# electech6/ORB_SLAM3_detailed_comments

Measured on AMD Instinct MI355X. Metric: frames/sec ORB extract+match, 752x480 stereo @1200 feat (1 frame = 1 stereo pair; BASELINE.json configs[1]), higher is better.
Workload: dtype u8

## Files before the change

orb_slam3_detailed_comments_amd/csrc/k_describe.hip:

```cpp
#include "orbx_types.h"
#include "orbx_block.h"
#include "orbx_simd.h"
#include "orbx_kernels.h"
#include "undistort_model.h"
#include "glibc_sincosf_model.h"
#include "glibc_logf_model.h"
#include "glibc_tanf_model.h"
#include "glibc_atan2f_model.h"

namespace orbx {

__device__ const signed char d_brief_pattern[1024] = {
#include "brief_pattern.inc"
};
#define BRIEF_PATTERN d_brief_pattern

__device__ __forceinline__ float fast_atan2_deg(float y, float x) {
    const float s = (float)(180.0 / 3.1415926535897932384626433832795);
    const float p1 = 0.9997878412794807f * s, p3 = -0.3258083974640975f * s;
    const float p5 = 0.1555786518463281f * s, p7 = -0.04432655554792128f * s;
    const float eps = 2.2204460492503131e-16f;
    const float ax = fabsf(x), ay = fabsf(y);
    float a, c, c2;
    if (ax >= ay) {
        c = __fdiv_rn(ay, __fadd_rn(ax, eps)); c2 = __fmul_rn(c, c);
        a = __fmul_rn(__fadd_rn(__fmul_rn(__fadd_rn(__fmul_rn(__fadd_rn(__fmul_rn(p7, c2), p5), c2), p3), c2), p1), c);
    } else {
        c = __fdiv_rn(ax, __fadd_rn(ay, eps)); c2 = __fmul_rn(c, c);
        a = __fsub_rn(90.f, __fmul_rn(__fadd_rn(__fmul_rn(__fadd_rn(__fmul_rn(__fadd_rn(__fmul_rn(p7, c2), p5), c2), p3), c2), p1), c));
    }
    if (x < 0) a = __fsub_rn(180.f, a);
    if (y < 0) a = __fsub_rn(360.f, a);
    return a;
}

__device__ __forceinline__ void steer_from_moments(float m01, float m10, float* angle, float* a, float* b) {
    const float ang = fast_atan2_deg(m01, m10);
    const float factorPI = (float)(3.1415926535897932384626433832795 / 180.f);
    const float rad = __fmul_rn(ang, factorPI);
    *angle = ang; *a = glibc_cosf(rad); *b = glibc_sinf(rad);
}

constexpr int kLayoutPer = 8;
__global__ void __launch_bounds__(256) k_layout(const LevelInfo* __restrict__ lv, int nlevels,
                                                const uint32_t* __restrict__ lvl_keys, int kp_total_cap,
                                                const int* __restrict__ lvl_count, int lap0, int lap1,
                                                int* __restrict__ final_idx, int* __restrict__ n_out, int* __restrict__ mono_out,
                                                int nb, int* __restrict__ row_start, int* __restrict__ row_items) {
    ORBX_DYN_SMEM(smem);
    __shared__ unsigned long long s_scan[20];
    __shared__ int s_cnt[kMaxLevels], s_off[kMaxLevels + 1];
    __shared__ float s_scale[kMaxLevels];
    const int b = (int)blockIdx.x, tid = (int)threadIdx.x;
    if (tid < nlevels) { s_cnt[tid] = lvl_count[(size_t)b * nlevels + tid]; s_off[tid] = lv[tid].kp_off; s_scale[tid] = lv[tid].scale; }
    if (tid == 0) s_off[nlevels] = kp_total_cap;
    int* hist = (int*)smem; int* cursor = hist + (nb + 1);
    if (row_start != nullptr) for (int i = tid; i <= nb; i += 256) hist[i] = 0;
    __syncthreads();
    auto bucket_of = [&](uint32_t key, int l) {
        float yf = (float)(key_y(key) + kBorder);
        if (l != 0) yf = __fmul_rn(yf, s_scale[l]);
        const int first = (int)floorf(__fsub_rn(yf, __fmul_rn(2.0f, s_scale[l])));
        return imin(imax(first, 0) >> kStereoRowShift, nb - 1);
    };
    int total = 0;
    for (int l = 0; l < nlevels; l++) total += s_cnt[l];
    int mono_run = 0, lap_run = 0;
    int valid[kLayoutPer], lvl[kLayoutPer], fin[kLayoutPer];
    uint32_t key[kLayoutPer];
    for (int base = 0; base < kp_total_cap; base += 256 * kLayoutPer) {
        const int s0 = base + tid * kLayoutPer;
        int l = 0;
        while (l + 1 < nlevels && s_off[l + 1] <= s0) l++;
#pragma unroll
        for (int k = 0; k < kLayoutPer; k++) {
            const int s = s0 + k;
            while (l + 1 < nlevels && s_off[l + 1] <= s) l++;
            lvl[k] = l;
            valid[k] = s < kp_total_cap && s - s_off[l] < s_cnt[l];
            key[k] = valid[k] ? lvl_keys[(size_t)b * kp_total_cap + s] : 0u;
        }
        int lapf[kLayoutPer], nm = 0, nl = 0;
#pragma unroll
        for (int k = 0; k < kLayoutPer; k++) {
            float xf = (float)(key_x(key[k]) + kBorder);
            if (lvl[k] != 0) xf = __fmul_rn(xf, s_scale[lvl[k]]);
            lapf[k] = valid[k] && xf >= (float)lap0 && xf <= (float)lap1;
            nm += valid[k] && !lapf[k]; nl += lapf[k];
            if (row_start != nullptr && valid[k]) atomicAdd(&hist[bucket_of(key[k], lvl[k])], 1);
        }
        unsigned long long tot;
        const unsigned long long ex = block_excl_scan<unsigned long long>((unsigned long long)nm | ((unsigned long long)nl << 32), &tot, s_scan);
        int pm = mono_run + (int)(ex & 0xFFFFFFFFu), pl = lap_run + (int)(ex >> 32);
#pragma unroll
        for (int k = 0; k < kLayoutPer; k++) {
            fin[k] = lapf[k] ? total - 1 - pl : pm;
            if (valid[k]) { final_idx[(size_t)b * kp_total_cap + s0 + k] = fin[k]; if (lapf[k]) pl++; else pm++; }
            else if (s0 + k < kp_total_cap) final_idx[(size_t)b * kp_total_cap + s0 + k] = total + (s0 + k) - (pm + pl);
        }
        mono_run += (int)(tot & 0xFFFFFFFFu); lap_run += (int)(tot >> 32);
    }
    if (tid == 0) { n_out[b] = total; mono_out[b] = mono_run; }
    if (row_start == nullptr) return;
    __syncthreads();
    int run = 0;
    for (int c0 = 0; c0 < nb; c0 += 256) {
        const int c = c0 + tid;
        const int v = c < nb ? hist[c] : 0;
        unsigned long long tot;
        const int ex = run + (int)block_excl_scan<unsigned long long>((unsigned long long)v, &tot, s_scan);
        if (c < nb) { cursor[c] = ex; row_start[(size_t)b * (nb + 1) + c] = ex; }
        run += (int)tot;
    }
    if (tid == 0) row_start[(size_t)b * (nb + 1) + nb] = run;
    __syncthreads();
    if (kp_total_cap <= 256 * kLayoutPer) {
#pragma unroll
        for (int k = 0; k < kLayoutPer; k++)
            if (valid[k]) row_items[(size_t)b * kp_total_cap + atomicAdd(&cursor[bucket_of(key[k], lvl[k])], 1)] = fin[k];
        return;
    }
    int l = 0;
    for (int s = tid; s < kp_total_cap; s += 256) {
        while (l + 1 < nlevels && s_off[l + 1] <= s) l++;
        if (s - s_off[l] < s_cnt[l])
            row_items[(size_t)b * kp_total_cap + atomicAdd(&cursor[bucket_of(lvl_keys[(size_t)b * kp_total_cap + s], l)], 1)] = final_idx[(size_t)b * kp_total_cap + s];
    }
}

constexpr int kKpPerWave = 8;
constexpr int kWinR = 18, kWinRows = 2 * kWinR + 1, kWinDw = 10, kWinTrips = (kWinRows * kWinDw + 63) / 64;
static_assert(kKpPerWave == kKpPerWaveDecl, "orbx_kernels.h out of date");
constexpr int kKpPerWaveSmall = kKpPerWaveSmallDecl;
template <int KPW>
__device__ __forceinline__ void orient_brief_impl(const LevelInfo* __restrict__ lv, int nlevels,
                                                      const uint8_t* __restrict__ pyr, const uint8_t* __restrict__ blur, size_t pyr_stride,
                                                      const uint32_t* __restrict__ lvl_keys, int kp_total_cap,
                                                      const int* __restrict__ lvl_count, const int* __restrict__ final_idx,
                                                      UmaxTab umax, KeyPointRec* __restrict__ out_kps,
                                                      unsigned long long* __restrict__ out_desc, int4* __restrict__ out_aux, int B, int groups_per_image) {
    __shared__ __attribute__((aligned(16))) uint8_t s_win[4][kWinRows * kWinDw * 4];
    const int id = (int)blockIdx.x, nx = groups_per_image;
    const int b = 8 * (id / (8 * nx)) + (id & 7), gx = (id >> 3) % nx;
    if (b >= B) return;
    const int lane = lane_id();
    const int slot0 = (gx * 4 + (int)(threadIdx.x >> 6)) * KPW;
    if (slot0 >= kp_total_cap) return;
    const int myslot = slot0 + (lane < KPW ? lane : 0);
    int my_valid = 0, my_level = 0, my_pitch = 0, my_fi = 0;
    uint32_t my_key = 0;
    int my_off = 0;
    if (myslot < kp_total_cap) {
        for (int l = 1; l < nlevels; l++) if (myslot >= lv[l].kp_off) my_level = l;
        const int i = myslot - lv[my_level].kp_off;
        my_valid = i < lvl_count[(size_t)b * nlevels + my_level];
        if (!my_valid && lane < KPW) {
            const int zrow = final_idx[(size_t)b * kp_total_cap + myslot];
            unsigned long long* z = out_desc + ((size_t)b * kp_total_cap + zrow) * 4;
            z[0] = 0ull; z[1] = 0ull; z[2] = 0ull; z[3] = 0ull;
        }
        if (my_valid) {
            my_key = lvl_keys[(size_t)b * kp_total_cap + myslot];
            my_pitch = lv[my_level].pitch;
            my_off = (int)lv[my_level].off + (key_y(my_key) + kBorder) * my_pitch + (key_x(my_key) + kBorder);
            my_fi = final_idx[(size_t)b * kp_total_cap + myslot];
        }
    }
    const unsigned long long vmask = __ballot(my_valid && lane < KPW);
    if (vmask == 0ull) return;
    const BufRsrc raw0 = buf_make(pyr + (size_t)b * pyr_stride);
    const BufRsrc blur0 = buf_make(blur + (size_t)b * pyr_stride);
    const int r8 = lane >> 3, cg = lane & 7;
    uint32_t wu4[4], wv4[4], on4[4];
#pragma unroll
    for (int trip = 0; trip < 4; trip++) {
        const int v = -kHalfPatch + 8 * trip + r8;
        const int av = v < 0 ? -v : v;
        uint32_t pu = 0, pv = 0, po = 0;
#pragma unroll
        for (int j = 0; j < 4; j++) {
            const int u = -kHalfPatch + 4 * cg + j;
            const int au = u < 0 ? -u : u;
            const bool on = av <= kHalfPatch && au <= kHalfPatch && au <= umax.u[av <= kHalfPatch ? av : 0];
            if (on) { pu |= (uint32_t)(u + 16) << (8 * j); pv |= (uint32_t)(v + 16) << (8 * j); po |= 1u << (8 * j); }
        }
        wu4[trip] = pu; wv4[trip] = pv; on4[trip] = po;
    }
    int my_m10 = 0, my_m01 = 0;
    for (int k = 0; k < KPW; k++) {
        if (!((vmask >> k) & 1ull)) continue;
        const int pitch = ORBX_READLANE(my_pitch, k);
        const uint32_t so = (uint32_t)(ORBX_READLANE(my_off, k) - kHalfPatch * pitch - kHalfPatch);
        uint32_t I4[4];
#pragma unroll
        for (int trip = 0; trip < 4; trip++)
            I4[trip] = buf_load_u32(raw0, (uint32_t)(__mul24(8 * trip + r8, pitch) + 4 * cg), so);
        uint32_t du = 0, dv = 0, ds = 0;
#pragma unroll
        for (int trip = 0; trip < 4; trip++) { du = dot4_u8(I4[trip], wu4[trip], du); dv = dot4_u8(I4[trip], wv4[trip], dv); ds = dot4_u8(I4[trip], on4[trip], ds); }
        int m10 = (int)du - 16 * (int)ds, m01 = (int)dv - 16 * (int)ds;
        m10 = wave_sum(m10); m01 = wave_sum(m01);
        if (lane == k) { my_m10 = m10; my_m01 = m01; }
    }
    float my_angle, my_a, my_b;
    steer_from_moments((float)my_m01, (float)my_m10, &my_angle, &my_a, &my_b);
    float px0[4], py0[4], px1[4], py1[4];
#pragma unroll
    for (int r = 0; r < 4; r++) {
        const signed char* p = &BRIEF_PATTERN[4 * (64 * r + lane)];
        px0[r] = (float)p[0]; py0[r] = (float)p[1]; px1[r] = (float)p[2]; py1[r] = (float)p[3];
    }
    uint8_t* win = s_win[threadIdx.x >> 6];
    for (int k = 0; k < KPW; k++) {
        if (!((vmask >> k) & 1ull)) continue;
        const int pitch = ORBX_READLANE(my_pitch, k);
        const uint32_t so = (uint32_t)(ORBX_READLANE(my_off, k) - kWinR * pitch - kWinR);
        const float a = __int_as_float(ORBX_READLANE(__float_as_int(my_a), k)), bb = __int_as_float(ORBX_READLANE(__float_as_int(my_b), k));
        const int fi = ORBX_READLANE(my_fi, k);
        uint32_t wv[kWinTrips];
#pragma unroll
        for (int t = 0; t < kWinTrips; t++) {
            const int i = lane + 64 * t;
            if (i < kWinRows * kWinDw) wv[t] = buf_load_u32(blur0, (uint32_t)(__mul24(i / kWinDw, pitch) + 4 * (i % kWinDw)), so);
        }
        ORBX_WAVE_SYNC();
#pragma unroll
        for (int t = 0; t < kWinTrips; t++) { const int i = lane + 64 * t; if (i < kWinRows * kWinDw) ((uint32_t*)win)[i] = wv[t]; }
        ORBX_WAVE_SYNC();
        constexpr float kRoundMagic = 12582912.0f;
        constexpr uint32_t kRoundFold = 0x400000u * (4u * kWinDw) + 0x4B400000u - (uint32_t)(kWinR * 4 * kWinDw + kWinR);
        int t0v[4], t1v[4];
#pragma unroll
        for (int r = 0; r < 4; r++) {
            const uint32_t r0 = __float_as_uint(__fadd_rn(__fadd_rn(__fmul_rn(px0[r], bb), __fmul_rn(py0[r], a)), kRoundMagic));
            const uint32_t c0 = __float_as_uint(__fadd_rn(__fsub_rn(__fmul_rn(px0[r], a), __fmul_rn(py0[r], bb)), kRoundMagic));
            const uint32_t r1 = __float_as_uint(__fadd_rn(__fadd_rn(__fmul_rn(px1[r], bb), __fmul_rn(py1[r], a)), kRoundMagic));
            const uint32_t c1 = __float_as_uint(__fadd_rn(__fsub_rn(__fmul_rn(px1[r], a), __fmul_rn(py1[r], bb)), kRoundMagic));
            t0v[r] = win[(uint32_t)__umul24(r0, 4 * kWinDw) + c0 - kRoundFold];
            t1v[r] = win[(uint32_t)__umul24(r1, 4 * kWinDw) + c1 - kRoundFold];
        }
        unsigned long long mine = 0;
#pragma unroll
        for (int r = 0; r < 4; r++) {
            const unsigned long long w = ORBX_BALLOT(t0v[r] < t1v[r]);
            if (lane == r) mine = w;
        }
        if (lane < 4) out_desc[((size_t)b * kp_total_cap + fi) * 4 + lane] = mine;
    }
    if (lane < KPW && my_valid) {
        const LevelInfo L = lv[my_level];
        KeyPointRec k;
        float xf = (float)(key_x(my_key) + kBorder), yf = (float)(key_y(my_key) + kBorder);
        if (my_level != 0) { xf = __fmul_rn(xf, L.scale); yf = __fmul_rn(yf, L.scale); }
        k.x = xf; k.y = yf; k.size = (float)L.patch; k.angle = my_angle; k.response = (float)key_s(my_key);
        k.octave = my_level; k.class_id = -1;
        out_kps[(size_t)b * kp_total_cap + my_fi] = k;
        const float r = __fmul_rn(2.0f, L.scale);
        int4 aux; aux.x = (int)floorf(__fsub_rn(yf, r)); aux.y = (int)ceilf(__fadd_rn(yf, r)); aux.z = __float_as_int(xf); aux.w = my_level;
        out_aux[(size_t)b * kp_total_cap + my_fi] = aux;
    }
}

__global__ void __launch_bounds__(256) k_orient_brief(const LevelInfo* __restrict__ lv, int nlevels,
                                                      const uint8_t* __restrict__ pyr, const uint8_t* __restrict__ blur, size_t pyr_stride,
                                                      const uint32_t* __restrict__ lvl_keys, int kp_total_cap,
                                                      const int* __restrict__ lvl_count, const int* __restrict__ final_idx,
                                                      UmaxTab umax, KeyPointRec* __restrict__ out_kps,
                                                      unsigned long long* __restrict__ out_desc, int4* __restrict__ out_aux, int B, int groups_per_image) {
    orient_brief_impl<kKpPerWave>(lv, nlevels, pyr, blur, pyr_stride, lvl_keys, kp_total_cap, lvl_count, final_idx, umax, out_kps, out_desc, out_aux, B, groups_per_image);
}
__global__ void __launch_bounds__(256) k_orient_brief_small(const LevelInfo* __restrict__ lv, int nlevels,
                                                      const uint8_t* __restrict__ pyr, const uint8_t* __restrict__ blur, size_t pyr_stride,
                                                      const uint32_t* __restrict__ lvl_keys, int kp_total_cap,
                                                      const int* __restrict__ lvl_count, const int* __restrict__ final_idx,
                                                      UmaxTab umax, KeyPointRec* __restrict__ out_kps,
                                                      unsigned long long* __restrict__ out_desc, int4* __restrict__ out_aux, int B, int groups_per_image) {
    orient_brief_impl<kKpPerWaveSmall>(lv, nlevels, pyr, blur, pyr_stride, lvl_keys, kp_total_cap, lvl_count, final_idx, umax, out_kps, out_desc, out_aux, B, groups_per_image);
}

__global__ void __launch_bounds__(256) k_undistort(const KeyPointRec* __restrict__ kps, const int* __restrict__ n_per_frame, int cap, UndistortParams U,
                                                   KeyPointRec* __restrict__ kps_un) {
    const size_t b = blockIdx.y;
    const int i = (int)(blockIdx.x * 256 + threadIdx.x);
    if (i >= cap || i >= n_per_frame[b]) return;
    KeyPointRec k = kps[b * (size_t)cap + i];
    float x, y;
    undistort_point(U, k.x, k.y, &x, &y);
    k.x = x; k.y = y;
    kps_un[b * (size_t)cap + i] = k;
}

__global__ void __launch_bounds__(256) k_model_selftest(int op, uint32_t start_bits, const float* __restrict__ a, const float* __restrict__ b, int n,
                                                        float* __restrict__ out) {
    const int i = (int)(blockIdx.x * 256 + threadIdx.x);
    if (i >= n) return;
    const float x = a != nullptr ? a[i] : at_float(start_bits + (uint32_t)i);
    const float y = b != nullptr ? b[i] : 0.0f;
    float r = 0.0f;
    switch (op) {
        case 0: r = glibc_cosf(x); break;
        case 1: r = glibc_sinf(x); break;
        case 2: r = glibc_logf_model<false>(x); break;
        case 3: r = glibc_tanf_model(x); break;
        case 4: r = glibc_atanf_model(x); break;
        case 5: r = glibc_atan2f_model(x, y); break;
        case 6: r = fast_atan2_deg(x, y); break;
        default: {
            float ca, sa;
            steer_from_moments(x, y, &r, &ca, &sa);
            out[(size_t)n + i] = ca; out[2 * (size_t)n + i] = sa;
        }
    }
    out[i] = r;
}

}
```

orb_slam3_detailed_comments_amd/csrc/k_match.hip:

```cpp
#include "orbx_types.h"
#include "orbx_block.h"
#include "orbx_kernels.h"
#include "orbx_simd.h"
#include "kb8_model.h"

namespace orbx {

__device__ __forceinline__ int hamming256(const unsigned long long* __restrict__ a, const unsigned long long* __restrict__ b) {
    return __popcll(a[0] ^ b[0]) + __popcll(a[1] ^ b[1]) + __popcll(a[2] ^ b[2]) + __popcll(a[3] ^ b[3]);
}

__global__ void __launch_bounds__(256) k_hamming_matrix(const unsigned long long* __restrict__ A, int na,
                                                        const unsigned long long* __restrict__ Bm, int nb,
                                                        int* __restrict__ out) {
    const int i = (int)blockIdx.y, j = (int)(blockIdx.x * 256 + threadIdx.x);
    if (i >= na || j >= nb) return;
    out[(size_t)i * nb + j] = hamming256(A + 4 * (size_t)i, Bm + 4 * (size_t)j);
}

__global__ void __launch_bounds__(256) k_stereo_match(const LevelInfo* __restrict__ lv,
                                                      const KeyPointRec* __restrict__ kpsL, const unsigned long long* __restrict__ descL, const int* __restrict__ nL,
                                                      const KeyPointRec* __restrict__ kpsR, const unsigned long long* __restrict__ descR,
                                                      const int4* __restrict__ auxR, const int* __restrict__ nR,
                                                      const int* __restrict__ bucket_start, const int* __restrict__ bucket_items, int nb, int lookback,
                                                      int cap, const uint8_t* __restrict__ pyrL, const uint8_t* __restrict__ pyrR, size_t pyr_stride,
                                                      StereoParams P, float* __restrict__ uRight, float* __restrict__ depth, int* __restrict__ sad) {
    const int b = (int)blockIdx.y, lane = lane_id();
    const int iL = (int)blockIdx.x * 4 + (int)(threadIdx.x >> 6);
    if (iL >= cap) return;
    const size_t o = (size_t)b * cap + iL;
    if (iL >= nL[b]) { if (lane == 0) { uRight[o] = -1.0f; depth[o] = -1.0f; sad[o] = -1; } return; }
    const KeyPointRec kL = kpsL[o];
    const int levelL = kL.octave;
    const float uL = kL.x, vL = kL.y;
    const float maxD = __fdiv_rn(P.mbf, P.mb);
    const float minU = __fsub_rn(uL, maxD), maxU = uL;
    float out_u = -1.0f, out_d = -1.0f; int out_sad = -1;
    const int rowL = __float2int_rz(vL);
    const int nr = nR[b];
    unsigned best = (unsigned)P.th_high << 16;
    if (!(maxU < 0)) {
        const unsigned long long* dl = descL + 4 * o;
        const unsigned long long d0 = dl[0], d1 = dl[1], d2 = dl[2], d3 = dl[3];
        const int4* ar = auxR + (size_t)b * cap;
        const int* bs = bucket_start + (size_t)b * (nb + 1);
        const int* items = bucket_items + (size_t)b * cap;
        const int jbeg = bs[imin(imax(rowL - lookback, 0) >> kStereoRowShift, nb - 1)], jend = bs[imin(imax(rowL, 0) >> kStereoRowShift, nb - 1) + 1];
        auto visit = [&](int iR, const int4& a) {
            if (rowL < a.x || rowL > a.y) return;
            if (a.w < levelL - 1 || a.w > levelL + 1) return;
            const float xr = __int_as_float(a.z);
            if (xr >= minU && xr <= maxU) {
                const unsigned long long* dr = descR + 4 * ((size_t)b * cap + iR);
                const int dist = __popcll(d0 ^ dr[0]) + __popcll(d1 ^ dr[1]) + __popcll(d2 ^ dr[2]) + __popcll(d3 ^ dr[3]);
                const unsigned cand = ((unsigned)dist << 16) | (unsigned)iR;
                if ((P.debug_flags & 2) ? dist < (int)(best >> 16) : cand < best) best = cand;
            }
        };
        if (P.debug_flags & 4) {
            for (int j = jend - 1; j >= jbeg; j--) { const int iR = items[j]; visit(iR, ar[iR]); }
        } else
        for (int base = jbeg; base < jend; base += 128) {
            int4 a[2]; int idx[2];
#pragma unroll
            for (int u = 0; u < 2; u++) {
                int j = base + 64 * u + lane;
                const bool in = j < jend;
                if (P.debug_flags & 1) j = jend - 1 - (j - jbeg);
                idx[u] = in ? items[j] : -1;
            }
#pragma unroll
            for (int u = 0; u < 2; u++) {
                if (idx[u] >= 0) a[u] = ar[idx[u]]; else { a[u].x = 1; a[u].y = 0; a[u].z = 0; a[u].w = 0; }
            }
#pragma unroll
            for (int u = 0; u < 2; u++) visit(idx[u], a[u]);
        }
    }
    best = wave_min_u32(best);
    const int bestDist = (int)(best >> 16);
    if (bestDist < P.th_orb && nr > 0) {
        const int bestIdxR = (int)(best & 0xFFFFu);
        const float uR0 = kpsR[(size_t)b * cap + bestIdxR].x;
        const LevelInfo Lv = lv[levelL];
        const float sf = Lv.inv_scale;
        const float scaleduL = roundf(__fmul_rn(kL.x, sf)), scaledvL = roundf(__fmul_rn(kL.y, sf));
        const float scaleduR0 = roundf(__fmul_rn(uR0, sf));
        const int w = 5, Lh = 5;
        const float iniu = scaleduR0 + (float)(Lh - w), endu = scaleduR0 + (float)(Lh + w + 1);
        const int cu = (int)scaleduL, cv = (int)scaledvL, cr = (int)scaleduR0;
        const bool inb = cv - w >= 0 && cv + w < Lv.h && cu - w >= 0 && cu + w < Lv.w && cr - Lh - w >= 0 && cr + Lh + w < Lv.w;
        if (!(iniu < 0 || endu >= (float)Lv.w) && inb) {
            const uint8_t* IL = pyrL + (size_t)b * pyr_stride + Lv.off;
            const uint8_t* IR = pyrR + (size_t)b * pyr_stride + Lv.off;
            const int g = lane >> 4, k = lane & 15;
            uint32_t acc = 0;
            if (k < 11) {
#pragma unroll
                for (int t = 0; t < 3; t++) {
                    const int row = g + 4 * t;
                    if (row < 11) {
                        const int rofs = __mul24(cv - w + row, Lv.pitch);
                        const uint8_t* lp = IL + (uint32_t)(rofs + (cu - w));
                        const uint8_t* rp = IR + (uint32_t)(rofs + (cr - w - Lh + k));
                        const uint32_t l0 = load_u32_any(lp), l1 = load_u32_any(lp + 4), l2 = load_u32_any(lp + 7) & 0xFFFFFF00u;
                        const uint32_t r0 = load_u32_any(rp), r1 = load_u32_any(rp + 4), r2 = load_u32_any(rp + 7) & 0xFFFFFF00u;
                        acc = sad4_u8(l0, r0, sad4_u8(l1, r1, sad4_u8(l2, r2, acc)));
                    }
                }
            }
            acc += __shfl_xor(acc, 16);
            acc += __shfl_xor(acc, 32);
            const unsigned skey = wave_min_u32(k < 11 ? (acc << 4) | (unsigned)k : 0xFFFFFFFFu);
            const int bestS = (int)(skey >> 4), bi = (int)(skey & 15u), bestinc = bi - Lh;
            if (!(bestinc == -Lh || bestinc == Lh)) {
                const float dist1 = (float)ORBX_READLANE(acc, bi - 1), dist2 = (float)bestS, dist3 = (float)ORBX_READLANE(acc, bi + 1);
                const float deltaR = __fdiv_rn(__fsub_rn(dist1, dist3),
                                               __fmul_rn(2.0f, __fsub_rn(__fadd_rn(dist1, dist3), __fmul_rn(2.0f, dist2))));
                if (!(deltaR < -1 || deltaR > 1)) {
                    float bestuR = __fmul_rn(Lv.scale, __fadd_rn(__fadd_rn(scaleduR0, (float)bestinc), deltaR));
                    float disparity = __fsub_rn(uL, bestuR);
                    if (disparity >= 0 && disparity < maxD) {
                        if (disparity <= 0) { disparity = 0.01f; bestuR = (float)((double)uL - 0.01); }
                        out_d = __fdiv_rn(P.mbf, disparity);
                        out_u = bestuR;
                        out_sad = bestS;
                    }
                }
            }
        }
    }
    if (lane == 0) { uRight[o] = out_u; depth[o] = out_d; sad[o] = out_sad; }
}

__global__ void __launch_bounds__(256) k_stereo_median(const int* __restrict__ nL, int cap,
                                                       float* __restrict__ uRight, float* __restrict__ depth,
                                                       const int* __restrict__ sad, int* __restrict__ n_matches) {
    __shared__ unsigned long long s_scan[20];
    __shared__ int s_hist[256];
    __shared__ int s_med[3];
    const int b = (int)blockIdx.x, tid = (int)threadIdx.x;
    const int n = nL[b];
    const int* sd = sad + (size_t)b * cap;
    int med = -1;
    for (int pass = 0; pass < 2; pass++) {
        s_hist[tid] = 0;
        __syncthreads();
        const int bin = pass ? s_med[1] : 0;
        for (int i = tid; i < n; i += 256) {
            const int s = sd[i];
            if (s >= 0 && (pass == 0 || (s >> 7) == bin)) atomicAdd(&s_hist[pass ? s & 127 : imin(s >> 7, 255)], 1);
        }
        __syncthreads();
        unsigned long long tot;
        const int c = s_hist[tid];
        const int ex = (int)block_excl_scan<unsigned long long>((unsigned long long)c, &tot, s_scan);
        const int cnt = pass ? 0 : (int)tot;
        if (pass == 0 && cnt == 0) { if (tid == 0) n_matches[b] = 0; return; }
        const int k = pass ? s_med[2] : cnt / 2;
        if (ex <= k && k < ex + c) {
            if (pass == 0) { s_med[1] = tid; s_med[2] = k - ex; }
            else s_med[0] = (bin << 7) | tid;
        }
        __syncthreads();
    }
    med = s_med[0];
    const float median = (float)med;
    const float thDist = __fmul_rn(1.5f * 1.4f, median);
    int kept = 0;
    for (int i = tid; i < n; i += 256) {
        const int s = sad[(size_t)b * cap + i];
        if (s >= 0) {
            if (!((float)s < thDist)) { uRight[(size_t)b * cap + i] = -1.0f; depth[(size_t)b * cap + i] = -1.0f; }
            else kept++;
        }
    }
    kept = wave_sum(kept);
    if ((tid & 63) == 0) s_scan[tid >> 6] = (unsigned long long)kept;
    __syncthreads();
    if (tid == 0) n_matches[b] = (int)(s_scan[0] + s_scan[1] + s_scan[2] + s_scan[3]);
}

__global__ void __launch_bounds__(256) k_knn2(const unsigned long long* __restrict__ descQ, const int* __restrict__ qoff, const int* __restrict__ nq,
                                              const unsigned long long* __restrict__ descT, const int* __restrict__ toff, const int* __restrict__ nt,
                                              int cap, int* __restrict__ idx0, int* __restrict__ dist0, int* __restrict__ idx1, int* __restrict__ dist1,
                                              uint8_t* __restrict__ ratio_ok) {
    const int b = (int)blockIdx.y, lane = lane_id();
    const int q = (int)blockIdx.x * 4 + (int)(threadIdx.x >> 6);
    const int q0 = qoff ? qoff[b] : 0, t0 = toff ? toff[b] : 0;
    const int nQ = nq[b] - q0, nT = nt[b] - t0;
    if (q >= cap) return;
    const size_t o = (size_t)b * cap + q;
    if (q >= nQ) { if (lane == 0) { idx0[o] = -1; idx1[o] = -1; dist0[o] = -1; dist1[o] = -1; ratio_ok[o] = 0; } return; }
    const unsigned long long* dq = descQ + 4 * ((size_t)b * cap + q0 + q);
    const unsigned long long a0 = dq[0], a1 = dq[1], a2 = dq[2], a3 = dq[3];
    unsigned k0 = 0xFFFFFFFFu, k1 = 0xFFFFFFFFu;
    for (int j = lane; j < nT; j += 64) {
        const unsigned long long* dt = descT + 4 * ((size_t)b * cap + t0 + j);
        const int d = __popcll(a0 ^ dt[0]) + __popcll(a1 ^ dt[1]) + __popcll(a2 ^ dt[2]) + __popcll(a3 ^ dt[3]);
        const unsigned key = ((unsigned)d << 16) | (unsigned)j;
        if (key < k0) { k1 = k0; k0 = key; } else if (key < k1) k1 = key;
    }
    const unsigned b0 = wave_min_u32(k0);
    if (k0 == b0) k0 = k1;
    const unsigned b1 = wave_min_u32(k0);
    if (lane == 0) {
        const int i0 = b0 == 0xFFFFFFFFu ? -1 : (int)(b0 & 0xFFFF), i1 = b1 == 0xFFFFFFFFu ? -1 : (int)(b1 & 0xFFFF);
        const int dd0 = i0 < 0 ? -1 : (int)(b0 >> 16), dd1 = i1 < 0 ? -1 : (int)(b1 >> 16);
        idx0[o] = i0; idx1[o] = i1; dist0[o] = dd0; dist1[o] = dd1;
        ratio_ok[o] = (i1 >= 0 && (double)(float)dd0 < (double)(float)dd1 * 0.7) ? 1 : 0;
    }
}

__global__ void __launch_bounds__(256) k_knn2_mfma(const unsigned long long* __restrict__ descQ, const int* __restrict__ qoff, const int* __restrict__ nq,
                                                   const unsigned long long* __restrict__ descT, const int* __restrict__ toff, const int* __restrict__ nt,
                                                   int cap, int* __restrict__ idx0, int* __restrict__ dist0, int* __restrict__ idx1,
                                                   int* __restrict__ dist1, uint8_t* __restrict__ ratio_ok) {
    __shared__ unsigned s_top[4][32][2];
    __shared__ uint32_t s_lut[16];
    const int b = (int)blockIdx.y, lane = lane_id(), w = wave_id();
    const int qbase = (int)blockIdx.x * 32;
    const int q0 = qoff ? qoff[b] : 0, t0 = toff ? toff[b] : 0;
    const int nQ = nq[b] - q0, nT = nt[b] - t0;
    unsigned k0 = 0xFFFFFFFFu, k1 = 0xFFFFFFFFu;
    if (qbase < nQ) {
        if (threadIdx.x < 16) {
            const uint32_t bits = (uint32_t)__umul24((uint32_t)threadIdx.x, 0x204081u) & 0x01010101u;
            s_lut[threadIdx.x] = 0x01010101u | ((bits << 8) - bits);
        }
        __syncthreads();
        const int r = lane & 31, hoff = 16 * (lane >> 5);
        auto expand = [&](const uint32_t raw[4], int s) {
            const uint32_t h = (raw[s >> 1] >> (16 * (s & 1))) & 0xFFFFu;
            v4i_t v; int e[4];
#pragma unroll
            for (int j = 0; j < 4; j++) e[j] = (int)s_lut[(h >> (4 * j)) & 15u];
            __builtin_memcpy(&v, e, 16);
            return v;
        };
        auto load_bits = [&](const unsigned long long* desc, int row, uint32_t raw[4]) {
            __builtin_memcpy(raw, (const uint8_t*)(desc + 4 * ((size_t)b * cap + imin(row, cap - 1))) + hoff, 16);
        };
        v4i_t qb[8];
        {
            uint32_t raw[4];
            load_bits(descQ, q0 + qbase + r, raw);
#pragma unroll
            for (int s = 0; s < 8; s++) qb[s] = expand(raw, s);
        }
        const int ntiles = (nT + 31) >> 5;
        const int mlane = (256 << 15) + 4 * (lane >> 5);
        auto process = [&](const uint32_t raw[4], int tt) {
            v16i_t acc = v16i_zero();
#pragma unroll
            for (int s = 0; s < 8; s++) acc = mfma_i8_32x32x32(expand(raw, s), qb[s], acc);
            const int base = mlane + tt * 32;
            if ((tt + 1) * 32 <= nT) {
#pragma unroll
                for (int i = 0; i < 16; i++) {
                    const unsigned key = (unsigned)(__mul24(acc[i], -32768) + base + ((i & 3) + 8 * (i >> 2)));
                    k1 = umin32(k1, umax32(k0, key)); k0 = umin32(k0, key);
                }
            } else {
#pragma unroll
                for (int i = 0; i < 16; i++) {
                    unsigned key = (unsigned)(__mul24(acc[i], -32768) + base + ((i & 3) + 8 * (i >> 2)));
                    if ((int)(key & 0xFFFFu) >= nT) key = 0xFFFFFFFFu;
                    k1 = umin32(k1, umax32(k0, key)); k0 = umin32(k0, key);
                }
            }
        };
        uint32_t ta[4], tb[4];
        int tt = w;
        if (tt < ntiles) load_bits(descT, t0 + tt * 32 + r, ta);
        for (; tt + 4 < ntiles; tt += 8) {
            load_bits(descT, t0 + (tt + 4) * 32 + r, tb);
            process(ta, tt);
            if (tt + 8 < ntiles) load_bits(descT, t0 + (tt + 8) * 32 + r, ta);
            process(tb, tt + 4);
        }
        if (tt < ntiles) process(ta, tt);
        const unsigned p0 = __shfl_xor(k0, 32), p1 = __shfl_xor(k1, 32);
        const unsigned b0 = umin32(k0, p0), b1 = umin32(umax32(k0, p0), umin32(k1, p1));
        k0 = b0; k1 = b1;
        if (lane < 32) { s_top[w][lane][0] = k0; s_top[w][lane][1] = k1; }
        __syncthreads();
        if (w == 0 && lane < 32) {
#pragma unroll
            for (int o = 1; o < 4; o++) {
                const unsigned c0 = s_top[o][lane][0], c1 = s_top[o][lane][1];
                const unsigned n1 = umin32(umax32(k0, c0), umin32(k1, c1));
                k0 = umin32(k0, c0); k1 = n1;
            }
        }
    }
    const int q = qbase + lane;
    if (w == 0 && lane < 32 && q < cap) {
        const size_t o = (size_t)b * cap + q;
        if (q >= nQ) { idx0[o] = -1; idx1[o] = -1; dist0[o] = -1; dist1[o] = -1; ratio_ok[o] = 0; }
        else {
            const int i0 = k0 == 0xFFFFFFFFu ? -1 : (int)(k0 & 0xFFFF), i1 = k1 == 0xFFFFFFFFu ? -1 : (int)(k1 & 0xFFFF);
            const int dd0 = i0 < 0 ? -1 : (int)(k0 >> 16), dd1 = i1 < 0 ? -1 : (int)(k1 >> 16);
            idx0[o] = i0; idx1[o] = i1; dist0[o] = dd0; dist1[o] = dd1;
            ratio_ok[o] = (i1 >= 0 && (double)(float)dd0 < (double)(float)dd1 * 0.7) ? 1 : 0;
        }
    }
}

__global__ void __launch_bounds__(256) k_kb8_stereo(const KeyPointRec* __restrict__ kpsL, const int* __restrict__ monoL, const int* __restrict__ nL,
                                                    const KeyPointRec* __restrict__ kpsR, const int* __restrict__ monoR, int cap,
                                                    const int* __restrict__ idx0, const uint8_t* __restrict__ ratio_ok, KB8StereoParams P,
                                                    int* __restrict__ l2r, int* __restrict__ r2l, float* __restrict__ depth, float* __restrict__ p3d,
                                                    int* __restrict__ nmatches) {
    __shared__ int s_list[256];
    __shared__ int s_n;
    const int b = (int)blockIdx.y, i = (int)(blockIdx.x * 256 + threadIdx.x);
    if (threadIdx.x == 0) s_n = 0;
    __syncthreads();
    if (i < cap) {
        const size_t o = (size_t)b * cap + i;
        l2r[o] = -1; depth[o] = -1.0f;
        p3d[3 * o] = 0.f; p3d[3 * o + 1] = 0.f; p3d[3 * o + 2] = 0.f;
        const int q = i - monoL[b];
        if (i < nL[b] && q >= 0 && ratio_ok[(size_t)b * cap + q]) s_list[atomicAdd(&s_n, 1)] = i;
    }
    __syncthreads();
    if ((int)threadIdx.x < s_n) {
        const int i2 = s_list[threadIdx.x];
        const size_t o = (size_t)b * cap + i2;
        const int j = idx0[(size_t)b * cap + (i2 - monoL[b])] + monoR[b];
        const KeyPointRec kl = kpsL[o], kr = kpsR[(size_t)b * cap + j];
        KB8Cam c1, c2;
#pragma unroll
        for (int k = 0; k < 8; k++) { c1.p[k] = P.cam1[k]; c2.p[k] = P.cam2[k]; }
        float r1[3], r2[3], p[3];
        kb8_unproject(c1, kl.x, kl.y, r1);
        kb8_unproject(c2, kr.x, kr.y, r2);
        const float z = kb8_triangulate_matches(c1, c2, r1, r2, kl.x, kl.y, kr.x, kr.y, P.R12, P.t12, pick(P.sigma2, kl.octave), pick(P.sigma2, kr.octave), p);
        if (z > 0.0001f) {
            l2r[o] = j; depth[o] = z;
            p3d[3 * o] = p[0]; p3d[3 * o + 1] = p[1]; p3d[3 * o + 2] = p[2];
            atomicMax(&r2l[(size_t)b * cap + j], i2);
            atomicAdd(&nmatches[b], 1);
        }
    }
}

__global__ void __launch_bounds__(256) k_distinctive(const unsigned long long* __restrict__ desc, const int* __restrict__ start, int P,
                                                     int* __restrict__ best) {
    __shared__ int s_hist[4][320];
    const int lane = lane_id(), w = wave_id();
    const int p = (int)blockIdx.x * 4 + w;
    if (p >= P) return;
    const int s0 = start[p], N = start[p + 1] - s0;
    int* hist = s_hist[w];
#pragma unroll
    for (int t = 0; t < 5; t++) hist[lane * 5 + t] = 0;
    ORBX_WAVE_SYNC();
    if (N <= 0) { if (lane == 0) best[p] = -1; return; }
    const int rank = (N - 1) >> 1;
    int bestMedian = 0x7fffffff, bestIdx = 0;
    for (int i = 0; i < N; i++) {
        const unsigned long long* di = desc + 4 * (size_t)(s0 + i);
        const unsigned long long a0 = di[0], a1 = di[1], a2 = di[2], a3 = di[3];
        for (int j = lane; j < N; j += 64) {
            const unsigned long long* dj = desc + 4 * (size_t)(s0 + j);
            const int d = __popcll(a0 ^ dj[0]) + __popcll(a1 ^ dj[1]) + __popcll(a2 ^ dj[2]) + __popcll(a3 ^ dj[3]);
            atomicAdd(&hist[d], 1);
        }
        ORBX_WAVE_SYNC();
        int c[5], mine = 0;
#pragma unroll
        for (int t = 0; t < 5; t++) { c[t] = hist[lane * 5 + t]; mine += c[t]; }
        const int incl = wave_incl_scan(mine);
        int before = incl - mine, median = -1;
        if (before <= rank && rank < incl) {
#pragma unroll
            for (int t = 0; t < 5; t++) { if (median < 0 && rank < before + c[t]) median = lane * 5 + t; before += c[t]; }
        }
        const unsigned long long who = __ballot(median >= 0);
        median = __shfl(median, __ffsll(who) - 1);
        if (median < bestMedian) { bestMedian = median; bestIdx = i; }
#pragma unroll
        for (int t = 0; t < 5; t++) hist[lane * 5 + t] = 0;
        ORBX_WAVE_SYNC();
    }
    if (lane == 0) best[p] = bestIdx;
}

template <bool kLds>
__device__ __forceinline__ void distinctive_point(const DistinctiveRec R, int r, const unsigned long long* const* __restrict__ kf_desc,
                                                  const int* __restrict__ obs_kf, const int* __restrict__ obs_feat, int* __restrict__ best,
                                                  unsigned long long* __restrict__ best_desc, unsigned long long* cols) {
    constexpr int kChunks = kLds ? kDistinctiveMax / 64 : 1, kNever = 0x7fff;
    const int lane = lane_id(), N = R.n, rank = (N - 1) >> 1;
    unsigned long long c0 = 0, c1 = 0, c2 = 0, c3 = 0;
    if (kLds) {
        for (int j = lane; j < N; j += 64) {
            const unsigned long long* dj = kf_desc[obs_kf[R.start + j]] + 4 * (size_t)obs_feat[R.start + j];
            cols[j] = dj[0]; cols[N + j] = dj[1]; cols[2 * N + j] = dj[2]; cols[3 * N + j] = dj[3];
        }
        __syncthreads();
    } else if (lane < N) {
        const unsigned long long* dj = kf_desc[obs_kf[R.start + lane]] + 4 * (size_t)obs_feat[R.start + lane];
        c0 = dj[0]; c1 = dj[1]; c2 = dj[2]; c3 = dj[3];
    }
    int bestMedian = 257, bestIdx = 0;
    for (int i = 0; i < N; i++) {
        unsigned long long a0, a1, a2, a3;
        int d[kChunks];
        if (kLds) {
            a0 = cols[i]; a1 = cols[N + i]; a2 = cols[2 * N + i]; a3 = cols[3 * N + i];
#pragma unroll
            for (int c = 0; c < kChunks; c++) {
                if (c * 64 < N) {
                    const int j = c * 64 + lane, jj = imin(j, N - 1);
                    const int dist = __popcll(a0 ^ cols[jj]) + __popcll(a1 ^ cols[N + jj]) + __popcll(a2 ^ cols[2 * N + jj]) + __popcll(a3 ^ cols[3 * N + jj]);
                    d[c] = dist + (j < N ? 0 : kNever);
                }
            }
        } else {
            a0 = (unsigned long long)readlane_i64((long long)c0, i); a1 = (unsigned long long)readlane_i64((long long)c1, i);
            a2 = (unsigned long long)readlane_i64((long long)c2, i); a3 = (unsigned long long)readlane_i64((long long)c3, i);
            d[0] = __popcll(a0 ^ c0) + __popcll(a1 ^ c1) + __popcll(a2 ^ c2) + __popcll(a3 ^ c3) + (lane < N ? 0 : kNever);
        }
        auto count_le = [&](int v) {
            int n = 0;
#pragma unroll
            for (int c = 0; c < kChunks; c++)
                if (c * 64 < N) n += __popcll(ORBX_BALLOT(d[c] <= v));
            return n;
        };
        if (count_le(bestMedian - 1) > rank) {
            int lo = 0, hi = bestMedian - 1;
            while (lo < hi) {
                const int mid = (lo + hi) >> 1;
                if (count_le(mid) > rank) hi = mid; else lo = mid + 1;
            }
            bestMedian = lo; bestIdx = i;
        }
    }
    if (kLds) {
        if (lane < 4) {
            const unsigned long long v = cols[lane * N + bestIdx];
            best_desc[4 * (size_t)r + lane] = v;
            if (R.store) R.store[lane] = v;
        }
    } else if (lane == bestIdx) {
        unsigned long long* o = best_desc + 4 * (size_t)r;
        o[0] = c0; o[1] = c1; o[2] = c2; o[3] = c3;
        if (R.store) { R.store[0] = c0; R.store[1] = c1; R.store[2] = c2; R.store[3] = c3; }
    }
    if (lane == 0) best[r] = bestIdx;
}

template <bool kLds>
__global__ void __launch_bounds__(256) k_distinctive_resident(const DistinctiveRec* __restrict__ recs, int first, int count,
                                                              const unsigned long long* const* __restrict__ kf_desc, const int* __restrict__ obs_kf,
                                                              const int* __restrict__ obs_feat, int* __restrict__ best, unsigned long long* __restrict__ best_desc) {
    ORBX_DYN_SMEM(smem);
    const int k = (int)blockIdx.x * (int)(blockDim.x >> 6) + ORBX_UNIFORM(wave_id());
    if (k >= count) return;
    const int r = first + k;
    distinctive_point<kLds>(recs[r], r, kf_desc, obs_kf, obs_feat, best, best_desc, kLds ? (unsigned long long*)smem : nullptr);
}
template __global__ void k_distinctive_resident<false>(const DistinctiveRec* __restrict__, int, int, const unsigned long long* const* __restrict__, const int* __restrict__,
                                                       const int* __restrict__, int* __restrict__, unsigned long long* __restrict__);
template __global__ void k_distinctive_resident<true>(const DistinctiveRec* __restrict__, int, int, const unsigned long long* const* __restrict__, const int* __restrict__,
                                                      const int* __restrict__, int* __restrict__, unsigned long long* __restrict__);

}
```

orb_slam3_detailed_comments_amd/csrc/orbx_api.cpp:

```cpp
#include <mutex>
#include "orbx_internal.h"

#ifndef ORBX_PYR_FUSED_BATCH
#define ORBX_PYR_FUSED_BATCH 8
#endif
#ifndef ORBX_RESIZE_MIN_BLOCKS
#define ORBX_RESIZE_MIN_BLOCKS 2048
#endif
#ifndef ORBX_RESIZE_STRIP
#define ORBX_RESIZE_STRIP 16
#endif
#ifndef ORBX_FAST_LIST_BYTES
#define ORBX_FAST_LIST_BYTES 2048
#endif
#ifndef ORBX_QT_BIG_PIXELS
#define ORBX_QT_BIG_PIXELS 40000
#endif
#ifndef ORBX_QT_WIDE_BATCH
#define ORBX_QT_WIDE_BATCH 32
#endif
#ifndef ORBX_PRESORT_MAX
#define ORBX_PRESORT_MAX 5
#endif

using namespace orbx;

namespace orbx {
static thread_local std::string g_err;
int fail(int code, const char* fmt, ...) {
    char buf[512]; va_list ap; va_start(ap, fmt); vsnprintf(buf, sizeof buf, fmt, ap); va_end(ap);
    g_err = buf; return code;
}
const char* last_error_string() { return g_err.c_str(); }
}

namespace {
const char* kStageNames[ORBX_NSTAGES] = {"import", "pyramid", "fast_cells", "quadtree", "blur", "layout", "orient_brief", "match"};
}

namespace {

void init_tables(orbx_extractor* h) {
    h->scale[0] = 1.0f; h->sigma2[0] = 1.0f;
    for (int i = 1; i < h->nlevels; i++) {
        h->scale[i] = (float)(h->scale[i - 1] * h->scaleFactor);
        h->sigma2[i] = h->scale[i] * h->scale[i];
    }
    for (int i = 0; i < h->nlevels; i++) {
        h->inv_scale[i] = 1.0f / h->scale[i];
        h->inv_sigma2[i] = 1.0f / h->sigma2[i];
    }
    const float factor = (float)(1.0f / h->scaleFactor);
    float want = h->nfeatures * (1 - factor) / (1 - (float)pow((double)factor, (double)h->nlevels));
    int sum = 0;
    for (int l = 0; l < h->nlevels - 1; l++) {
        h->quota[l] = round_half_even_f(want);
        sum += h->quota[l];
        want *= factor;
    }
    h->quota[h->nlevels - 1] = std::max(h->nfeatures - sum, 0);
    int* um = h->umax.u;
    const int vmax = (int)floor(kHalfPatch * sqrt(2.f) / 2 + 1), vmin = (int)ceil(kHalfPatch * sqrt(2.f) / 2);
    const double hp2 = kHalfPatch * kHalfPatch;
    for (int v = 0; v <= vmax; ++v) um[v] = round_half_even_d(sqrt(hp2 - v * v));
    for (int v = kHalfPatch, v0 = 0; v >= vmin; --v) {
        while (um[v0] == um[v0 + 1]) ++v0;
        um[v] = v0;
        ++v0;
    }
}

void resize_axis(int ssize, int dsize, bool clamp_edges, std::vector<ResizeTap>& out) {
    const double inv = (double)dsize / ssize, sc = 1.0 / inv;
    for (int d = 0; d < dsize; d++) {
        float f = (float)((d + 0.5) * sc - 0.5);
        int s = (int)floorf(f);
        f -= s;
        if (clamp_edges) {
            if (s < 0) { f = 0; s = 0; }
            if (s >= ssize - 1) { f = 0; s = ssize - 1; }
        }
        int a0 = round_half_even_f((1.f - f) * 2048.f), a1 = round_half_even_f(f * 2048.f);
        a0 = std::min(std::max(a0, -32768), 32767); a1 = std::min(std::max(a1, -32768), 32767);
        ResizeTap t; t.ofs = s; t.w = (a0 & 0xFFFF) | (a1 << 16);
        out.push_back(t);
    }
}

void pyramid_spans(const orbx_extractor* h, bool columns, std::vector<PyrSpan>& out, int& ntiles, int* max_extent) {
    const int nl = h->nlevels, top = nl - 1;
    auto size_of = [&](int l) { return columns ? h->lv[l].w : h->lv[l].h; };
    auto taps_of = [&](int l) { return (columns ? h->xtab.data() + h->lv[l].xtab_off : h->ytab.data() + h->lv[l].ytab_off); };
    auto lo = [&](int l, int d) { return std::min(std::max(taps_of(l)[d].ofs, 0), size_of(l - 1) - 1); };
    auto hi = [&](int l, int d) { return std::min(std::max(taps_of(l)[d].ofs + 1, 0), size_of(l - 1) - 1); };
    const int T = (size_of(top) + kPyrTile - 1) / kPyrTile;
    ntiles = T;
    for (int l = 0; l < nl; l++) max_extent[l] = 0;
    out.assign((size_t)T * nl, PyrSpan{0, 0, 0, 0});
    std::vector<int> own0((size_t)(T + 1) * nl);
    for (int t = 0; t <= T; t++) own0[(size_t)t * nl + top] = std::min(t * kPyrTile, size_of(top));
    for (int l = top - 1; l >= 0; l--)
        for (int t = 0; t <= T; t++)
            own0[(size_t)t * nl + l] = t == 0 ? 0 : t == T ? size_of(l) : lo(l + 1, own0[(size_t)t * nl + l + 1]);
    for (int t = 0; t < T; t++) {
        int a = 0, b = 0;
        for (int l = top; l >= 0; l--) {
            const int o0 = own0[(size_t)t * nl + l], o1 = own0[(size_t)(t + 1) * nl + l];
            if (l == top) { a = o0; b = o1; }
            else {
                const int na = lo(l + 1, a), nb = hi(l + 1, std::min(b, size_of(l + 1)) - 1) + 1;
                a = l == 0 ? na : std::min(o0, na); b = l == 0 ? nb : std::max(o1, nb);
            }
            if (columns) { a &= ~3; b = (b + 3) & ~3; }
            PyrSpan sp; sp.a = (int16_t)a; sp.b = (int16_t)b; sp.o0 = (int16_t)o0; sp.o1 = (int16_t)o1;
            out[(size_t)t * nl + l] = sp;
            max_extent[l] = std::max(max_extent[l], b - a);
        }
    }
}

struct QuadtreePlan { int first_lds, node_cap_lds, lut_x, lut_y; size_t smem_lds, smem_spill, pool_stride; };
QuadtreePlan quadtree_plan(const orbx_extractor* h, int counter_bytes) {
    QuadtreePlan p;
    p.lut_x = (int)align_up((size_t)h->lv[0].bw + 1, 8); p.lut_y = (int)align_up((size_t)h->lv[0].bh + 1, 8);
    const size_t tables = (size_t)(h->nb_cap + 2) * 4 + (size_t)(counter_bytes + (counter_bytes == 32 ? 4 : 0)) * h->nb_cap + 2 * (size_t)(p.lut_x + p.lut_y) + 64;
    const size_t limit = rt::lds_limit(h->device);
    p.first_lds = h->nlevels; p.node_cap_lds = 0; p.smem_lds = 0;
    int cap = 0;
    for (int l = h->nlevels - 1; l >= 0; l--) {
        cap = std::max(cap, h->lv[l].kp_cap + 8);
        const size_t smem = align_up((size_t)cap * 81, 16) + tables;
        if (cap > h->qt_lds_nodes || smem + 2048 > limit) break;
        p.first_lds = l; p.node_cap_lds = cap; p.smem_lds = smem;
    }
    p.smem_spill = tables;
    p.pool_stride = align_up((size_t)h->node_cap * 81, 256);
    return p;
}

void export_layout(orbx_extractor* h) {
    FrameLayout& fl = h->exp_fl;
    memset(&fl, 0, sizeof fl);
    fl.edge = h->exp_edge;
    size_t off = 0; int bands = 0;
    for (int l = 0; l < h->nlevels; l++) {
        const int fw = h->lv[l].w + 2 * fl.edge, fh = h->lv[l].h + 2 * fl.edge;
        fl.step[l] = (int)align_up((size_t)fw, 16);
        fl.off[l] = (int)off; off = align_up(off + (size_t)fl.step[l] * fh, 64);
        fl.band[l] = bands; bands += (fh + kFrameRows - 1) / kFrameRows;
    }
    for (int l = h->nlevels; l <= kMaxLevels; l++) fl.band[l] = bands;
    h->exp_stride = align_up(off, 256);
}
int export_drain(orbx_extractor* h) { return h->have_exp_stream ? rt::stream_sync(h->s_exp) : 0; }
int export_prepare(orbx_extractor* h) {
    if (h->exp_edge <= 0 || h->W <= 0 || h->maxB <= 0) return ORBX_OK;
    if (export_drain(h)) return fail(ORBX_E_DEVICE, "export stream sync failed: %s", rt::last_error());
    export_layout(h);
    const size_t bytes = (size_t)h->maxB * h->exp_stride;
    if (bytes != h->exp_cap) h->exp_slot = -1;
    int e = h->d_exp.ensure(bytes);
    for (int k = 0; k < h->exp_depth; k++) e |= h->h_exp[k].ensure(bytes);
    if (e) return fail(ORBX_E_DEVICE, "allocation of the pyramid export (%d slots of %zu bytes) failed", h->exp_depth, bytes);
    h->exp_cap = bytes;
    return ORBX_OK;
}
void export_release(orbx_extractor* h) {
    export_drain(h);
    h->d_exp.release();
    for (auto& x : h->h_exp) x.release();
    for (auto& ev : h->ev_exp_slot) { rt::event_destroy(ev); ev = 0; }
    rt::event_destroy(h->ev_exp_fork); rt::event_destroy(h->ev_exp_read); h->ev_exp_fork = h->ev_exp_read = 0;
    if (h->have_exp_stream) rt::stream_destroy(h->s_exp);
    h->s_exp = 0; h->have_exp_stream = false;
    h->exp_edge = h->exp_depth = 0; h->exp_slot = -1; h->exp_B = 0; h->exp_cap = 0; h->exp_count = 0; h->exp_pending = h->exp_guard = false;
}
int export_enqueue(orbx_extractor* h, int B) {
    if (h->d_exp.n < (size_t)B * h->exp_stride) return fail(ORBX_E_INTERNAL, "pyramid export staging not allocated");
    const int slot = (int)(h->exp_count % (uint64_t)h->exp_depth);
    int e = rt::event_record(h->ev_exp_fork, h->s0) | rt::stream_wait_event(h->s_exp, h->ev_exp_fork);
    ORBX_LAUNCH(k_frame_pyramid, dim3(h->exp_fl.band[h->nlevels], B, 1), dim3(256, 1, 1), 0, h->s_exp, (const LevelInfo*)h->d_lv.p, h->nlevels,
                (const uint8_t*)h->d_pyr.p, h->pyr_stride, h->d_exp.p, h->exp_stride, h->exp_fl);
    e |= rt::event_record(h->ev_exp_read, h->s_exp);
    e |= rt::copy_d2h(h->h_exp[slot].p, h->d_exp.p, (size_t)B * h->exp_stride, h->s_exp);
    e |= rt::event_record(h->ev_exp_slot[slot], h->s_exp);
    if (e || rt::check_launch()) return fail(ORBX_E_DEVICE, "pyramid export failed: %s", rt::last_error());
    h->exp_slot = slot; h->exp_B = B; h->exp_count++; h->exp_pending = h->exp_guard = true;
    return ORBX_OK;
}

int configure(orbx_extractor* h, int W, int H, int B) {
    if (W <= 0 || H <= 0 || B <= 0) return fail(ORBX_E_ARG, "bad size %dx%d batch %d", W, H, B);
    const bool same_geom = (W == h->W && H == h->H);
    if (same_geom && B <= h->maxB && h->cfg_qt_lds_nodes == h->qt_lds_nodes) return ORBX_OK;
    if (rt::set_device(h->device)) return fail(ORBX_E_DEVICE, "hipSetDevice(%d) failed", h->device);
    if (export_drain(h)) return fail(ORBX_E_DEVICE, "export stream sync failed: %s", rt::last_error());
    if (!same_geom) {
        h->exp_slot = -1;
        if (W - 2 * kBorder > 4095 || H - 2 * kBorder > 4095) return fail(ORBX_E_ARG, "image larger than 4127 px is not supported");
        h->W = h->H = 0; h->maxB = 0; h->lastB = 0; h->ncells = 0; h->kp_total_cap = 0;
        h->cells.clear(); h->xtab.clear(); h->ytab.clear();
        size_t off = 0; int cand_off = 0, kp_off = 0, node_cap = 0, tile_b = 0, inner_b = 0, nb_cap = 1;
        for (int l = 0; l < h->nlevels; l++) {
            LevelInfo& L = h->lv[l];
            memset(&L, 0, sizeof L);
            L.w = round_half_even_f((float)W * h->inv_scale[l]);
            L.h = round_half_even_f((float)H * h->inv_scale[l]);
            L.pitch = (int)align_up((size_t)L.w, 64);
            L.off = (int)off; off += align_up((size_t)L.pitch * L.h, 256);
            L.scale = h->scale[l]; L.inv_scale = h->inv_scale[l]; L.quota = h->quota[l];
            L.patch = (int)(31 * h->scale[l]);
            const float Wc = 35;
            const int minBX = kBorder, minBY = kBorder, maxBX = L.w - kBorder, maxBY = L.h - kBorder;
            const float width = (float)(maxBX - minBX), height = (float)(maxBY - minBY);
            if (width < Wc || height < Wc) return fail(ORBX_E_ARG, "level %d (%dx%d) is too small for the 35-px FAST cell grid", l, L.w, L.h);
            L.ncols = (int)(width / Wc); L.nrows = (int)(height / Wc);
            L.wcell = (int)ceil(width / L.ncols); L.hcell = (int)ceil(height / L.nrows);
            L.bw = maxBX - minBX; L.bh = maxBY - minBY;
            L.nini = (int)roundf((float)L.bw / (float)L.bh);
            if (L.nini < 1) return fail(ORBX_E_ARG, "aspect ratio < 0.5 is not supported (the reference divides by zero)");
            L.hX = (float)L.bw / (float)L.nini;
            L.cell_begin = (int)h->cells.size();
            L.cand_off = cand_off;
            int slot = cand_off;
            for (int i = 0; i < L.nrows; i++) {
                const float iniY = (float)(minBY + i * L.hcell);
                float maxY = iniY + L.hcell + 6;
                if (iniY >= maxBY - 3) continue;
                if (maxY > maxBY) maxY = (float)maxBY;
                for (int j = 0; j < L.ncols; j++) {
                    const float iniX = (float)(minBX + j * L.wcell);
                    float maxX = iniX + L.wcell + 6;
                    if (iniX >= maxBX - 6) continue;
                    if (maxX > maxBX) maxX = (float)maxBX;
                    CellInfo c; memset(&c, 0, sizeof c);
                    c.level = (int16_t)l;
                    c.x0 = (int16_t)((int)iniX + 3); c.x1 = (int16_t)((int)maxX - 3);
                    c.y0 = (int16_t)((int)iniY + 3); c.y1 = (int16_t)((int)maxY - 3);
                    c.slot_off = slot;
                    const int iw = std::max(c.x1 - c.x0, 0), ih = std::max(c.y1 - c.y0, 0);
                    slot += ((iw + 1) / 2) * ((ih + 1) / 2);
                    if (iw > 0 && ih > 0) {
                        const int gx0 = (c.x0 - 3) & ~3, gx1 = (c.x1 + 3 + 3) & ~3;
                        const int wp = gx1 - gx0 <= kFastPitch ? kFastPitch : gx1 - gx0;
                        if (iw > 240 || iw * ih >= 8192 || wp * (ih + 6) > 16384) return fail(ORBX_E_ARG, "FAST cell too large");
                        tile_b = std::max(tile_b, wp * (ih + 6));
                        inner_b = std::max(inner_b, wp * (ih + 2));
                    }
                    h->cells.push_back(c);
                }
            }
            L.cell_count = (int)h->cells.size() - L.cell_begin;
            L.cand_cap = slot - cand_off;
            cand_off = slot;
            L.kp_cap = std::max(L.quota + 3, 4 * L.nini);
            L.kp_off = kp_off; kp_off += L.kp_cap;
            L.presort_depth = 0;
            while (L.presort_depth < ORBX_PRESORT_MAX && L.nini * (1 << (2 * (L.presort_depth + 1))) <= 1024) L.presort_depth++;
            nb_cap = std::max(nb_cap, L.nini * (1 << (2 * L.presort_depth)));
            L.qt_threads = (long long)L.bw * L.bh >= ORBX_QT_BIG_PIXELS ? kQuadtreeThreads : 256;
            node_cap = std::max(node_cap, L.kp_cap + 8);
            if (l > 0) {
                L.xtab_off = (int)h->xtab.size(); resize_axis(h->lv[l - 1].w, L.w, true, h->xtab);
                L.ytab_off = (int)h->ytab.size(); resize_axis(h->lv[l - 1].h, L.h, false, h->ytab);
                bool ok = true;
                const ResizeTap* xt = h->xtab.data() + L.xtab_off;
                for (int x = 0; x < L.w && ok; x += 4)
                    for (int k = 0; k < 4; k++) { const int xx = std::min(x + k, L.w - 1); if (std::min(xt[xx].ofs + 1, h->lv[l - 1].w - 1) - xt[x].ofs > 7 || xt[xx].ofs < xt[x].ofs) ok = false; }
                h->resize_rows_ok[l] = ok;
            }
        }
        h->pyr_stride = off; h->cand_stride = (size_t)cand_off; h->ncells = (int)h->cells.size();
        h->pyr_fused_ok = false; h->xspan.clear(); h->yspan.clear();
        if (h->nlevels > 1) {
            int mw[kMaxLevels], mh[kMaxLevels];
            pyramid_spans(h, true, h->xspan, h->pyr_ntx, mw);
            pyramid_spans(h, false, h->yspan, h->pyr_nty, mh);
            int nt = 0;
            for (int l = 1; l < h->nlevels; l++) { h->pyr_toff.x[l] = nt; nt += mw[l]; h->pyr_toff.y[l] = nt; nt += mh[l]; }
            h->pyr_toff.total = nt;
            size_t bufa = 0, bufb = 0, items = 0;
            for (int tx = 0; tx < h->pyr_ntx; tx++)
                for (int ty = 0; ty < h->pyr_nty; ty++)
                    for (int l = 0; l < h->nlevels; l++) {
                        const PyrSpan& sx = h->xspan[(size_t)tx * h->nlevels + l]; const PyrSpan& sy = h->yspan[(size_t)ty * h->nlevels + l];
                        const size_t bytes = (size_t)(sx.b - sx.a) * (sy.b - sy.a);
                        (l & 1 ? bufb : bufa) = std::max(l & 1 ? bufb : bufa, bytes);
                        items = std::max(items, bytes / 4);
                    }
            h->pyr_buf_a = (int)align_up(bufa, 16); h->pyr_buf_b = (int)align_up(bufb, 16);
            h->pyr_fused_ok = items < 8192 && (size_t)h->pyr_buf_a + h->pyr_buf_b + 8 * (size_t)nt + 48 * (size_t)h->nlevels <= 60000;
        }
        h->kp_total_cap = kp_off; h->node_cap = node_cap; h->nb_cap = nb_cap;
        h->fast_tile_bytes = (int)align_up((size_t)tile_b, 16); h->fast_inner_bytes = (int)align_up((size_t)inner_b, 16);
        if (h->kp_total_cap >= 65535) { h->kp_total_cap = 0; return fail(ORBX_E_ARG, "nfeatures too large"); }
        int e = 0;
        e |= h->d_lv.ensure(kMaxLevels); e |= h->d_cells.ensure(h->cells.size());
        e |= h->d_xtab.ensure(std::max<size_t>(h->xtab.size(), 1)); e |= h->d_ytab.ensure(std::max<size_t>(h->ytab.size(), 1));
        e |= h->d_xspan.ensure(std::max<size_t>(h->xspan.size(), 1)); e |= h->d_yspan.ensure(std::max<size_t>(h->yspan.size(), 1));
        if (e) return fail(ORBX_E_DEVICE, "device allocation failed (tables)");
        rt::copy_h2d(h->d_lv.p, h->lv, sizeof(LevelInfo) * kMaxLevels, h->s0);
        rt::copy_h2d(h->d_cells.p, h->cells.data(), sizeof(CellInfo) * h->cells.size(), h->s0);
        if (!h->xtab.empty()) rt::copy_h2d(h->d_xtab.p, h->xtab.data(), sizeof(ResizeTap) * h->xtab.size(), h->s0);
        if (!h->ytab.empty()) rt::copy_h2d(h->d_ytab.p, h->ytab.data(), sizeof(ResizeTap) * h->ytab.size(), h->s0);
        if (!h->xspan.empty()) rt::copy_h2d(h->d_xspan.p, h->xspan.data(), sizeof(PyrSpan) * h->xspan.size(), h->s0);
        if (!h->yspan.empty()) rt::copy_h2d(h->d_yspan.p, h->yspan.data(), sizeof(PyrSpan) * h->yspan.size(), h->s0);
        if (rt::stream_sync(h->s0)) return fail(ORBX_E_DEVICE, "table upload failed: %s", rt::last_error());
        h->W = W; h->H = H;
    }
    if (B > h->maxB || h->cfg_qt_lds_nodes != h->qt_lds_nodes) {
        const QuadtreePlan qp = quadtree_plan(h, 32);
        if (qp.first_lds > 0 && h->d_qtpool.ensure((size_t)std::max(B, h->maxB) * qp.first_lds * qp.pool_stride))
            return fail(ORBX_E_DEVICE, "device allocation failed (quadtree node pool, batch %d of %dx%d)", B, W, H);
        h->cfg_qt_lds_nodes = h->qt_lds_nodes;
    }
    if (B > h->maxB) {
        const size_t b = (size_t)B, cap = (size_t)h->kp_total_cap;
        int e = 0;
        e |= h->d_pyr.ensure(b * h->pyr_stride + 256); e |= h->d_blur.ensure(b * h->pyr_stride + 256);
        e |= h->d_slots.ensure(b * h->cand_stride + 4); e |= h->d_candA.ensure(b * h->cand_stride + 4); e |= h->d_candB.ensure(b * h->cand_stride + 4);
        e |= h->d_cell_count.ensure(b * h->ncells); e |= h->d_lvl_count.ensure(b * h->nlevels); e |= h->d_qtsorted.ensure(b * h->nlevels);
        e |= h->d_lvl_keys.ensure(b * cap); e |= h->d_final_idx.ensure(b * cap);
        e |= h->d_nm.ensure(2 * b + 4);
        h->d_status.p = h->d_nm.p ? h->d_nm.p + 2 * b : nullptr; h->d_status.n = h->d_nm.p ? 4 : 0;
        e |= h->d_kps.ensure(b * cap); e |= h->d_desc.ensure(b * cap * 4); e |= h->d_aux.ensure(b * cap * 4);
        e |= h->d_uRight.ensure(b * cap); e |= h->d_depth.ensure(b * cap); e |= h->d_sad.ensure(b * cap); e |= h->d_nmatch.ensure(b);
        e |= h->d_rowstart.ensure(b * (size_t)((h->H >> kStereoRowShift) + 3)); e |= h->d_rowitems.ensure(b * cap);
        e |= h->d_knn.ensure(4 * b * cap); e |= h->d_ratio.ensure(b * cap);
        e |= h->h_nm.ensure(3 * b + 4); e |= h->h_cnt.ensure(2 * b + 4); e |= h->d_qtprof.ensure(32);
        if (e) return fail(ORBX_E_DEVICE, "device allocation failed (batch %d of %dx%d)", B, W, H);
        h->cnt_gen = 0;
        rt::memset_async(h->d_status.p, 0, 4 * sizeof(int), h->s0);
        rt::memset_async(h->d_pyr.p, 0, b * h->pyr_stride + 256, h->s0);
        h->maxB = B;
    }
    return export_prepare(h);
}

void stage_begin(orbx_extractor* h, int st, rt::stream_t s) { if (h->profile) rt::event_record(h->ev_stage[st][0], s); }
void stage_end(orbx_extractor* h, int st, rt::stream_t s) { if (h->profile) rt::event_record(h->ev_stage[st][1], s); }

void enqueue_input(orbx_extractor* h, int B, const uint8_t* d_images, int sw, int sh, int stride, size_t image_stride) {
    const LevelInfo& L0 = h->lv[0];
    const dim3 blk2(64, 4, 1);
    const int C = h->in_channels;
    uint8_t* lvl0 = h->d_pyr.p + L0.off;
    const uint8_t* cur = d_images; int cur_stride = stride; size_t cur_img = image_stride;
    if (h->in_geometry != 0) {
        const bool direct = C == 1;
        uint8_t* dst = direct ? lvl0 : h->d_frame.p;
        const int dpitch = direct ? L0.pitch : L0.w * C; const size_t dstride = direct ? h->pyr_stride : (size_t)L0.w * L0.h * C;
        dim3 grid(((dpitch + C - 1) / C + 63) / 64, (L0.h + 3) / 4, B);
        if (h->in_geometry == 1)
            ORBX_LAUNCH(k_input_remap, grid, blk2, 0, h->s0, cur, sw, sh, cur_stride, cur_img, C, (const float*)h->d_mapx.p, (const float*)h->d_mapy.p,
                        L0.w, L0.h, dst, dpitch, dstride);
        else
            ORBX_LAUNCH(k_input_resize, grid, blk2, 0, h->s0, cur, sw, sh, cur_stride, cur_img, C, (const ResizeTap*)h->d_in_xt.p,
                        (const ResizeTap*)h->d_in_yt.p, L0.w, L0.h, dst, dpitch, dstride);
        cur = dst; cur_stride = dpitch; cur_img = dstride;
        if (direct) return;
    }
    const int ry = h->in_gray_variant ? 4899 : 9798, gy = h->in_gray_variant ? 9617 : 19235, by = h->in_gray_variant ? 1868 : 3735;
    dim3 grid((L0.pitch + 255) / 256, (L0.h + 3) / 4, B);
    ORBX_LAUNCH(k_input_gray, grid, blk2, 0, h->s0, cur, cur_stride, cur_img, C, h->in_rgb ? 0 : 2, ry, gy, by, h->in_gray_variant ? 14 : 15, L0.w, L0.h,
                lvl0, L0.pitch, h->pyr_stride);
}

int enqueue_extract(orbx_extractor* h, int B, const uint8_t* d_images, int src_w, int src_h, int stride, size_t image_stride, int lap0, int lap1, bool capturing) {
    const int nl = h->nlevels;
    const dim3 blk2(64, 4, 1), blk1(256, 1, 1);
    stage_begin(h, ST_IMPORT, h->s0);
    if (h->in_active && (h->in_channels != 1 || h->in_geometry != 0)) enqueue_input(h, B, d_images, src_w, src_h, stride, image_stride);
    else if (d_images == h->d_pyr.p + h->lv[0].off && stride == h->lv[0].pitch && image_stride == h->pyr_stride) {
    } else {
        const LevelInfo& L0 = h->lv[0];
        dim3 grid((L0.pitch + 255) / 256, (L0.h + 3) / 4, B);
        ORBX_LAUNCH(k_import, grid, blk2, 0, h->s0, (const LevelInfo*)h->d_lv.p, d_images, stride, image_stride, h->d_pyr.p, h->pyr_stride);
    }
    stage_end(h, ST_IMPORT, h->s0);
    if (B > ORBX_QT_WIDE_BATCH) { rt::event_record(h->ev_import, h->s0); h->import_lazy = false; }
    else h->import_lazy = true;
    stage_begin(h, ST_PYRAMID, h->s0);
    const bool fused = nl > 1 && h->pyr_fused_ok && (h->pyramid_mode == 2 || (h->pyramid_mode == 0 && B <= ORBX_PYR_FUSED_BATCH));
    if (fused) {
        dim3 grid(h->pyr_ntx * h->pyr_nty, B, 1);
        const size_t smem = (size_t)h->pyr_buf_a + h->pyr_buf_b + 8 * (size_t)h->pyr_toff.total + 48 * (size_t)nl;
        ORBX_LAUNCH(k_pyramid_fused, grid, dim3(kPyrThreads, 1, 1), smem, h->s0, (const LevelInfo*)h->d_lv.p, nl, (const ResizeTap*)h->d_xtab.p, (const ResizeTap*)h->d_ytab.p,
                    (const PyrSpan*)h->d_xspan.p, (const PyrSpan*)h->d_yspan.p, h->pyr_ntx, h->d_pyr.p, h->pyr_stride, h->pyr_buf_a, h->pyr_buf_b, h->pyr_toff);
    }
    for (int l = 1; l < nl && !fused; l++) {
        const LevelInfo& L = h->lv[l]; const LevelInfo& S = h->lv[l - 1];
        if (h->resize_rows_ok[l]) {
            int strip = ORBX_RESIZE_STRIP;
            while (strip > 4 && (long)((L.pitch + 255) / 256) * ((L.h + 4 * strip - 1) / (4 * strip)) * B < ORBX_RESIZE_MIN_BLOCKS) strip >>= 1;
            dim3 gridr((L.pitch + 255) / 256, (L.h + 4 * strip - 1) / (4 * strip), B);
            ORBX_LAUNCH(k_resize_rows, gridr, blk2, 0, h->s0, (const LevelInfo*)h->d_lv.p, l, (const ResizeTap*)h->d_xtab.p, (const ResizeTap*)h->d_ytab.p,
                        h->d_pyr.p, h->pyr_stride, strip);
            continue;
        }
        dim3 grid((L.pitch + 255) / 256, (L.h + kResizeRows - 1) / kResizeRows, B);
        const int lds_pitch = (int)align_up((size_t)ceil(256.0 * S.w / L.w) + 12, 4);
        const int lds_rows = (int)ceil((double)kResizeRows * S.h / L.h) + 3;
        ORBX_LAUNCH(k_resize, grid, blk2, (size_t)lds_pitch * lds_rows, h->s0, (const LevelInfo*)h->d_lv.p, l, (const ResizeTap*)h->d_xtab.p,
                    (const ResizeTap*)h->d_ytab.p, h->d_pyr.p, h->pyr_stride, lds_pitch, lds_rows);
    }
    stage_end(h, ST_PYRAMID, h->s0);
    if (!capturing && h->exp_edge > 0) { const int rc = export_enqueue(h, B); if (rc) return rc; }
    BlurTaps taps;
    {
        static const int A[7] = {18, 34, 48, 56, 48, 34, 18}, Bt[7] = {18, 34, 49, 55, 49, 34, 18};
        for (int i = 0; i < 7; i++) taps.k[i] = h->gauss_variant == 1 ? Bt[i] : A[i];
    }
    const bool blur_large = B > ORBX_QT_WIDE_BATCH;
    const int blur_rows = blur_large ? kBlurRowsLarge : kBlurRows;
    BlurTiles tiles; int nt = 0;
    for (int l = 0; l < nl; l++) { tiles.begin[l] = nt; nt += ((h->lv[l].w + 255) / 256) * ((h->lv[l].h + 4 * blur_rows - 1) / (4 * blur_rows)); }
    for (int l = nl; l <= kMaxLevels; l++) tiles.begin[l] = nt;
    const int fast_blocks = (h->ncells + 8 * kFastXcdRun - 1) / (8 * kFastXcdRun) * (8 * kFastXcdRun);
    const int list_bytes = ORBX_FAST_LIST_BYTES;
    const size_t fast_smem = 16 + (size_t)h->fast_tile_bytes + (size_t)h->fast_inner_bytes + (size_t)list_bytes + 64;
    const dim3 blkf(kFastThreadsDecl, 1, 1);
    const bool small_forms = B <= ORBX_QT_WIDE_BATCH && !h->profile && !h->serial;
    const bool one_launch = small_forms && h->small_forms;
    if (one_launch) {
        dim3 grid(4 * nt + fast_blocks, B, 1);
        ORBX_LAUNCH(k_fast_cells_blur, grid, blkf, fast_smem, h->s0, (const LevelInfo*)h->d_lv.p, (const CellInfo*)h->d_cells.p, h->ncells,
                    (const uint8_t*)h->d_pyr.p, h->pyr_stride, h->iniTh, h->minTh, h->d_slots.p, h->cand_stride, h->d_cell_count.p,
                    h->fast_tile_bytes, list_bytes, h->d_status.p, nl, h->d_blur.p, taps, tiles, 4 * nt);
    } else {
        rt::stream_t sb = h->serial ? h->s0 : h->s1;
        rt::event_record(h->ev_fork, h->s0);
        rt::stream_wait_event(sb, h->ev_fork);
        stage_begin(h, ST_BLUR, sb);
        {
            dim3 grid(nt, B, 1);
            if (blur_large) ORBX_LAUNCH(k_blur_large, grid, blk2, 0, sb, (const LevelInfo*)h->d_lv.p, nl, (const uint8_t*)h->d_pyr.p, h->d_blur.p, h->pyr_stride, taps, tiles);
            else ORBX_LAUNCH(k_blur, grid, blk2, 0, sb, (const LevelInfo*)h->d_lv.p, nl, (const uint8_t*)h->d_pyr.p, h->d_blur.p, h->pyr_stride, taps, tiles);
        }
        stage_end(h, ST_BLUR, sb);
        rt::event_record(h->ev_join, sb);
        stage_begin(h, ST_FAST, h->s0);
        {
            dim3 grid(fast_blocks, B, 1);
            ORBX_LAUNCH(k_fast_cells, grid, blkf, fast_smem, h->s0, (const LevelInfo*)h->d_lv.p, (const CellInfo*)h->d_cells.p, h->ncells,
                        (const uint8_t*)h->d_pyr.p, h->pyr_stride, h->iniTh, h->minTh, h->d_slots.p, h->cand_stride, h->d_cell_count.p,
                        h->fast_tile_bytes, list_bytes, h->d_status.p);
        }
    }
    stage_end(h, ST_FAST, h->s0);
    const int nb_rows = (h->H >> kStereoRowShift) + 2;
    stage_begin(h, ST_QUADTREE, h->s0);
    {
        int qt_block = 256;
        if (B <= ORBX_QT_WIDE_BATCH) for (int l = 0; l < nl; l++) qt_block = std::max(qt_block, h->lv[l].qt_threads);
        const int wide = qt_block > 256, counter_bytes = wide ? 32 : 16;
        const QuadtreePlan qp = quadtree_plan(h, counter_bytes);
        h->qt_pool_levels = qp.first_lds;
        const dim3 blkq(qt_block, 1, 1);
        long long* prof = h->serial ? (long long*)h->d_qtprof.p : (long long*)nullptr;
        if (qp.smem_spill + 2048 > rt::lds_limit(h->device))
            return fail(ORBX_E_CAPACITY, "the quadtree's bucket tables at %dx%d need %zu bytes of LDS, the device allows %zu", h->W, h->H, qp.smem_spill + 2048, rt::lds_limit(h->device));
        if (qp.first_lds > 0) {
            if (h->d_qtpool.n < (size_t)B * qp.first_lds * qp.pool_stride) return fail(ORBX_E_INTERNAL, "quadtree node pool not allocated");
            ORBX_LAUNCH(k_quadtree_spill, dim3(B, qp.first_lds, 1), blkq, qp.smem_spill, h->s0, (const LevelInfo*)h->d_lv.p, (const CellInfo*)h->d_cells.p, h->ncells,
                        (const int*)h->d_cell_count.p, (const uint32_t*)h->d_slots.p, h->cand_stride, h->d_candA.p, h->d_candB.p, h->cand_stride,
                        h->d_lvl_keys.p, h->kp_total_cap, h->d_lvl_count.p, nl, h->node_cap, h->nb_cap, qp.lut_x, qp.lut_y, h->d_status.p,
                        prof, wide, counter_bytes, h->d_qtpool.p, qp.pool_stride, h->d_qtsorted.p, h->qt_eager);
        }
        if (qp.first_lds < nl)
            ORBX_LAUNCH(k_quadtree, dim3(B, nl - qp.first_lds, 1), blkq, qp.smem_lds, h->s0, (const LevelInfo*)h->d_lv.p, (const CellInfo*)h->d_cells.p, h->ncells,
                        (const int*)h->d_cell_count.p, (const uint32_t*)h->d_slots.p, h->cand_stride, h->d_candA.p, h->d_candB.p, h->cand_stride,
                        h->d_lvl_keys.p, h->kp_total_cap, h->d_lvl_count.p, nl, qp.node_cap_lds, h->nb_cap, qp.lut_x, qp.lut_y, h->d_status.p,
                        prof, wide, counter_bytes, qp.first_lds, h->d_qtsorted.p, h->qt_eager);
    }
    stage_end(h, ST_QUADTREE, h->s0);
    stage_begin(h, ST_LAYOUT, h->s0);
    {
        dim3 grid(B, 1, 1);
        ORBX_LAUNCH(k_layout, grid, blk1, 2 * (size_t)(nb_rows + 1) * sizeof(int), h->s0, (const LevelInfo*)h->d_lv.p, nl, (const uint32_t*)h->d_lvl_keys.p, h->kp_total_cap,
                    (const int*)h->d_lvl_count.p, lap0, lap1, h->d_final_idx.p, h->d_nm.p, h->d_nm.p + h->maxB, nb_rows, h->d_rowstart.p, h->d_rowitems.p);
    }
    stage_end(h, ST_LAYOUT, h->s0);
    if (!one_launch) rt::stream_wait_event(h->s0, h->ev_join);
    stage_begin(h, ST_DESCRIBE, h->s0);
    {
        const bool small = B <= ORBX_QT_WIDE_BATCH;
        const int kpw = small ? kKpPerWaveSmallDecl : kKpPerWaveDecl;
        const int gpi = (h->kp_total_cap + 4 * kpw - 1) / (4 * kpw);
        dim3 grid(gpi * 8 * ((B + 7) / 8), 1, 1);
        if (small) ORBX_LAUNCH(k_orient_brief_small, grid, blk1, 0, h->s0, (const LevelInfo*)h->d_lv.p, nl, (const uint8_t*)h->d_pyr.p, (const uint8_t*)h->d_blur.p,
                    h->pyr_stride, (const uint32_t*)h->d_lvl_keys.p, h->kp_total_cap, (const int*)h->d_lvl_count.p, (const int*)h->d_final_idx.p,
                    h->umax, h->d_kps.p, h->d_desc.p, (int4*)h->d_aux.p, B, gpi);
        else ORBX_LAUNCH(k_orient_brief, grid, blk1, 0, h->s0, (const LevelInfo*)h->d_lv.p, nl, (const uint8_t*)h->d_pyr.p, (const uint8_t*)h->d_blur.p,
                    h->pyr_stride, (const uint32_t*)h->d_lvl_keys.p, h->kp_total_cap, (const int*)h->d_lvl_count.p, (const int*)h->d_final_idx.p,
                    h->umax, h->d_kps.p, h->d_desc.p, (int4*)h->d_aux.p, B, gpi);
    }
    if (h->undist.active) {
        dim3 grid((h->kp_total_cap + 255) / 256, B, 1);
        ORBX_LAUNCH(k_undistort, grid, blk1, 0, h->s0, (const KeyPointRec*)h->d_kps.p, (const int*)h->d_nm.p, h->kp_total_cap, h->undist, h->d_kps_un.p);
    }
    stage_end(h, ST_DESCRIBE, h->s0);
    if (B > ORBX_QT_WIDE_BATCH && !capturing) {
        const int e = rt::copy_d2h(h->h_cnt.p, h->d_nm.p, sizeof(int) * (2 * h->maxB + 1), h->s0) | rt::event_record(h->ev_done, h->s0);
        h->done_lazy = false; h->cnt_gen = e ? 0 : h->extract_gen + 1;
    } else h->done_lazy = true;
    h->lastB = B; h->extract_gen++; h->ex_undist_gen = h->undist_gen; h->ex_undist_active = h->undist.active != 0;
    if (rt::check_launch()) return fail(ORBX_E_DEVICE, "kernel launch failed: %s", rt::last_error());
    return ORBX_OK;
}

}

extern "C" {

const char* orbx_last_error(void) { return orbx::last_error_string(); }
const char* orbx_stage_name(int i) { return (i >= 0 && i < ORBX_NSTAGES) ? kStageNames[i] : ""; }
int orbx_device_count(void) { return rt::device_count(); }

int orbx_create(orbx_extractor** out, int nfeatures, float scale_factor, int nlevels, int ini_th, int min_th, int device_id) {
    if (!out) return fail(ORBX_E_ARG, "null out");
    *out = nullptr;
    if (nfeatures <= 0 || nlevels < 1 || nlevels > kMaxLevels || !(scale_factor > 1.0f) || ini_th < 0 || min_th < 0 || ini_th > 255 || min_th > 255)
        return fail(ORBX_E_ARG, "bad extractor parameters");
    if (rt::device_count() <= device_id || device_id < 0) return fail(ORBX_E_DEVICE, "no usable GPU %d (HIP reports %d devices)", device_id, rt::device_count());
    if (rt::set_device(device_id)) return fail(ORBX_E_DEVICE, "hipSetDevice(%d) failed", device_id);
    orbx_extractor* h = new orbx_extractor();
    h->nfeatures = nfeatures; h->scaleFactor = scale_factor; h->nlevels = nlevels; h->iniTh = ini_th; h->minTh = min_th; h->device = device_id;
    init_tables(h);
    int e = rt::stream_create(&h->s0) | rt::stream_create(&h->s1) | rt::stream_create(&h->s_copy) | rt::event_create(&h->ev_fork) | rt::event_create(&h->ev_join) |
            rt::event_create(&h->ev_done) | rt::event_create(&h->ev_copy) | rt::event_create(&h->ev_import) | rt::event_create(&h->ev_lp);
    for (int i = 0; i < ORBX_NSTAGES; i++) { e |= rt::event_create(&h->ev_stage[i][0]); e |= rt::event_create(&h->ev_stage[i][1]); h->stage_ms[i] = 0; }
    h->have_streams = true;
    if (e) { orbx_destroy(h); return fail(ORBX_E_DEVICE, "stream/event creation failed"); }
    *out = h;
    return ORBX_OK;
}

void orbx_destroy(orbx_extractor* h) {
    if (!h) return;
    rt::set_device(h->device);
    export_release(h);
    if (h->have_streams) {
        rt::stream_sync(h->s0); rt::stream_sync(h->s1);
#ifndef ORBX_EMU
        if (h->graph_exec) (void)hipGraphExecDestroy(h->graph_exec);
        if (h->graph) (void)hipGraphDestroy(h->graph);
#endif
        for (int i = 0; i < ORBX_NSTAGES; i++) { rt::event_destroy(h->ev_stage[i][0]); rt::event_destroy(h->ev_stage[i][1]); }
        rt::stream_sync(h->s_copy);
        rt::event_destroy(h->ev_fork); rt::event_destroy(h->ev_join); rt::event_destroy(h->ev_done); rt::event_destroy(h->ev_copy); rt::event_destroy(h->ev_import); rt::event_destroy(h->ev_lp);
        rt::stream_destroy(h->s0); rt::stream_destroy(h->s1); rt::stream_destroy(h->s_copy);
    }
    orbv_forget_handle(h);
    h->d_lv.release(); h->d_cells.release(); h->d_xtab.release(); h->d_ytab.release(); h->d_xspan.release(); h->d_yspan.release(); h->d_pyr.release(); h->d_blur.release(); h->d_stage.release();
    h->d_slots.release(); h->d_candA.release(); h->d_candB.release(); h->d_lvl_keys.release(); h->d_cell_count.release(); h->d_lvl_count.release(); h->d_qtsorted.release();
    h->d_final_idx.release(); h->d_status.p = nullptr; h->d_status.n = 0; h->d_nm.release(); h->d_kps.release(); h->d_desc.release();
    h->d_uRight.release(); h->d_depth.release(); h->d_sad.release(); h->d_nmatch.release(); h->d_knn.release(); h->d_ratio.release();
    h->d_l2r.release(); h->d_r2l.release(); h->d_p3d.release(); h->d_hamA.release(); h->d_hamB.release(); h->d_hamOut.release(); h->h_stage.release(); h->h_nm.release(); h->h_cnt.release();
    for (auto& x : h->d_sr) x.release();
    h->h_packA.release(); h->h_packB.release(); h->h_out.release(); h->h_res.release();
    for (auto& x : h->d_si) x.release();
    h->d_kps_un.release();
    h->d_lp.release(); h->d_depth_in.release(); h->h_lp_in.release(); h->h_lp_out.release();
    h->d_aux.release(); h->d_qtprof.release(); h->d_qtpool.release(); h->d_rowstart.release(); h->d_rowitems.release();
    h->d_mapx.release(); h->d_mapy.release(); h->d_in_xt.release(); h->d_in_yt.release(); h->d_frame.release();
    h->d_exp.release(); for (auto& x : h->h_exp) x.release();
    delete h;
}

int orbx_set_gaussian_taps(orbx_extractor* h, int variant) {
    if (!h || (variant != 0 && variant != 1)) return fail(ORBX_E_ARG, "bad gaussian variant");
    h->gauss_variant = variant; return ORBX_OK;
}
int orbx_reserve(orbx_extractor* h, int width, int height, int max_batch) { if (!h) return fail(ORBX_E_ARG, "null handle"); return configure(h, width, height, max_batch); }
int orbx_get_levels(const orbx_extractor* h) { return h ? h->nlevels : 0; }
float orbx_get_scale_factor(const orbx_extractor* h) { return h ? (float)h->scaleFactor : 0.f; }
int orbx_get_level_tables(const orbx_extractor* h, float* scale, float* inv_scale, float* sigma2, float* inv_sigma2, int* fpl, int* umax16) {
    if (!h) return fail(ORBX_E_ARG, "null handle");
    for (int i = 0; i < h->nlevels; i++) {
        if (scale) scale[i] = h->scale[i];
        if (inv_scale) inv_scale[i] = h->inv_scale[i];
        if (sigma2) sigma2[i] = h->sigma2[i];
        if (inv_sigma2) inv_sigma2[i] = h->inv_sigma2[i];
        if (fpl) fpl[i] = h->quota[i];
    }
    if (umax16) for (int i = 0; i < 16; i++) umax16[i] = h->umax.u[i];
    return ORBX_OK;
}
int orbx_max_keypoints(const orbx_extractor* h) {
    if (!h) return 0;
    if (h->kp_total_cap) return h->kp_total_cap;
    int s = 0; for (int l = 0; l < h->nlevels; l++) s += std::max(h->quota[l] + 3, 16); return s;
}

int orbx_extract_batch(orbx_extractor* h, int B, const uint8_t* images, int width, int height, int stride, size_t image_stride,
                       int on_device, int lap0, int lap1) {
    if (!h) return fail(ORBX_E_ARG, "null handle");
    if (!images || width <= 0 || height <= 0 || B <= 0) return fail(ORBX_E_EMPTY, "empty image");
    const int C = h->in_active ? h->in_channels : 1;
    const size_t row_bytes = (size_t)width * C;
    if ((size_t)stride < row_bytes) return fail(ORBX_E_ARG, "stride < width * channels");
    if (B > 1 && image_stride < (size_t)stride * (height - 1) + row_bytes) return fail(ORBX_E_ARG, "image_stride too small");
    const bool geom = h->in_active && h->in_geometry != 0;
    int rc = configure(h, geom ? h->in_out_w : width, geom ? h->in_out_h : height, B);
    if (rc) return rc;
    rt::set_device(h->device);
    if (h->undist.active && h->d_kps_un.ensure((size_t)h->maxB * h->kp_total_cap)) return fail(ORBX_E_DEVICE, "allocation failed (undistorted keypoints)");
    if (h->in_active) {
        if (h->in_geometry == 2 && (h->in_tap_w != width || h->in_tap_h != height)) {
            std::vector<ResizeTap> xt, yt;
            resize_axis(width, h->in_out_w, true, xt); resize_axis(height, h->in_out_h, false, yt);
            if (h->d_in_xt.ensure(xt.size()) || h->d_in_yt.ensure(yt.size())) return fail(ORBX_E_DEVICE, "allocation failed");
            rt::copy_h2d(h->d_in_xt.p, xt.data(), sizeof(ResizeTap) * xt.size(), h->s0); rt::copy_h2d(h->d_in_yt.p, yt.data(), sizeof(ResizeTap) * yt.size(), h->s0);
            rt::stream_sync(h->s0);
            h->in_tap_w = width; h->in_tap_h = height;
        }
        if (geom && C > 1 && h->d_frame.ensure((size_t)B * h->W * h->H * C + 16)) return fail(ORBX_E_DEVICE, "allocation failed");
    }
    if (h->fetch_pending) return fail(ORBX_E_INTERNAL, "a download of the previous results is still in flight");
    if (h->exp_guard) {
        if (rt::stream_wait_event(h->s0, h->ev_exp_read)) return fail(ORBX_E_DEVICE, "extraction could not be ordered behind the pyramid export: %s", rt::last_error());
        h->exp_guard = false;
    }
    const uint8_t* d_images = images;
    if (!on_device) {
        const size_t bytes = (size_t)(B - 1) * image_stride + (size_t)stride * (height - 1) + row_bytes;
        if (h->d_stage.ensure(bytes + 16)) return fail(ORBX_E_DEVICE, "staging allocation failed");
        if (rt::copy_h2d(h->d_stage.p, images, bytes, h->s0)) return fail(ORBX_E_DEVICE, "H2D copy failed: %s", rt::last_error());
        d_images = h->d_stage.p;
    }
    if (h->copy_pending) {
        if (rt::stream_wait_event(h->s0, h->ev_copy)) return fail(ORBX_E_DEVICE, "extraction could not be ordered behind the input upload: %s", rt::last_error());
        h->copy_pending = false;
    }
#ifndef ORBX_EMU
    if (h->use_graph && !h->profile && !h->in_active) {
        const bool same = h->graph_exec && h->g_B == B && h->g_images == d_images && h->g_stride == stride && h->g_image_stride == image_stride &&
                          h->g_lap0 == lap0 && h->g_lap1 == lap1 && h->g_W == h->W && h->g_H == h->H && h->g_pyr == h->d_pyr.p && h->g_gauss == h->gauss_variant && h->g_undist_gen == h->undist_gen && h->g_pyramid_mode == h->pyramid_mode && h->g_small_forms == h->small_forms && h->g_exp_edge == h->exp_edge;
        if (!same) {
            if (h->graph_exec) { (void)hipGraphExecDestroy(h->graph_exec); h->graph_exec = nullptr; }
            if (h->graph) { (void)hipGraphDestroy(h->graph); h->graph = nullptr; }
            if (hipStreamBeginCapture(h->s0, hipStreamCaptureModeThreadLocal) != hipSuccess) return fail(ORBX_E_DEVICE, "graph capture failed to start");
            rc = enqueue_extract(h, B, d_images, width, height, stride, image_stride, lap0, lap1, true);
            const hipError_t e = hipStreamEndCapture(h->s0, &h->graph);
            if (rc || e != hipSuccess || hipGraphInstantiate(&h->graph_exec, h->graph, nullptr, nullptr, 0) != hipSuccess) {
                h->graph_exec = nullptr;
                return fail(ORBX_E_DEVICE, "graph capture/instantiate failed: %s", rt::last_error());
            }
            h->g_B = B; h->g_images = d_images; h->g_stride = stride; h->g_image_stride = image_stride; h->g_lap0 = lap0; h->g_lap1 = lap1;
            h->g_W = h->W; h->g_H = h->H; h->g_pyr = h->d_pyr.p; h->g_gauss = h->gauss_variant; h->g_undist_gen = h->undist_gen; h->g_pyramid_mode = h->pyramid_mode; h->g_small_forms = h->small_forms; h->g_exp_edge = h->exp_edge;
        }
        if (hipGraphLaunch(h->graph_exec, h->s0) != hipSuccess) return fail(ORBX_E_DEVICE, "graph launch failed: %s", rt::last_error());
        if (h->exp_edge > 0 && (rc = export_enqueue(h, B))) return rc;
        h->import_lazy = true; h->done_lazy = true;
        h->lastB = B; h->extract_gen++; h->ex_undist_gen = h->undist_gen; h->ex_undist_active = h->undist.active != 0;
        return ORBX_OK;
    }
#endif
    return enqueue_extract(h, B, d_images, width, height, stride, image_stride, lap0, lap1, false);
}

int orbx_set_input(orbx_extractor* h, const OrbxInputSpec* spec) {
    if (!h) return fail(ORBX_E_ARG, "null handle");
    if (!spec) { h->in_active = false; return ORBX_OK; }
    if (spec->channels != 1 && spec->channels != 3 && spec->channels != 4) return fail(ORBX_E_ARG, "channels must be 1, 3 or 4");
    if (spec->geometry < 0 || spec->geometry > 2) return fail(ORBX_E_ARG, "unknown geometry");
    if (spec->geometry != 0 && (spec->out_w <= 0 || spec->out_h <= 0)) return fail(ORBX_E_ARG, "output size missing");
    if (spec->geometry == 1 && (!spec->map_x || !spec->map_y)) return fail(ORBX_E_ARG, "rectification maps missing");
    rt::set_device(h->device);
    if (spec->geometry == 1) {
        const size_t n = (size_t)spec->out_w * spec->out_h;
        if (h->d_mapx.ensure(n) || h->d_mapy.ensure(n)) return fail(ORBX_E_DEVICE, "allocation failed");
        if (rt::copy_h2d(h->d_mapx.p, spec->map_x, n * sizeof(float), h->s0) | rt::copy_h2d(h->d_mapy.p, spec->map_y, n * sizeof(float), h->s0) | rt::stream_sync(h->s0))
            return fail(ORBX_E_DEVICE, "map upload failed");
    }
    h->in_channels = spec->channels; h->in_rgb = spec->rgb ? 1 : 0; h->in_gray_variant = spec->gray_variant ? 1 : 0; h->in_geometry = spec->geometry;
    h->in_out_w = spec->out_w; h->in_out_h = spec->out_h; h->in_tap_w = h->in_tap_h = 0;
    h->in_active = true;
    return ORBX_OK;
}

int orbx_sync(orbx_extractor* h) {
    if (!h) return fail(ORBX_E_ARG, "null handle");
    rt::set_device(h->device);
    if (rt::stream_sync(h->s0) || rt::stream_sync(h->s1)) return fail(ORBX_E_DEVICE, "stream sync failed: %s", rt::last_error());
    if (h->copy_pending && rt::stream_sync(h->s_copy)) return fail(ORBX_E_DEVICE, "copy stream sync failed: %s", rt::last_error());
    if (export_drain(h)) return fail(ORBX_E_DEVICE, "export stream sync failed: %s", rt::last_error());
    if (h->profile) for (int i = 0; i < ORBX_NSTAGES; i++) if (i != ST_MATCH) h->stage_ms[i] = rt::event_elapsed_ms(h->ev_stage[i][0], h->ev_stage[i][1]);
    return ORBX_OK;
}

int orbx_fetch(orbx_extractor* h, OrbxKeyPoint* kps, uint8_t* desc, int cap, int* n_out, int* mono_out) {
    if (!h || h->lastB <= 0) return fail(ORBX_E_ARG, "nothing to fetch");
    rt::set_device(h->device);
    const int B = h->lastB; const size_t tc = (size_t)h->kp_total_cap;
    const size_t kb = (size_t)B * tc * sizeof(KeyPointRec), db = (size_t)B * tc * 32;
    const bool direct = (cap == h->kp_total_cap);
    if (!direct && h->h_stage.ensure(kb + db + 64)) return fail(ORBX_E_DEVICE, "pinned allocation failed");
    const int* nm = h->h_nm.p;
    int e = 0;
    if (h->cnt_gen == h->extract_gen) {
        if (rt::event_sync(h->ev_done)) return fail(ORBX_E_DEVICE, "extraction failed: %s", rt::last_error());
        nm = h->h_cnt.p;
        h->fetch_pending = true;
        if (kps) e |= rt::copy_d2h(direct ? (void*)kps : (void*)h->h_stage.p, h->d_kps.p, kb, h->s1);
        if (desc) e |= rt::copy_d2h(direct ? (void*)desc : (void*)(h->h_stage.p + kb), h->d_desc.p, db, h->s1);
        const int se = rt::stream_sync(h->s1);
        h->fetch_pending = se != 0;
        e |= se;
    } else {
        e = rt::copy_d2h(h->h_nm.p, h->d_nm.p, sizeof(int) * (2 * h->maxB + 1), h->s0);
        if (kps) e |= rt::copy_d2h(direct ? (void*)kps : (void*)h->h_stage.p, h->d_kps.p, kb, h->s0);
        if (desc) e |= rt::copy_d2h(direct ? (void*)desc : (void*)(h->h_stage.p + kb), h->d_desc.p, db, h->s0);
        e |= rt::stream_sync(h->s0);
    }
    if (e) return fail(ORBX_E_DEVICE, "D2H failed: %s", rt::last_error());
    if (h->profile) orbx_sync(h);
    if (nm[2 * h->maxB] != 0) return fail(ORBX_E_INTERNAL, "device quadtree capacity check tripped");
    int rc = ORBX_OK;
    for (int b = 0; b < B; b++) {
        const int n = nm[b];
        if (n_out) n_out[b] = n;
        if (mono_out) mono_out[b] = nm[h->maxB + b];
        if (direct) continue;
        if (n > cap) { rc = ORBX_E_CAPACITY; continue; }
        if (kps) memcpy(kps + (size_t)b * cap, h->h_stage.p + (size_t)b * tc * sizeof(KeyPointRec), (size_t)n * sizeof(KeyPointRec));
        if (desc) memcpy(desc + (size_t)b * cap * 32, h->h_stage.p + kb + (size_t)b * tc * 32, (size_t)n * 32);
    }
    if (rc) return fail(rc, "output capacity %d too small", cap);
    return ORBX_OK;
}

int orbx_extract(orbx_extractor* h, const uint8_t* image, int width, int height, int stride, int lap0, int lap1,
                 OrbxKeyPoint* kps, uint8_t* desc, int cap, int* n_out, int* mono_out) {
    if (n_out) *n_out = 0;
    if (mono_out) *mono_out = -1;
    int rc = orbx_extract_batch(h, 1, image, width, height, stride, (size_t)stride * height, 0, lap0, lap1);
    if (rc) return rc;
    return orbx_fetch(h, kps, desc, cap, n_out, mono_out);
}

int orbx_pyramid_level(orbx_extractor* h, int b, int level, int blurred, uint8_t* dst, int dst_stride, int* width, int* height) {
    if (!h || level < 0 || level >= h->nlevels || b < 0 || b >= h->lastB) return fail(ORBX_E_ARG, "bad pyramid query");
    const LevelInfo& L = h->lv[level];
    if (width) *width = L.w;
    if (height) *height = L.h;
    if (!dst) return ORBX_OK;
    if (dst_stride < L.w) return fail(ORBX_E_ARG, "dst_stride < width");
    rt::set_device(h->device);
    const size_t plane = (size_t)L.pitch * L.h;
    if (h->h_stage.ensure(plane + 64)) return fail(ORBX_E_DEVICE, "pinned allocation failed");
    rt::stream_sync(h->s1);
    const uint8_t* src = (blurred ? h->d_blur.p : h->d_pyr.p) + (size_t)b * h->pyr_stride + L.off;
    if (rt::copy_d2h(h->h_stage.p, src, plane, h->s0) || rt::stream_sync(h->s0)) return fail(ORBX_E_DEVICE, "D2H failed");
    for (int y = 0; y < L.h; y++) memcpy(dst + (size_t)y * dst_stride, h->h_stage.p + (size_t)y * L.pitch, L.w);
    return ORBX_OK;
}

int orbx_pyramid_fetch(orbx_extractor* h, int b, int blurred, uint8_t* const* dst, const int* dst_stride) {
    if (!h || !dst || !dst_stride || b < 0 || b >= h->lastB) return fail(ORBX_E_ARG, "bad pyramid query");
    for (int l = 0; l < h->nlevels; l++) if (!dst[l] || dst_stride[l] < h->lv[l].w) return fail(ORBX_E_ARG, "level %d: destination missing or too narrow", l);
    rt::set_device(h->device);
    if (h->h_stage.ensure(h->pyr_stride + 64)) return fail(ORBX_E_DEVICE, "pinned allocation failed");
    rt::stream_sync(h->s1);
    const uint8_t* src = (blurred ? h->d_blur.p : h->d_pyr.p) + (size_t)b * h->pyr_stride;
    if (rt::copy_d2h(h->h_stage.p, src, h->pyr_stride, h->s0) || rt::stream_sync(h->s0)) return fail(ORBX_E_DEVICE, "D2H failed");
    for (int l = 0; l < h->nlevels; l++) {
        const LevelInfo& L = h->lv[l];
        for (int y = 0; y < L.h; y++) memcpy(dst[l] + (size_t)y * dst_stride[l], h->h_stage.p + L.off + (size_t)y * L.pitch, L.w);
    }
    return ORBX_OK;
}

int orbx_set_pyramid_export(orbx_extractor* h, int edge, int depth) {
    if (!h) return fail(ORBX_E_ARG, "null handle");
    if (edge < 0 || edge > kExportMaxEdge || (edge > 0 && (depth < 1 || depth > kExportMaxDepth)))
        return fail(ORBX_E_ARG, "pyramid export: edge 0 (off) .. %d, depth 1 .. %d", kExportMaxEdge, kExportMaxDepth);
    if (edge == h->exp_edge && (edge == 0 || depth == h->exp_depth)) return ORBX_OK;
    rt::set_device(h->device);
    export_release(h);
    if (edge == 0) return ORBX_OK;
    int e = rt::stream_create(&h->s_exp);
    h->have_exp_stream = e == 0;
    e |= rt::event_create(&h->ev_exp_fork) | rt::event_create(&h->ev_exp_read);
    for (int k = 0; k < depth; k++) e |= rt::event_create(&h->ev_exp_slot[k]);
    if (e) { export_release(h); return fail(ORBX_E_DEVICE, "pyramid export: stream/event creation failed"); }
    h->exp_edge = edge; h->exp_depth = depth;
    const int rc = export_prepare(h);
    if (rc) export_release(h);
    return rc;
}

int orbx_pyramid_exported(orbx_extractor* h, int b, const uint8_t** base, size_t* offset, int* step, int* width, int* height) {
    if (!h || h->exp_slot < 0 || b < 0 || b >= h->exp_B || b >= h->lastB)
        return fail(ORBX_E_ARG, "no exported pyramid for image %d of the last extraction (export off, switched on since, or the geometry changed)", b);
    rt::set_device(h->device);
    if (rt::event_sync(h->ev_exp_slot[h->exp_slot])) return fail(ORBX_E_DEVICE, "pyramid export failed: %s", rt::last_error());
    if (base) *base = h->h_exp[h->exp_slot].p + (size_t)b * h->exp_stride;
    for (int l = 0; l < h->nlevels; l++) {
        if (offset) offset[l] = (size_t)h->exp_fl.off[l];
        if (step) step[l] = h->exp_fl.step[l];
        if (width) width[l] = h->lv[l].w;
        if (height) height[l] = h->lv[l].h;
    }
    return ORBX_OK;
}

int orbx_device_alloc(orbx_extractor* h, size_t bytes, void** dptr) {
    if (!h || !dptr) return fail(ORBX_E_ARG, "null");
    rt::set_device(h->device);
    *dptr = rt::dmalloc(bytes);
    return *dptr ? ORBX_OK : fail(ORBX_E_DEVICE, "hipMalloc(%zu) failed", bytes);
}
int orbx_device_free(orbx_extractor* h, void* dptr) { if (!h) return ORBX_E_ARG; rt::set_device(h->device); rt::dfree(dptr); return ORBX_OK; }
int orbx_device_upload(orbx_extractor* h, void* dptr, const void* host, size_t bytes) {
    if (!h || !dptr || !host) return fail(ORBX_E_ARG, "null");
    rt::set_device(h->device);
    if (rt::copy_h2d(dptr, host, bytes, h->s0) || rt::stream_sync(h->s0)) return fail(ORBX_E_DEVICE, "upload failed");
    return ORBX_OK;
}

int orbx_device_upload_async(orbx_extractor* h, void* dptr, const void* host, size_t bytes) {
    if (!h || !dptr || !host) return fail(ORBX_E_ARG, "null");
    rt::set_device(h->device);
    record_import_if_pending(h);
    if (h->lastB > 0 && rt::stream_wait_event(h->s_copy, h->ev_import)) return fail(ORBX_E_DEVICE, "upload could not be ordered behind the previous extraction: %s", rt::last_error());
    if (h->exp_pending && rt::stream_wait_event(h->s_copy, h->ev_exp_read)) return fail(ORBX_E_DEVICE, "upload could not be ordered behind the pyramid export: %s", rt::last_error());
    if (rt::copy_h2d(dptr, host, bytes, h->s_copy) || rt::event_record(h->ev_copy, h->s_copy)) return fail(ORBX_E_DEVICE, "upload failed: %s", rt::last_error());
    h->copy_pending = true;
    return ORBX_OK;
}

int orbx_debug_quadtree_profile(orbx_extractor* h, long long out[16]) {
    if (!h || !out || !h->d_qtprof.p) return ORBX_E_ARG;
    rt::set_device(h->device);
    if (rt::copy_d2h(out, h->d_qtprof.p, sizeof(long long) * 16, h->s0) || rt::stream_sync(h->s0)) return ORBX_E_DEVICE;
    return ORBX_OK;
}

int orbx_debug_simd_selftest(orbx_extractor* h, const uint32_t* a, const uint32_t* b, const uint32_t* c, int n, uint32_t* out) {
    if (!h || !a || !b || !c || !out || n <= 0 || (n & 255)) return fail(ORBX_E_ARG, "bad arguments (n must be a positive multiple of 256)");
    rt::set_device(h->device);
    orbx::DevBuf<uint32_t> d;
    const size_t N = (size_t)n;
    if (d.ensure((3 + kSimdSelftestOps) * N)) return fail(ORBX_E_DEVICE, "allocation failed");
    int e = rt::copy_h2d(d.p, a, 4 * N, h->s0) | rt::copy_h2d(d.p + N, b, 4 * N, h->s0) | rt::copy_h2d(d.p + 2 * N, c, 4 * N, h->s0);
    dim3 grid((n + 255) / 256, 1, 1), blk(256, 1, 1);
    ORBX_LAUNCH(k_simd_selftest, grid, blk, 0, h->s0, (const uint32_t*)d.p, (const uint32_t*)(d.p + N), (const uint32_t*)(d.p + 2 * N), n, d.p + 3 * N);
    e |= rt::copy_d2h(out, d.p + 3 * N, 4 * N * kSimdSelftestOps, h->s0);
    if (e || rt::stream_sync(h->s0) || rt::check_launch()) { d.release(); return fail(ORBX_E_DEVICE, "self-test failed: %s", rt::last_error()); }
    d.release();
    return ORBX_OK;
}

int orbx_debug_model_eval(orbx_extractor* h, int op, uint32_t start_bits, const float* a, const float* b, int n, float* out) {
    if (!h || !out || n <= 0 || n > kModelSelftestMax || op < 0 || op >= kModelSelftestOps) return fail(ORBX_E_ARG, "bad arguments (op 0 .. %d, 1 .. %d elements)", kModelSelftestOps - 1, kModelSelftestMax);
    if (op >= 5 && (!a || !b)) return fail(ORBX_E_ARG, "op %d takes two operand arrays", op);
    rt::set_device(h->device);
    orbx::DevBuf<float> d;
    const size_t N = (size_t)n, nout = op == 7 ? 3 * N : N, off_a = nout, off_b = nout + (a ? N : 0);
    if (d.ensure(off_b + (b ? N : 0))) return fail(ORBX_E_DEVICE, "allocation failed");
    int e = 0;
    if (a) e |= rt::copy_h2d(d.p + off_a, a, 4 * N, h->s0);
    if (b) e |= rt::copy_h2d(d.p + off_b, b, 4 * N, h->s0);
    dim3 grid((n + 255) / 256, 1, 1), blk(256, 1, 1);
    ORBX_LAUNCH(k_model_selftest, grid, blk, 0, h->s0, op, start_bits, a ? (const float*)(d.p + off_a) : (const float*)nullptr,
                b ? (const float*)(d.p + off_b) : (const float*)nullptr, n, d.p);
    e |= rt::copy_d2h(out, d.p, 4 * nout, h->s0);
    if (e || rt::stream_sync(h->s0) || rt::check_launch()) { d.release(); return fail(ORBX_E_DEVICE, "model self-test failed: %s", rt::last_error()); }
    d.release();
    return ORBX_OK;
}

int orbx_debug_quadtree_selftest(orbx_extractor* h, int op, int spill, int threads, const void* in, int n, int start, int total, int mx, int my, void* out) {
    if (!h || !in || !out || (threads != 256 && threads != 1024) || (spill != 0 && spill != 1)) return fail(ORBX_E_ARG, "bad arguments (256 or 1024 threads, spill 0 or 1)");
    size_t in_bytes = 0, out_bytes = 0, pool_bytes = 0, smem = 0;
    if (op == ORBX_QT_SELFTEST_SORT) {
        const int nmax = spill ? 65535 : 4095;
        if (n < 0 || n > nmax) return fail(ORBX_E_ARG, "the %s form sorts at most %d keys", spill ? "pool" : "LDS", nmax);
        in_bytes = out_bytes = (size_t)n * 8;
        (spill ? pool_bytes : smem) = quadtree_selftest_sort_bytes(n, spill != 0);
    } else if (op == ORBX_QT_SELFTEST_PARTITION4) {
        if (n < 1 || start < 1 || total > (1 << 24) || (long long)start + n > (long long)total) return fail(ORBX_E_ARG, "the span [start, start + n) must lie inside [1, total)");
        in_bytes = (size_t)total * 4; out_bytes = in_bytes + 16;
    } else if (op == ORBX_QT_SELFTEST_SCAN) {
        if (n != threads) return fail(ORBX_E_ARG, "the scan takes one value per thread");
        in_bytes = (size_t)n * 8; out_bytes = in_bytes + 8;
    } else return fail(ORBX_E_ARG, "no such self-test %d", op);
    rt::set_device(h->device);
    if (smem + 2048 > rt::lds_limit(h->device)) return fail(ORBX_E_CAPACITY, "%d keys need %zu bytes of LDS, the device allows %zu", n, smem + 2048, rt::lds_limit(h->device));
    orbx::DevBuf<uint8_t> d;
    const size_t off_out = align_up(in_bytes + 8, 256), off_pool = off_out + align_up(out_bytes + 8, 256);
    if (d.ensure(off_pool + pool_bytes + 256)) return fail(ORBX_E_DEVICE, "allocation failed");
    int e = in_bytes ? rt::copy_h2d(d.p, in, in_bytes, h->s0) : 0;
    if (op == ORBX_QT_SELFTEST_PARTITION4) e |= rt::copy_h2d(d.p + off_out, out, in_bytes, h->s0);
    ORBX_LAUNCH(k_quadtree_selftest, dim3(1, 1, 1), dim3(threads, 1, 1), smem, h->s0, op, spill, (const void*)d.p, (void*)(d.p + off_out), d.p + off_pool, n, start, total, mx, my);
    if (out_bytes) e |= rt::copy_d2h(out, d.p + off_out, out_bytes, h->s0);
    if (e || rt::stream_sync(h->s0) || rt::check_launch()) { d.release(); return fail(ORBX_E_DEVICE, "self-test failed: %s", rt::last_error()); }
    d.release();
    return ORBX_OK;
}

int orbx_debug_live_resources(long long out[4]) {
    if (!out) return fail(ORBX_E_ARG, "null out");
    const rt::Live& l = rt::live();
    out[0] = l.dev.load(); out[1] = l.pinned.load(); out[2] = l.streams.load(); out[3] = l.events.load();
    return ORBX_OK;
}

int orbx_host_alloc(orbx_extractor* h, size_t bytes, void** hptr) {
    if (!h || !hptr) return fail(ORBX_E_ARG, "null");
    rt::set_device(h->device);
    *hptr = rt::hmalloc(bytes);
    return *hptr ? ORBX_OK : fail(ORBX_E_DEVICE, "pinned host allocation of %zu bytes failed", bytes);
}
int orbx_host_free(orbx_extractor* h, void* hptr) { if (!h) return ORBX_E_ARG; rt::set_device(h->device); rt::hfree(hptr); return ORBX_OK; }

int orbx_debug_stereo_flags(orbx_extractor* h, int flags) { if (!h) return ORBX_E_ARG; h->debug_stereo_flags = flags; return ORBX_OK; }

int orbx_device_outputs(orbx_extractor* h, void** kps, void** desc, void** n, void** mono, int* cap, int* B) {
    if (!h || h->lastB <= 0) return fail(ORBX_E_ARG, "nothing extracted yet");
    if (kps) *kps = h->d_kps.p;
    if (desc) *desc = h->d_desc.p;
    if (n) *n = h->d_nm.p;
    if (mono) *mono = h->d_nm.p + h->maxB;
    if (cap) *cap = h->kp_total_cap;
    if (B) *B = h->lastB;
    return ORBX_OK;
}

int orbx_set_undistort(orbx_extractor* h, const float K[4], const float* dist, int ndist, int opencv_variant) {
    if (!h) return fail(ORBX_E_ARG, "null handle");
    h->undist_gen++;
    memset(&h->undist, 0, sizeof h->undist);
    if (!K || !dist || ndist <= 0 || dist[0] == 0.0f) return ORBX_OK;
    if (ndist != 4 && ndist != 5) return fail(ORBX_E_ARG, "distortion coefficients: k1, k2, p1, p2[, k3]");
    if (opencv_variant != 0 && opencv_variant != 1) return fail(ORBX_E_ARG, "bad OpenCV variant");
    UndistortParams& U = h->undist;
    U.fx = K[0]; U.fy = K[1]; U.cx = K[2]; U.cy = K[3]; U.ifx = 1. / U.fx; U.ify = 1. / U.fy;
    for (int i = 0; i < ndist; i++) U.k[i] = dist[i];
    U.variant = opencv_variant; U.active = 1;
    return ORBX_OK;
}
int orbx_fetch_undistorted(orbx_extractor* h, OrbxKeyPoint* kps_un, int cap) {
    if (!h || !kps_un || h->lastB <= 0) return fail(ORBX_E_ARG, "nothing to fetch");
    if (cap < h->kp_total_cap) return fail(ORBX_E_CAPACITY, "rows need %d entries", h->kp_total_cap);
    rt::set_device(h->device);
    const size_t tc = (size_t)h->kp_total_cap;
    if (undistort_stale(h)) return fail(ORBX_E_ARG, "orbx_set_undistort was called after the last extraction: mvKeysUn of that batch belongs to the previous model - extract again");
    const KeyPointRec* src = h->ex_undist_active ? h->d_kps_un.p : h->d_kps.p;
    int e = 0;
    if ((size_t)cap == tc) e = rt::copy_d2h(kps_un, src, (size_t)h->lastB * tc * sizeof(KeyPointRec), h->s0);
    else for (int b = 0; b < h->lastB; b++) e |= rt::copy_d2h(kps_un + (size_t)b * cap, src + (size_t)b * tc, tc * sizeof(KeyPointRec), h->s0);
    if (e || rt::stream_sync(h->s0)) return fail(ORBX_E_DEVICE, "D2H failed: %s", rt::last_error());
    return ORBX_OK;
}
int orbx_undistorted_bounds(const orbx_extractor* h, int width, int height, float out[4]) {
    if (!h || !out) return fail(ORBX_E_ARG, "null");
    if (!h->undist.active) { out[0] = 0.0f; out[1] = (float)width; out[2] = 0.0f; out[3] = (float)height; return ORBX_OK; }
    float x[4], y[4];
    const float cu[4] = {0.0f, (float)width, 0.0f, (float)width}, cv[4] = {0.0f, 0.0f, (float)height, (float)height};
    for (int i = 0; i < 4; i++) undistort_point(h->undist, cu[i], cv[i], &x[i], &y[i]);
    out[0] = std::min(x[0], x[2]); out[1] = std::max(x[1], x[3]); out[2] = std::min(y[0], y[1]); out[3] = std::max(y[2], y[3]);
    return ORBX_OK;
}

int orbx_input_buffer(orbx_extractor* h, int width, int height, int B, void** dptr, int* stride, size_t* image_stride) {
    if (!h || !dptr) return fail(ORBX_E_ARG, "null");
    if (h->in_active && (h->in_channels != 1 || h->in_geometry != 0)) return fail(ORBX_E_ARG, "zero-copy input needs plain 8-bit grey frames (an input pre-step is set)");
    const int rc = configure(h, width, height, B); if (rc) return rc;
    if (h->exp_pending && rt::event_sync(h->ev_exp_read)) return fail(ORBX_E_DEVICE, "pyramid export failed: %s", rt::last_error());
    *dptr = h->d_pyr.p + h->lv[0].off;
    if (stride) *stride = h->lv[0].pitch;
    if (image_stride) *image_stride = h->pyr_stride;
    return ORBX_OK;
}
int orbx_input_upload(orbx_extractor* h, int B, const uint8_t* images, int width, int height, int stride, size_t image_stride) {
    void* d = nullptr; int pitch = 0; size_t istr = 0;
    if (!images || stride < width) return fail(ORBX_E_ARG, "bad input images");
    int rc = orbx_input_buffer(h, width, height, B, &d, &pitch, &istr); if (rc) return rc;
    rt::set_device(h->device);
    int e = 0;
    for (int b = 0; b < B; b++) e |= rt::copy2d((uint8_t*)d + (size_t)b * istr, (size_t)pitch, images + (size_t)b * image_stride, (size_t)stride, (size_t)width, (size_t)height, 0, h->s0);
    if (e || rt::stream_sync(h->s0)) return fail(ORBX_E_DEVICE, "input upload failed: %s", rt::last_error());
    return ORBX_OK;
}

int orbx_device_snapshot(orbx_extractor* h, void* desc_dst, void* n_dst) {
    if (!h || h->lastB <= 0) return fail(ORBX_E_ARG, "nothing extracted yet");
    rt::set_device(h->device);
    int e = 0;
    if (desc_dst) e |= rt::copy_d2d(desc_dst, h->d_desc.p, (size_t)h->lastB * h->kp_total_cap * 32, h->s0);
    if (n_dst) e |= rt::copy_d2d(n_dst, h->d_nm.p, sizeof(int) * (size_t)h->lastB, h->s0);
    if (e || rt::stream_sync(h->s0)) return fail(ORBX_E_DEVICE, "snapshot failed: %s", rt::last_error());
    return ORBX_OK;
}
int orbx_device_id(const orbx_extractor* h) { return h ? (rt::memory_is_host() ? ORBX_DEVICE_HOST : h->device) : ORBX_E_ARG; }

int orbx_set_pyramid_mode(orbx_extractor* h, int mode) {
    if (!h || mode < 0 || mode > 2) return fail(ORBX_E_ARG, "pyramid mode 0 (by batch size), 1 (one launch per level) or 2 (one launch)");
    h->pyramid_mode = mode;
    return ORBX_OK;
}

int orbx_set_small_batch_forms(orbx_extractor* h, int on) { if (!h) return ORBX_E_ARG; h->small_forms = on != 0; return ORBX_OK; }
int orbx_set_host_wait(int device_id, int mode) {
    if (mode < 0 || mode > 3) return fail(ORBX_E_ARG, "host wait mode %d (0 default, 1 blocking, 2 spin, 3 yield)", mode);
    if (device_id < 0 || device_id >= rt::device_count()) return fail(ORBX_E_DEVICE, "no usable GPU %d", device_id);
    if (rt::set_host_wait(device_id, mode)) return fail(ORBX_E_DEVICE, "hipSetDeviceFlags failed: %s", rt::last_error());
    return ORBX_OK;
}
int orbx_debug_quadtree_pool_levels(orbx_extractor* h) { return h ? h->qt_pool_levels : ORBX_E_ARG; }
int orbx_debug_quadtree_lds_nodes(orbx_extractor* h, int max_nodes) {
    if (!h || max_nodes < 0) return ORBX_E_ARG;
    h->qt_lds_nodes = std::min(max_nodes, kQuadtreeLdsNodes);
    h->g_B = 0;
    return ORBX_OK;
}

int orbx_debug_quadtree_eager(orbx_extractor* h, int on) {
    if (!h) return ORBX_E_ARG;
    h->qt_eager = on != 0;
    h->g_B = 0;
    return ORBX_OK;
}
int orbx_debug_quadtree_sorted(orbx_extractor* h, int b, int* per_level) {
    if (!h || !per_level || b < 0 || b >= h->lastB || !h->d_qtsorted.p) return fail(ORBX_E_ARG, "bad probe");
    rt::set_device(h->device);
    if (rt::stream_sync(h->s0) || rt::copy_d2h(per_level, h->d_qtsorted.p + (size_t)b * h->nlevels, sizeof(int) * h->nlevels, h->s0) || rt::stream_sync(h->s0))
        return fail(ORBX_E_DEVICE, "probe failed: %s", rt::last_error());
    return ORBX_OK;
}

int orbx_set_graph_replay(orbx_extractor* h, int on) { if (!h) return ORBX_E_ARG; h->use_graph = on != 0; return ORBX_OK; }

int orbx_profile_enable(orbx_extractor* h, int on) { if (!h) return ORBX_E_ARG; h->profile = on != 0; h->serial = on == 2; return ORBX_OK; }
int orbx_profile_get(orbx_extractor* h, float ms[ORBX_NSTAGES]) {
    if (!h || !ms) return ORBX_E_ARG;
    for (int i = 0; i < ORBX_NSTAGES; i++) ms[i] = h->stage_ms[i];
    return ORBX_OK;
}

int orbx_debug_candidates(orbx_extractor* h, int b, int level, int* xys, int cap) {
    if (!h || (!xys && cap > 0) || level < 0 || level >= h->nlevels || b < 0 || b >= h->lastB) return fail(ORBX_E_ARG, "bad probe");
    rt::set_device(h->device);
    rt::stream_sync(h->s0);
    const LevelInfo& L = h->lv[level];
    std::vector<int> counts(L.cell_count);
    rt::copy_d2h(counts.data(), h->d_cell_count.p + (size_t)b * h->ncells + L.cell_begin, sizeof(int) * L.cell_count, h->s0);
    std::vector<uint32_t> slots(L.cand_cap + 1);
    rt::copy_d2h(slots.data(), h->d_slots.p + (size_t)b * h->cand_stride + L.cand_off, sizeof(uint32_t) * L.cand_cap, h->s0);
    rt::stream_sync(h->s0);
    int n = 0;
    for (int c = 0; c < L.cell_count; c++) {
        const int so = h->cells[L.cell_begin + c].slot_off - L.cand_off;
        for (int k = 0; k < counts[c]; k++) {
            if (n < cap) { const uint32_t key = slots[so + k]; xys[3 * n] = key_x(key); xys[3 * n + 1] = key_y(key); xys[3 * n + 2] = key_s(key); }
            n++;
        }
    }
    return n;
}
int orbx_debug_level_keys(orbx_extractor* h, int b, int level, int* xys, int cap) {
    if (!h || (!xys && cap > 0) || level < 0 || level >= h->nlevels || b < 0 || b >= h->lastB) return fail(ORBX_E_ARG, "bad probe");
    rt::set_device(h->device);
    rt::stream_sync(h->s0);
    const LevelInfo& L = h->lv[level];
    int cnt = 0;
    rt::copy_d2h(&cnt, h->d_lvl_count.p + (size_t)b * h->nlevels + level, sizeof(int), h->s0);
    std::vector<uint32_t> keys(L.kp_cap);
    rt::copy_d2h(keys.data(), h->d_lvl_keys.p + (size_t)b * h->kp_total_cap + L.kp_off, sizeof(uint32_t) * L.kp_cap, h->s0);
    rt::stream_sync(h->s0);
    for (int i = 0; i < cnt && i < cap; i++) { xys[3 * i] = key_x(keys[i]); xys[3 * i + 1] = key_y(keys[i]); xys[3 * i + 2] = key_s(keys[i]); }
    return cnt;
}

int orbm_hamming_matrix(orbx_extractor* h, const uint8_t* a, int na, const uint8_t* b, int nb, int* out) {
    if (!h || !a || !b || !out || na <= 0 || nb <= 0) return fail(ORBX_E_ARG, "bad hamming arguments");
    rt::set_device(h->device);
    if (h->d_hamA.ensure((size_t)na * 4) || h->d_hamB.ensure((size_t)nb * 4) || h->d_hamOut.ensure((size_t)na * nb)) return fail(ORBX_E_DEVICE, "allocation failed");
    const size_t ba = (size_t)na * 32, bb = (size_t)nb * 32;
    if (h->h_packA.ensure(ba + bb + 16)) return fail(ORBX_E_DEVICE, "allocation failed");
    memcpy(h->h_packA.p, a, ba); memcpy(h->h_packA.p + ba, b, bb);
    rt::copy_h2d(h->d_hamA.p, h->h_packA.p, ba, h->s0);
    rt::copy_h2d(h->d_hamB.p, h->h_packA.p + ba, bb, h->s0);
    dim3 grid((nb + 255) / 256, na, 1), blk(256, 1, 1);
    ORBX_LAUNCH(k_hamming_matrix, grid, blk, 0, h->s0, (const unsigned long long*)h->d_hamA.p, na, (const unsigned long long*)h->d_hamB.p, nb, h->d_hamOut.p);
    if (fetch_sync(h, out, h->d_hamOut.p, sizeof(int) * (size_t)na * nb)) return fail(ORBX_E_DEVICE, "hamming failed: %s", rt::last_error());
    return ORBX_OK;
}

static int check_pair(orbx_extractor* L, int lf, orbx_extractor* R, int rf, int B) {
    if (!L || !R || B <= 0 || lf < 0 || rf < 0) return fail(ORBX_E_ARG, "bad matcher arguments");
    if (lf + B > L->lastB || rf + B > R->lastB) return fail(ORBX_E_ARG, "matcher range exceeds the last extracted batch");
    if (L->W != R->W || L->H != R->H || L->nlevels != R->nlevels || L->kp_total_cap != R->kp_total_cap || L->device != R->device)
        return fail(ORBX_E_ARG, "left/right extractors differ in geometry, parameters or device");
    return ORBX_OK;
}

int orbm_stereo_match(orbx_extractor* L, int lf, orbx_extractor* R, int rf, int B, float bf, float bl) {
    int rc = check_pair(L, lf, R, rf, B); if (rc) return rc;
    rt::set_device(L->device);
    if (L != R) { record_done_if_pending(R); rt::stream_wait_event(L->s0, R->ev_done); }
    const int cap = L->kp_total_cap;
    StereoParams P; P.mbf = bf; P.mb = bl; P.th_high = 100; P.th_orb = (100 + 50) / 2;
    P.debug_flags = L->debug_stereo_flags;
    if (L->profile) rt::event_record(L->ev_stage[ST_MATCH][0], L->s0);
    dim3 grid((cap + 3) / 4, B, 1), blk(256, 1, 1);
    const int nb = (R->H >> kStereoRowShift) + 2;
    const int lookback = (int)std::ceil(4.0f * R->scale[R->nlevels - 1]) + 2;
    ORBX_LAUNCH(k_stereo_match, grid, blk, 0, L->s0, (const LevelInfo*)L->d_lv.p,
                (const KeyPointRec*)(L->d_kps.p + (size_t)lf * cap), (const unsigned long long*)(L->d_desc.p + (size_t)lf * cap * 4), (const int*)(L->d_nm.p + lf),
                (const KeyPointRec*)(R->d_kps.p + (size_t)rf * cap), (const unsigned long long*)(R->d_desc.p + (size_t)rf * cap * 4),
                (const int4*)(R->d_aux.p + (size_t)rf * cap * 4), (const int*)(R->d_nm.p + rf),
                (const int*)(R->d_rowstart.p + (size_t)rf * (nb + 1)), (const int*)(R->d_rowitems.p + (size_t)rf * cap), nb, lookback, cap, (const uint8_t*)(L->d_pyr.p + (size_t)lf * L->pyr_stride), (const uint8_t*)(R->d_pyr.p + (size_t)rf * R->pyr_stride), L->pyr_stride,
                P, L->d_uRight.p, L->d_depth.p, L->d_sad.p);
    dim3 grid2(B, 1, 1);
    ORBX_LAUNCH(k_stereo_median, grid2, blk, 0, L->s0, (const int*)(L->d_nm.p + lf), cap, L->d_uRight.p, L->d_depth.p,
                (const int*)L->d_sad.p, L->d_nmatch.p);
    if (L->profile) rt::event_record(L->ev_stage[ST_MATCH][1], L->s0);
    L->ur_B = 0;
    if (rt::check_launch()) return fail(ORBX_E_DEVICE, "kernel launch failed: %s", rt::last_error());
    L->ur_first = lf; L->ur_B = B; L->ur_gen = L->extract_gen;
    return ORBX_OK;
}

int orbm_stereo_fetch(orbx_extractor* L, int B, float* uRight, float* depth, int cap, int* n_matches) {
    if (!L || B <= 0 || B > L->maxB) return fail(ORBX_E_ARG, "bad fetch");
    rt::set_device(L->device);
    const size_t tc = (size_t)L->kp_total_cap;
    const bool direct = ((size_t)cap == tc);
    if (!direct && L->h_stage.ensure(2 * B * tc * sizeof(float) + 64)) return fail(ORBX_E_DEVICE, "pinned allocation failed");
    float* hu = direct ? uRight : (float*)L->h_stage.p; float* hd = direct ? depth : hu + B * tc;
    int e = 0;
    if (hu) e |= rt::copy_d2h(hu, L->d_uRight.p, B * tc * sizeof(float), L->s0);
    if (hd) e |= rt::copy_d2h(hd, L->d_depth.p, B * tc * sizeof(float), L->s0);
    e |= rt::copy_d2h(L->h_nm.p, L->d_nmatch.p, sizeof(int) * B, L->s0);
    if (e || rt::stream_sync(L->s0)) return fail(ORBX_E_DEVICE, "D2H failed: %s", rt::last_error());
    if (L->profile) L->stage_ms[ST_MATCH] = rt::event_elapsed_ms(L->ev_stage[ST_MATCH][0], L->ev_stage[ST_MATCH][1]);
    const size_t ncopy = std::min<size_t>(tc, (size_t)cap);
    for (int b = 0; b < B; b++) {
        if (!direct && uRight) memcpy(uRight + (size_t)b * cap, hu + b * tc, ncopy * sizeof(float));
        if (!direct && depth) memcpy(depth + (size_t)b * cap, hd + b * tc, ncopy * sizeof(float));
        if (n_matches) n_matches[b] = L->h_nm.p[b];
    }
    return ORBX_OK;
}

int orbm_knn2(orbx_extractor* L, int lf, orbx_extractor* R, int rf, int B) {
    int rc = check_pair(L, lf, R, rf, B); if (rc) return rc;
    rt::set_device(L->device);
    if (L != R) { record_done_if_pending(R); rt::stream_wait_event(L->s0, R->ev_done); }
    const int cap = L->kp_total_cap; const size_t bc = (size_t)L->maxB * cap;
    if (L->profile) rt::event_record(L->ev_stage[ST_MATCH][0], L->s0);
    const dim3 blk(256, 1, 1);
    const int* qoff = L->d_nm.p + L->maxB + lf; const int* nq = L->d_nm.p + lf;
    const int* toff = R->d_nm.p + R->maxB + rf; const int* nt = R->d_nm.p + rf;
    if (L->debug_stereo_flags & 8) {
        dim3 grid((cap + 3) / 4, B, 1);
        ORBX_LAUNCH(k_knn2, grid, blk, 0, L->s0,
                    (const unsigned long long*)(L->d_desc.p + (size_t)lf * cap * 4), qoff, nq,
                    (const unsigned long long*)(R->d_desc.p + (size_t)rf * cap * 4), toff, nt,
                    cap, L->d_knn.p, L->d_knn.p + bc, L->d_knn.p + 2 * bc, L->d_knn.p + 3 * bc, L->d_ratio.p);
    } else {
        dim3 grid((cap + 31) / 32, B, 1);
        ORBX_LAUNCH(k_knn2_mfma, grid, blk, 0, L->s0,
                    (const unsigned long long*)(L->d_desc.p + (size_t)lf * cap * 4), qoff, nq,
                    (const unsigned long long*)(R->d_desc.p + (size_t)rf * cap * 4), toff, nt,
                    cap, L->d_knn.p, L->d_knn.p + bc, L->d_knn.p + 2 * bc, L->d_knn.p + 3 * bc, L->d_ratio.p);
    }
    if (L->profile) rt::event_record(L->ev_stage[ST_MATCH][1], L->s0);
    if (rt::check_launch()) return fail(ORBX_E_DEVICE, "kernel launch failed: %s", rt::last_error());
    return ORBX_OK;
}

int orbm_stereo_fisheye(orbx_extractor* L, int lf, orbx_extractor* R, int rf, int B, const OrbmKB8Stereo* S) {
    if (L) L->fe_B = 0;
    if (!S) return fail(ORBX_E_ARG, "null camera parameters");
    int rc = orbm_knn2(L, lf, R, rf, B); if (rc) return rc;
    const int cap = L->kp_total_cap; const size_t bc = (size_t)L->maxB * cap;
    if (L->d_l2r.ensure(bc) || L->d_r2l.ensure(bc) || L->d_p3d.ensure(3 * bc)) return fail(ORBX_E_DEVICE, "allocation failed");
    KB8StereoParams P; memset(&P, 0, sizeof P);
    for (int i = 0; i < 8; i++) { P.cam1[i] = S->cam1[i]; P.cam2[i] = S->cam2[i]; }
    for (int i = 0; i < 9; i++) P.R12[i] = S->R12[i];
    for (int i = 0; i < 3; i++) P.t12[i] = S->t12[i];
    for (int l = 0; l < L->nlevels; l++) P.sigma2[l] = L->sigma2[l];
    rt::memset_async(L->d_r2l.p, 0xFF, sizeof(int) * (size_t)B * cap, L->s0);
    rt::memset_async(L->d_nmatch.p, 0, sizeof(int) * (size_t)B, L->s0);
    dim3 grid((cap + 255) / 256, B, 1), blk(256, 1, 1);
    ORBX_LAUNCH(k_kb8_stereo, grid, blk, 0, L->s0, (const KeyPointRec*)(L->d_kps.p + (size_t)lf * cap), (const int*)(L->d_nm.p + L->maxB + lf), (const int*)(L->d_nm.p + lf),
                (const KeyPointRec*)(R->d_kps.p + (size_t)rf * cap), (const int*)(R->d_nm.p + R->maxB + rf), cap, (const int*)L->d_knn.p, (const uint8_t*)L->d_ratio.p, P,
                L->d_l2r.p, L->d_r2l.p, L->d_depth.p, L->d_p3d.p, L->d_nmatch.p);
    if (L->profile) rt::event_record(L->ev_stage[ST_MATCH][1], L->s0);
    if (rt::check_launch()) return fail(ORBX_E_DEVICE, "kernel launch failed: %s", rt::last_error());
    L->fe_R = R; L->fe_lf = lf; L->fe_rf = rf; L->fe_B = B; L->fe_gen_L = L->extract_gen; L->fe_gen_R = R->extract_gen;
    return ORBX_OK;
}

int orbm_stereo_fisheye_fetch(orbx_extractor* L, int B, int* l2r, int* r2l, float* depth, float* p3d, int* n_matches, int cap) {
    if (!L || B <= 0 || B > L->maxB || !L->d_l2r.p) return fail(ORBX_E_ARG, "bad fetch");
    rt::set_device(L->device);
    const size_t tc = (size_t)L->kp_total_cap, n = (size_t)B * tc;
    if (L->h_stage.ensure(n * (2 * sizeof(int) + 4 * sizeof(float)) + 64)) return fail(ORBX_E_DEVICE, "pinned allocation failed");
    int* hl = (int*)L->h_stage.p; int* hr = hl + n; float* hd = (float*)(hr + n); float* hp = hd + n;
    int e = rt::copy_d2h(hl, L->d_l2r.p, n * sizeof(int), L->s0) | rt::copy_d2h(hr, L->d_r2l.p, n * sizeof(int), L->s0) |
            rt::copy_d2h(hd, L->d_depth.p, n * sizeof(float), L->s0) | rt::copy_d2h(hp, L->d_p3d.p, 3 * n * sizeof(float), L->s0) |
            rt::copy_d2h(L->h_nm.p, L->d_nmatch.p, sizeof(int) * B, L->s0);
    if (e || rt::stream_sync(L->s0)) return fail(ORBX_E_DEVICE, "D2H failed: %s", rt::last_error());
    if (L->profile) L->stage_ms[ST_MATCH] = rt::event_elapsed_ms(L->ev_stage[ST_MATCH][0], L->ev_stage[ST_MATCH][1]);
    const size_t ncopy = std::min<size_t>(tc, (size_t)cap);
    for (int b = 0; b < B; b++) {
        if (l2r) memcpy(l2r + (size_t)b * cap, hl + b * tc, ncopy * sizeof(int));
        if (r2l) memcpy(r2l + (size_t)b * cap, hr + b * tc, ncopy * sizeof(int));
        if (depth) memcpy(depth + (size_t)b * cap, hd + b * tc, ncopy * sizeof(float));
        if (p3d) memcpy(p3d + 3 * (size_t)b * cap, hp + 3 * b * tc, 3 * ncopy * sizeof(float));
        if (n_matches) n_matches[b] = L->h_nm.p[b];
    }
    return ORBX_OK;
}

int orbm_knn2_fetch(orbx_extractor* L, int B, int* idx0, int* dist0, int* idx1, int* dist1, uint8_t* ratio_ok, int cap) {
    if (!L || B <= 0 || B > L->maxB) return fail(ORBX_E_ARG, "bad fetch");
    rt::set_device(L->device);
    const size_t tc = (size_t)L->kp_total_cap, bc = (size_t)L->maxB * tc;
    if (L->h_stage.ensure(4 * B * tc * sizeof(int) + B * tc + 64)) return fail(ORBX_E_DEVICE, "pinned allocation failed");
    int* hk = (int*)L->h_stage.p; uint8_t* hr = L->h_stage.p + 4 * B * tc * sizeof(int);
    int e = 0;
    for (int k = 0; k < 4; k++) e |= rt::copy_d2h(hk + k * B * tc, L->d_knn.p + k * bc, B * tc * sizeof(int), L->s0);
    e |= rt::copy_d2h(hr, L->d_ratio.p, B * tc, L->s0);
    if (e || rt::stream_sync(L->s0)) return fail(ORBX_E_DEVICE, "D2H failed: %s", rt::last_error());
    if (L->profile) L->stage_ms[ST_MATCH] = rt::event_elapsed_ms(L->ev_stage[ST_MATCH][0], L->ev_stage[ST_MATCH][1]);
    const size_t ncopy = std::min<size_t>(tc, (size_t)cap);
    int* outs[4] = {idx0, dist0, idx1, dist1};
    for (int b = 0; b < B; b++) {
        for (int k = 0; k < 4; k++) if (outs[k]) memcpy(outs[k] + (size_t)b * cap, hk + k * B * tc + b * tc, ncopy * sizeof(int));
        if (ratio_ok) memcpy(ratio_ok + (size_t)b * cap, hr + b * tc, ncopy);
    }
    return ORBX_OK;
}

}
```

orb_slam3_detailed_comments_amd/csrc/orbx_internal.h:

```cpp
#pragma once
#include <algorithm>
#include <cmath>
#include <cstdarg>
#include <cstdint>
#include <cstring>
#include <mutex>
#include <string>
#include <vector>
#include "../../include/orbx.h"
#include "orbx_kernels.h"
#include "orbx_rt.h"

namespace orbx {

int fail(int code, const char* fmt, ...);

inline int round_half_even_f(float v) { return (int)lrintf(v); }
inline int round_half_even_d(double v) { return (int)lrint(v); }
inline size_t align_up(size_t v, size_t a) { return (v + a - 1) / a * a; }

constexpr int kExportMaxDepth = 8, kExportMaxEdge = 256;

enum Stage { ST_IMPORT = 0, ST_PYRAMID, ST_FAST, ST_QUADTREE, ST_BLUR, ST_LAYOUT, ST_DESCRIBE, ST_MATCH };

template <typename T> struct DevBuf {
    T* p = nullptr; size_t n = 0;
    int ensure(size_t count) {
        if (count <= n && p) return 0;
        rt::dfree(p); p = (T*)rt::dmalloc(count * sizeof(T)); n = p ? count : 0;
        return p ? 0 : -1;
    }
    void release() { rt::dfree(p); p = nullptr; n = 0; }
};
template <typename T> struct HostBuf {
    T* p = nullptr; size_t n = 0;
    int ensure(size_t count) {
        if (count <= n && p) return 0;
        rt::hfree(p); p = (T*)rt::hmalloc(count * sizeof(T)); n = p ? count : 0;
        return p ? 0 : -1;
    }
    void release() { rt::hfree(p); p = nullptr; n = 0; }
};

struct VocFrameArrays {
    const uint32_t* fv_node; const int* fv_start; const int* fv_feat; const int* nout; int cap, lastB, device, first; const void* handle; uint64_t extract_gen;
    int rig, first_r; const void* handle_r; uint64_t extract_gen_r; const unsigned long long* desc;
};
}
struct orbv_vocabulary;
struct orbx_extractor;
namespace orbx {
int orbv_frame_arrays(const orbv_vocabulary* v, VocFrameArrays* out);
std::unique_lock<std::mutex> orbv_lock(const orbv_vocabulary* v);
void orbv_forget_handle(const orbx_extractor* h);

struct PendingBatch {
    int B = 0, M = 0;
    std::vector<int> M_b;
    size_t o_result = 0, o_view[2] = {0, 0};
    bool want_view = false, rig = false;
    int m(size_t b) const { return M_b.empty() ? M : M_b[b]; }
};
}

struct orbx_extractor {
    int nfeatures = 0, nlevels = 0, iniTh = 0, minTh = 0, device = 0, gauss_variant = 0;
    double scaleFactor = 1.0;
    float scale[orbx::kMaxLevels], inv_scale[orbx::kMaxLevels], sigma2[orbx::kMaxLevels], inv_sigma2[orbx::kMaxLevels];
    int quota[orbx::kMaxLevels];
    orbx::UmaxTab umax;
    int W = 0, H = 0, maxB = 0;
    orbx::LevelInfo lv[orbx::kMaxLevels];
    std::vector<orbx::CellInfo> cells;
    std::vector<orbx::ResizeTap> xtab, ytab;
    bool resize_rows_ok[orbx::kMaxLevels] = {};
    std::vector<orbx::PyrSpan> xspan, yspan;
    int pyr_ntx = 0, pyr_nty = 0, pyr_buf_a = 0, pyr_buf_b = 0;
    orbx::PyrTapOffsets pyr_toff = {};
    bool pyr_fused_ok = false;
    bool small_forms = true, g_small_forms = true;
    int pyramid_mode = 0, g_pyramid_mode = 0;
    size_t pyr_stride = 0, cand_stride = 0;
    int ncells = 0, kp_total_cap = 0, node_cap = 0, nb_cap = 1, fast_tile_bytes = 0, fast_inner_bytes = 0;
    orbx::DevBuf<orbx::LevelInfo> d_lv; orbx::DevBuf<orbx::CellInfo> d_cells; orbx::DevBuf<orbx::ResizeTap> d_xtab, d_ytab;
    orbx::DevBuf<orbx::PyrSpan> d_xspan, d_yspan;
    orbx::DevBuf<uint8_t> d_pyr, d_blur, d_stage;
    orbx::DevBuf<uint32_t> d_slots, d_candA, d_candB, d_lvl_keys;
    orbx::DevBuf<int> d_cell_count, d_lvl_count, d_final_idx, d_nm, d_status;
    orbx::DevBuf<orbx::KeyPointRec> d_kps; orbx::DevBuf<unsigned long long> d_desc;
    orbx::DevBuf<float> d_uRight, d_depth; orbx::DevBuf<int> d_sad, d_nmatch;
    int ur_first = 0, ur_B = 0; uint64_t ur_gen = 0;
    orbx::DevBuf<int> d_knn; orbx::DevBuf<uint8_t> d_ratio;
    orbx::DevBuf<int> d_l2r, d_r2l; orbx::DevBuf<float> d_p3d;
    orbx::DevBuf<unsigned long long> d_hamA, d_hamB; orbx::DevBuf<int> d_hamOut;
    orbx::HostBuf<uint8_t> h_stage;
    orbx::HostBuf<int> h_nm;
    orbx::rt::stream_t s0 = 0, s1 = 0, s_copy = 0;
    orbx::rt::event_t ev_fork = 0, ev_join = 0, ev_done = 0, ev_copy = 0, ev_import = 0;
    bool copy_pending = false;
    bool done_lazy = false, import_lazy = false;
    bool fetch_pending = false;
    orbx::HostBuf<int> h_cnt; uint64_t cnt_gen = 0;
    orbx::rt::event_t ev_stage[ORBX_NSTAGES][2] = {};
    bool profile = false, serial = false, have_streams = false;
    int lastB = 0;
    uint64_t extract_gen = 0;
    int debug_stereo_flags = 0;
    float stage_ms[ORBX_NSTAGES];
    orbx::DevBuf<uint8_t> d_sr[12];
    orbx::HostBuf<uint8_t> h_packA, h_packB, h_out;
    orbx::HostBuf<uint8_t> h_res;
    size_t area_pool = 0, area_last_total = 0;
    orbx::DevBuf<int> d_si[8];
    orbx::DevBuf<long long> d_qtprof;
    orbx::DevBuf<int> d_qtsorted; int qt_eager = 0;
    orbx::DevBuf<uint8_t> d_qtpool; int qt_lds_nodes = orbx::kQuadtreeLdsNodes, cfg_qt_lds_nodes = 0, qt_pool_levels = 0;
    bool use_graph = false;
#ifndef ORBX_EMU
    hipGraph_t graph = nullptr; hipGraphExec_t graph_exec = nullptr;
#endif
    int g_B = 0, g_stride = 0, g_lap0 = 0, g_lap1 = 0, g_W = 0, g_H = 0, g_gauss = 0; size_t g_image_stride = 0;
    const void* g_images = nullptr; const void* g_pyr = nullptr;
    bool in_active = false; int in_channels = 1, in_rgb = 1, in_gray_variant = 0, in_geometry = 0, in_out_w = 0, in_out_h = 0, in_tap_w = 0, in_tap_h = 0;
    orbx::DevBuf<float> d_mapx, d_mapy; orbx::DevBuf<orbx::ResizeTap> d_in_xt, d_in_yt; orbx::DevBuf<uint8_t> d_frame;
    orbx::DevBuf<int> d_rowstart, d_rowitems;
    orbx::DevBuf<uint8_t> d_lp, d_depth_in; orbx::HostBuf<uint8_t> h_lp_in, h_lp_out;
    size_t lp_pool = 0; bool lp_pending = false;
    orbx::PendingBatch batch;
    const orbx_extractor* fe_R = nullptr; int fe_lf = 0, fe_rf = 0, fe_B = 0; uint64_t fe_gen_L = 0, fe_gen_R = 0;
    orbx::rt::event_t ev_lp = 0;
    orbx::UndistortParams undist = {}; int undist_gen = 0, g_undist_gen = 0; orbx::DevBuf<orbx::KeyPointRec> d_kps_un;
    int ex_undist_gen = 0; bool ex_undist_active = false;
    orbx::DevBuf<int> d_aux;
    int exp_edge = 0, exp_depth = 0, exp_slot = -1, exp_B = 0, g_exp_edge = 0;
    uint64_t exp_count = 0;
    size_t exp_stride = 0, exp_cap = 0;
    orbx::FrameLayout exp_fl = {};
    orbx::rt::stream_t s_exp = 0;
    orbx::rt::event_t ev_exp_fork = 0, ev_exp_read = 0, ev_exp_slot[orbx::kExportMaxDepth] = {};
    bool have_exp_stream = false;
    bool exp_pending = false, exp_guard = false;
    orbx::DevBuf<uint8_t> d_exp; orbx::HostBuf<uint8_t> h_exp[orbx::kExportMaxDepth];
};
inline void record_done_if_pending(orbx_extractor* h) { if (h->done_lazy) { orbx::rt::event_record(h->ev_done, h->s0); h->done_lazy = false; } }
inline void record_import_if_pending(orbx_extractor* h) { if (h->import_lazy) { orbx::rt::event_record(h->ev_import, h->s0); h->import_lazy = false; } }
inline int fetch_sync(orbx_extractor* h, void* dst, const void* dev_src, size_t bytes) {
    if (bytes == 0) return orbx::rt::stream_sync(h->s0);
    if (orbx::rt::memory_is_host()) { if (orbx::rt::stream_sync(h->s0)) return -1; memcpy(dst, dev_src, bytes); return 0; }
    if (h->h_res.ensure(bytes + 64)) return -1;
    if (orbx::rt::copy_d2h(h->h_res.p, dev_src, bytes, h->s0) || orbx::rt::stream_sync(h->s0)) return -1;
    memcpy(dst, h->h_res.p, bytes);
    return 0;
}
inline bool undistort_stale(const orbx_extractor* h) { return h->lastB > 0 && h->ex_undist_gen != h->undist_gen; }
```

orb_slam3_detailed_comments_amd/csrc/orbx_kernels.h:

```cpp
#pragma once
#include "orbx_types.h"
#include "undistort_model.h"

namespace orbx {

__global__ void k_import(const LevelInfo* __restrict__ lv, const uint8_t* __restrict__ images, int stride,
                         size_t image_stride, uint8_t* __restrict__ pyr, size_t pyr_stride);
__global__ void k_resize(const LevelInfo* __restrict__ lv, int level, const ResizeTap* __restrict__ xtab,
                         const ResizeTap* __restrict__ ytab, uint8_t* __restrict__ pyr, size_t pyr_stride,
                         int lds_pitch, int lds_rows);
__global__ void k_resize_rows(const LevelInfo* __restrict__ lv, int level, const ResizeTap* __restrict__ xtab,
                              const ResizeTap* __restrict__ ytab, uint8_t* __restrict__ pyr, size_t pyr_stride, int strip_rows);
#ifndef ORBX_PYR_THREADS
#define ORBX_PYR_THREADS 512
#endif
#ifndef ORBX_PYR_TILE
#define ORBX_PYR_TILE 16
#endif
constexpr int kPyrTile = ORBX_PYR_TILE;
constexpr int kPyrThreads = ORBX_PYR_THREADS;
__global__ void k_pyramid_fused(const LevelInfo* __restrict__ lv, int nlevels, const ResizeTap* __restrict__ xtab, const ResizeTap* __restrict__ ytab,
                                const PyrSpan* __restrict__ xspan, const PyrSpan* __restrict__ yspan, int ntx, uint8_t* __restrict__ pyr, size_t pyr_stride,
                                int buf_a_bytes, int buf_b_bytes, PyrTapOffsets toff);
#ifndef ORBX_FAST_XCD_RUN
#define ORBX_FAST_XCD_RUN 4
#endif
constexpr int kFastXcdRun = ORBX_FAST_XCD_RUN;
constexpr int kFastThreadsDecl = 64;
constexpr int kFastPitch = 48;
__global__ void k_fast_cells(const LevelInfo* __restrict__ lv, const CellInfo* __restrict__ cells, int ncells,
                             const uint8_t* __restrict__ pyr, size_t pyr_stride, int iniTh, int minTh,
                             uint32_t* __restrict__ slots, size_t slots_stride, int* __restrict__ cell_count,
                             int tile_bytes, int list_bytes, int* __restrict__ status);
constexpr int kFrameRows = 8;
__global__ void k_frame_pyramid(const LevelInfo* __restrict__ lv, int nlevels, const uint8_t* __restrict__ pyr, size_t pyr_stride,
                                uint8_t* __restrict__ out, size_t out_stride, FrameLayout fl);
constexpr int kResizeRows = 8;
#ifndef ORBX_BLUR_ROWS
#define ORBX_BLUR_ROWS 16
#endif
#ifndef ORBX_BLUR_ROWS_LARGE
#define ORBX_BLUR_ROWS_LARGE 32
#endif
constexpr int kBlurRows = ORBX_BLUR_ROWS, kBlurRowsLarge = ORBX_BLUR_ROWS_LARGE;
constexpr int kSimdSelftestOps = 22;
__global__ void k_simd_selftest(const uint32_t* __restrict__ a, const uint32_t* __restrict__ b, const uint32_t* __restrict__ c, int n, uint32_t* __restrict__ out);
constexpr int kModelSelftestOps = 8, kModelSelftestMax = 1 << 26;
__global__ void k_model_selftest(int op, uint32_t start_bits, const float* __restrict__ a, const float* __restrict__ b, int n, float* __restrict__ out);
__global__ void k_blur(const LevelInfo* __restrict__ lv, int nlevels, const uint8_t* __restrict__ pyr,
                       uint8_t* __restrict__ blur, size_t pyr_stride, BlurTaps taps, BlurTiles tiles);
__global__ void k_blur_large(const LevelInfo* __restrict__ lv, int nlevels, const uint8_t* __restrict__ pyr,
                             uint8_t* __restrict__ blur, size_t pyr_stride, BlurTaps taps, BlurTiles tiles);
constexpr int kQuadtreeThreads = 1024;
__global__ void k_fast_cells_blur(const LevelInfo* __restrict__ lv, const CellInfo* __restrict__ cells, int ncells,
                                  const uint8_t* __restrict__ pyr, size_t pyr_stride, int iniTh, int minTh,
                                  uint32_t* __restrict__ slots, size_t slots_stride, int* __restrict__ cell_count,
                                  int tile_bytes, int list_bytes, int* __restrict__ status,
                                  int nlevels, uint8_t* __restrict__ blur, BlurTaps taps, BlurTiles tiles, int blur_waves);
__global__ void k_quadtree(const LevelInfo* __restrict__ lv, const CellInfo* __restrict__ cells, int ncells,
                           const int* __restrict__ cell_count, const uint32_t* __restrict__ slots, size_t slots_stride,
                           uint32_t* __restrict__ candA, uint32_t* __restrict__ candB, size_t cand_stride,
                           uint32_t* __restrict__ lvl_keys, int kp_total_cap, int* __restrict__ lvl_count,
                           int nlevels, int node_cap, int nb_cap, int lut_x, int lut_y, int* __restrict__ status, long long* __restrict__ qt_prof,
                           int wide, int counter_bytes, int level0, int* __restrict__ qt_sorted, int eager);
__global__ void k_quadtree_spill(const LevelInfo* __restrict__ lv, const CellInfo* __restrict__ cells, int ncells,
                           const int* __restrict__ cell_count, const uint32_t* __restrict__ slots, size_t slots_stride,
                           uint32_t* __restrict__ candA, uint32_t* __restrict__ candB, size_t cand_stride,
                           uint32_t* __restrict__ lvl_keys, int kp_total_cap, int* __restrict__ lvl_count,
                           int nlevels, int node_cap, int nb_cap, int lut_x, int lut_y, int* __restrict__ status, long long* __restrict__ qt_prof,
                           int wide, int counter_bytes, unsigned char* __restrict__ pool, size_t pool_stride, int* __restrict__ qt_sorted, int eager);
constexpr int kQuadtreeLdsNodes = 4000;
ORBX_HD constexpr int quadtree_selftest_seg_cap(int n) { return (n / 8 + 8 + 1) & ~1; }
ORBX_HD constexpr size_t quadtree_selftest_sort_bytes(int n, bool spill) { return (size_t)quadtree_selftest_seg_cap(n) * 2 * (spill ? 8 : 4) + (size_t)n * 17 + 16; }
__global__ void k_quadtree_selftest(int op, int spill, const void* __restrict__ in, void* __restrict__ out, unsigned char* __restrict__ pool,
                                    int n, int s, int total, int mx, int my);
__global__ void k_layout(const LevelInfo* __restrict__ lv, int nlevels, const uint32_t* __restrict__ lvl_keys,
                         int kp_total_cap, const int* __restrict__ lvl_count, int lap0, int lap1,
                         int* __restrict__ final_idx, int* __restrict__ n_out, int* __restrict__ mono_out,
                         int nb, int* __restrict__ row_start, int* __restrict__ row_items);
#ifndef ORBX_STEREO_ROW_SHIFT
#define ORBX_STEREO_ROW_SHIFT 3
#endif
constexpr int kStereoRowShift = ORBX_STEREO_ROW_SHIFT;
constexpr int kKpPerWaveDecl = 8;
constexpr int kKpPerWaveSmallDecl = 2;
__global__ void k_orient_brief(const LevelInfo* __restrict__ lv, int nlevels, const uint8_t* __restrict__ pyr,
                               const uint8_t* __restrict__ blur, size_t pyr_stride,
                               const uint32_t* __restrict__ lvl_keys, int kp_total_cap,
                               const int* __restrict__ lvl_count, const int* __restrict__ final_idx, UmaxTab umax,
                               KeyPointRec* __restrict__ out_kps, unsigned long long* __restrict__ out_desc, int4* __restrict__ out_aux,
                               int B, int groups_per_image);
__global__ void k_orient_brief_small(const LevelInfo* __restrict__ lv, int nlevels, const uint8_t* __restrict__ pyr,
                               const uint8_t* __restrict__ blur, size_t pyr_stride,
                               const uint32_t* __restrict__ lvl_keys, int kp_total_cap,
                               const int* __restrict__ lvl_count, const int* __restrict__ final_idx, UmaxTab umax,
                               KeyPointRec* __restrict__ out_kps, unsigned long long* __restrict__ out_desc, int4* __restrict__ out_aux,
                               int B, int groups_per_image);
__global__ void k_undistort(const KeyPointRec* __restrict__ kps, const int* __restrict__ n_per_frame, int cap, UndistortParams U, KeyPointRec* __restrict__ kps_un);
__global__ void k_hamming_matrix(const unsigned long long* __restrict__ A, int na,
                                 const unsigned long long* __restrict__ Bm, int nb, int* __restrict__ out);
__global__ void k_stereo_match(const LevelInfo* __restrict__ lv, const KeyPointRec* __restrict__ kpsL,
                               const unsigned long long* __restrict__ descL, const int* __restrict__ nL,
                               const KeyPointRec* __restrict__ kpsR, const unsigned long long* __restrict__ descR,
                               const int4* __restrict__ auxR, const int* __restrict__ nR, const int* __restrict__ bucket_start,
                               const int* __restrict__ bucket_items, int nb, int lookback, int cap, const uint8_t* __restrict__ pyrL,
                               const uint8_t* __restrict__ pyrR, size_t pyr_stride, StereoParams P,
                               float* __restrict__ uRight, float* __restrict__ depth, int* __restrict__ sad);
__global__ void k_stereo_median(const int* __restrict__ nL, int cap, float* __restrict__ uRight,
                                float* __restrict__ depth, const int* __restrict__ sad, int* __restrict__ n_matches);
__global__ void k_kb8_stereo(const KeyPointRec* __restrict__ kpsL, const int* __restrict__ monoL, const int* __restrict__ nL,
                             const KeyPointRec* __restrict__ kpsR, const int* __restrict__ monoR, int cap, const int* __restrict__ idx0,
                             const uint8_t* __restrict__ ratio_ok, KB8StereoParams P, int* __restrict__ l2r, int* __restrict__ r2l,
                             float* __restrict__ depth, float* __restrict__ p3d, int* __restrict__ nmatches);
__global__ void k_knn2_mfma(const unsigned long long* __restrict__ descQ, const int* __restrict__ qoff, const int* __restrict__ nq,
                            const unsigned long long* __restrict__ descT, const int* __restrict__ toff, const int* __restrict__ nt, int cap,
                            int* __restrict__ idx0, int* __restrict__ dist0, int* __restrict__ idx1, int* __restrict__ dist1, uint8_t* __restrict__ ratio_ok);
__global__ void k_knn2(const unsigned long long* __restrict__ descQ, const int* __restrict__ qoff, const int* __restrict__ nq,
                       const unsigned long long* __restrict__ descT, const int* __restrict__ toff, const int* __restrict__ nt,
                       int cap, int* __restrict__ idx0, int* __restrict__ dist0, int* __restrict__ idx1,
                       int* __restrict__ dist1, uint8_t* __restrict__ ratio_ok);

constexpr int kGridThreads = 1024;
constexpr int kGridCellStride = 64 * 48 + 2;
__global__ void k_grid_build(const KeyPointRec* __restrict__ kps, int N, GridParams g, int* __restrict__ cell_of,
                             int* __restrict__ cell_start, int* __restrict__ cell_items, const int* __restrict__ n_per_frame, int frame_stride);
__global__ void k_grid_build_kfs(const GridBuildRec* __restrict__ recs);
__global__ void k_fuse_candidates(const FuseTargetRec* __restrict__ T, int M, const float* __restrict__ pos, const float* __restrict__ normal, const float* __restrict__ min_d,
                                  const float* __restrict__ max_d, const unsigned long long* __restrict__ qdesc, const uint8_t* __restrict__ skip, float th, int chi2_gate,
                                  int th_low, int debug_flags, int* __restrict__ best_idx, int* __restrict__ best_dist);
__global__ void k_sim3_candidates(const Sim3TargetRec* __restrict__ T, int M, const float* __restrict__ pos, const float* __restrict__ normal, const float* __restrict__ min_d,
                                  const float* __restrict__ max_d, const unsigned long long* __restrict__ qdesc, const uint8_t* __restrict__ occupied,
                                  const uint8_t* __restrict__ skip, float th, float max_dist, int debug_flags, int* __restrict__ choice);
__global__ void k_sim3_accept(const Sim3TargetRec* __restrict__ T, int M, const float* __restrict__ pos, const float* __restrict__ normal, const float* __restrict__ min_d,
                              const float* __restrict__ max_d, const unsigned long long* __restrict__ qdesc, const uint8_t* __restrict__ occupied, float th, float max_dist,
                              int debug_flags, int cap, const int* __restrict__ choice, int* __restrict__ assigned, int* __restrict__ nmatches);
constexpr int kAreaWaves = 16;
__global__ void k_area_search(const AreaQuery* __restrict__ queries, const unsigned long long* __restrict__ qdesc, int Q,
                              const KeyPointRec* __restrict__ kps, const float* __restrict__ u_right,
                              const unsigned long long* __restrict__ fdesc, GridParams g, const int* __restrict__ cell_start,
                              const int* __restrict__ cell_items, int gate_right, int* __restrict__ pool_counter, int pool_cap,
                              int* __restrict__ q_start, int* __restrict__ q_count, int2* __restrict__ entries);
__global__ void k_frustum(FrustumParams F, int M, const float* __restrict__ pos, const float* __restrict__ normal, const float* __restrict__ min_dist,
                          const float* __restrict__ max_dist, const uint8_t* __restrict__ is_bad, uint8_t* __restrict__ in_view, float* __restrict__ track,
                          int* __restrict__ scale_level, AreaQuery* __restrict__ queries, int* __restrict__ zero4);
__global__ void k_frustum_batch(const FrustumParams* __restrict__ Fb, const FrameMapRec* __restrict__ maps, const uint8_t* __restrict__ is_bad, uint8_t* __restrict__ in_view,
                                float* __restrict__ track, int* __restrict__ scale_level, AreaQuery* __restrict__ queries, int* __restrict__ zero4);
__global__ void k_project_points(ProjectParams P, int M, const float* __restrict__ pos, const float* __restrict__ normal, const float* __restrict__ min_inv,
                                 const float* __restrict__ max_inv, const uint8_t* __restrict__ skip, uint8_t* __restrict__ valid, float* __restrict__ out, int debug_flags);
__global__ void k_area_search_threads(const AreaQuery* __restrict__ queries, const FrameMapRec* __restrict__ maps, const KeyPointRec* __restrict__ kps,
                                      const float* __restrict__ u_right, const unsigned long long* __restrict__ fdesc, GridParams g,
                                      const int* __restrict__ cell_start, const int* __restrict__ cell_items, int gate_right, int* __restrict__ pool_counter,
                                      int pool_cap, int* __restrict__ q_start, int* __restrict__ q_count, int2* __restrict__ entries, int frame_stride);
__global__ void k_lastframe_queries(const FrustumParams* __restrict__ Fb, int capL, const int* __restrict__ n_last, const float* __restrict__ pos,
                                    const uint8_t* __restrict__ valid, const int* __restrict__ octave, AreaQuery* __restrict__ queries, int* __restrict__ zero4);
__global__ void k_keyframe_queries(const FrustumParams* __restrict__ Fb, int capL, const int* __restrict__ n_kf, const float* __restrict__ pos,
                                   const uint8_t* __restrict__ valid, const float* __restrict__ min_dist, const float* __restrict__ max_dist,
                                   AreaQuery* __restrict__ queries, int* __restrict__ zero4);
__global__ void k_lastframe_accept(const FrameMapRec* __restrict__ maps, int cap, const int* __restrict__ n_per_frame, const int* __restrict__ q_start,
                                   const int* __restrict__ q_count, const int2* __restrict__ entries, const uint8_t* __restrict__ occupied0,
                                   const uint8_t* __restrict__ has_obs, int th_high, int* __restrict__ assigned, int* __restrict__ nmatches,
                                   const float* __restrict__ last_angle, const KeyPointRec* __restrict__ cur_kps, int check_ori);
__global__ void k_local_accept(const FrameMapRec* __restrict__ maps, int cap, const int* __restrict__ n_per_frame, const int* __restrict__ q_start,
                               const int* __restrict__ q_count, const int2* __restrict__ entries, const uint8_t* __restrict__ occupied0,
                               const uint8_t* __restrict__ has_obs, float nnratio, int th_high, int* __restrict__ assigned, int* __restrict__ nmatches);
__global__ void k_frustum_rig(const FrustumParams* __restrict__ Fb, const FrameMapRec* __restrict__ maps, const uint8_t* __restrict__ is_bad, uint8_t* in_view1,
                              uint8_t* in_view2, float* track1, float* track2, int* level1, int* level2, AreaQuery* __restrict__ q1, AreaQuery* __restrict__ q2,
                              int* __restrict__ zero4);
__global__ void k_lastframe_queries_rig(const FrustumParams* __restrict__ Fb, int capL, const int* __restrict__ n_last, const float* __restrict__ pos,
                                        const uint8_t* __restrict__ valid, const int* __restrict__ octave, RigRelPose trl, AreaQuery* q1,
                                        AreaQuery* __restrict__ q2, int* __restrict__ zero4);
__global__ void k_rig_local_accept(const FrameMapRec* __restrict__ maps, int cap, const int* __restrict__ n1, const int* __restrict__ n2, const int* __restrict__ qs1,
                                   const int* __restrict__ qc1, const int* __restrict__ qs2, const int* __restrict__ qc2, const int2* __restrict__ entries,
                                   const uint8_t* __restrict__ occupied0, const uint8_t* __restrict__ has_obs, const int* __restrict__ l2r,
                                   const int* __restrict__ r2l, float nnratio, int th_high, int* __restrict__ assigned, int* __restrict__ nmatches);
__global__ void k_rig_lastframe_accept(const FrameMapRec* __restrict__ maps, int cap, const int* __restrict__ n1, const int* __restrict__ n2, const int* __restrict__ qs1,
                                       const int* __restrict__ qc1, const int* __restrict__ qs2, const int* __restrict__ qc2, const int2* __restrict__ entries,
                                       const uint8_t* __restrict__ occupied0, const uint8_t* __restrict__ has_obs, int th_high, int* __restrict__ assigned,
                                       int* __restrict__ nmatches, const float* __restrict__ last_angle, const KeyPointRec* __restrict__ kps1,
                                       const KeyPointRec* __restrict__ kps2, int check_ori);
__global__ void k_stereo_from_depth(const KeyPointRec* __restrict__ kps, const KeyPointRec* __restrict__ kps_un, const int* __restrict__ n_per_frame, int cap,
                                    const float* __restrict__ depth, int stride, size_t image_stride, int w, int h, float mbf, float* __restrict__ u_right,
                                    float* __restrict__ depth_out, int* __restrict__ n_valid);
__global__ void k_bow_search(const BowItem* __restrict__ items, int nitems, const KeyPointRec* __restrict__ kps1,
                             const unsigned long long* __restrict__ desc1, const float* __restrict__ ur1,
                             const KeyPointRec* __restrict__ kps2, const unsigned long long* __restrict__ desc2,
                             const float* __restrict__ ur2, const uint8_t* __restrict__ has_mp2, const int* __restrict__ feat2,
                             const BowParams* __restrict__ Ps, int* __restrict__ best2);
__global__ void k_bow_search_kb8(const BowItem* __restrict__ items, int nitems, const KeyPointRec* __restrict__ kps1,
                             const unsigned long long* __restrict__ desc1, const float* __restrict__ ur1,
                             const KeyPointRec* __restrict__ kps2, const unsigned long long* __restrict__ desc2,
                             const float* __restrict__ ur2, const uint8_t* __restrict__ has_mp2, const int* __restrict__ feat2,
                             const BowParams* __restrict__ Ps, int* __restrict__ best2);
__global__ void k_sft_resident(ResidentKF k1, const uint8_t* __restrict__ flags, const SftNeighbour* __restrict__ nb, int* __restrict__ best);
__global__ void k_keyframe_counts(const KfSnapRec* __restrict__ recs, int n, int* __restrict__ out);
__global__ void k_keyframe_snapshot(const KfSnapRec* __restrict__ recs);
__global__ void k_sft_resident_kb8(ResidentKF k1, const uint8_t* __restrict__ flags, const SftNeighbour* __restrict__ nb, int* __restrict__ best);
__global__ void k_bow_match_resident(const BowPairResident* __restrict__ pairs, const uint8_t* __restrict__ flags, float nnratio, int th_low,
                                     int th_inclusive, int* __restrict__ m12, int N1cap, int* __restrict__ status);
__global__ void k_bow_rotation_prune(const BowPairResident* __restrict__ pairs, int* __restrict__ m12, int N1cap, int check_ori, int* __restrict__ nmatches);
__global__ void k_bow_match_rig(const BowPairRig* __restrict__ pairs, const uint8_t* __restrict__ flags, float nnratio, int th_low,
                                int* __restrict__ assigned, int S, int* __restrict__ status);
__global__ void k_bow_rotation_prune_rig(const BowPairRig* __restrict__ pairs, int* __restrict__ assigned, int S, int check_ori, int* __restrict__ nmatches);
__global__ void k_bow_dists(const BowItem* __restrict__ items, int nitems, const unsigned long long* __restrict__ desc1,
                            const unsigned long long* __restrict__ desc2, const uint8_t* __restrict__ eligible2,
                            const int* __restrict__ feat2, int* __restrict__ out);
__global__ void k_map_scatter(int n, const int* __restrict__ slots, const unsigned long long* __restrict__ desc, const float* __restrict__ pos,
                              const float* __restrict__ normal, const float* __restrict__ min_d, const float* __restrict__ max_d, const uint8_t* __restrict__ bad,
                              MapStore S);
__global__ void k_map_seen(const int* __restrict__ seen_start, const int* __restrict__ seen_slots, unsigned* __restrict__ seen_stamp, int nslots, unsigned mark);
__global__ void k_map_stamp(const MapSeg* __restrict__ segs, const int* __restrict__ kf_slots, int row_cap, const uint8_t* __restrict__ state,
                            unsigned* __restrict__ stamp, int nslots, unsigned top);
__global__ void k_map_compact(const MapSeg* __restrict__ segs, const int* __restrict__ kf_slots, int row_cap, const uint8_t* __restrict__ state,
                              const unsigned* __restrict__ stamp, int nslots, unsigned top, int* __restrict__ chunk_cnt, const int* __restrict__ chunk_off,
                              const MapSetRec* __restrict__ sets);
__global__ void k_map_scan(const int* __restrict__ frame_chunk0, const int* __restrict__ chunk_cnt, int* __restrict__ chunk_off, int* __restrict__ M_out);
__global__ void k_map_gather(const MapSetRec* __restrict__ sets, MapStore S, const unsigned* __restrict__ seen_stamp, int nslots, unsigned base);
__global__ void k_map_rows_gather(MapStore S, int cap, const int* __restrict__ n, const int* __restrict__ slots, const MapRowRec* __restrict__ rows,
                                  const uint8_t* __restrict__ excluded, uint8_t* __restrict__ valid, float* __restrict__ pos, unsigned long long* __restrict__ desc,
                                  float* __restrict__ min_d, float* __restrict__ max_d, float* __restrict__ angle);
__global__ void k_map_row_flags(const int* __restrict__ kf_slots, int row_cap, const uint8_t* __restrict__ state, const MapRowFlagRec* __restrict__ recs,
                                uint8_t* __restrict__ flags);

__global__ void k_distinctive(const unsigned long long* __restrict__ desc, const int* __restrict__ start, int P, int* __restrict__ best);
template <bool kLds>
__global__ void k_distinctive_resident(const DistinctiveRec* __restrict__ recs, int first, int count,
                                       const unsigned long long* const* __restrict__ kf_desc, const int* __restrict__ obs_kf, const int* __restrict__ obs_feat,
                                       int* __restrict__ best, unsigned long long* __restrict__ best_desc);
__global__ void k_voc_descend(const unsigned long long* __restrict__ fdesc, const int* __restrict__ n_feat, int n_fixed, int cap, int B,
                              const unsigned long long* __restrict__ slot_desc, const VocSlot* __restrict__ slots,
                              const double* __restrict__ slot_weight, int root_children, int nid_level, unsigned* __restrict__ out_word,
                              unsigned* __restrict__ out_node, double* __restrict__ out_weight);
__global__ void k_voc_gather_rig(const unsigned long long* __restrict__ desc_l, const int* __restrict__ n_l, const unsigned long long* __restrict__ desc_r,
                                 const int* __restrict__ n_r, int cap, int B, unsigned long long* __restrict__ out, int* __restrict__ n_out);
__global__ void k_voc_assemble(const unsigned* __restrict__ word, const unsigned* __restrict__ node, const double* __restrict__ weight,
                               const int* __restrict__ n_feat, int n_fixed, int cap, int P, int weighting, int norm,
                               unsigned* __restrict__ bow_id, double* __restrict__ bow_val, int* __restrict__ bow_start,
                               unsigned* __restrict__ fv_node, int* __restrict__ fv_start, unsigned* __restrict__ fv_feat,
                               int* __restrict__ n_out);
__global__ void k_kfdb_count(const unsigned* __restrict__ ids, const long long* __restrict__ rstart, const int* __restrict__ rn,
                             const int* __restrict__ rmult, int R, KfdbQuerySet qs, int* __restrict__ cnt, int* __restrict__ firstpos);
__global__ void k_kfdb_order(int* __restrict__ cnt, const int* __restrict__ firstpos, const unsigned long long* __restrict__ rkey, int R,
                             const int* __restrict__ qn, int qn_step, const int* __restrict__ xstart, const int* __restrict__ xrec, int score_all,
                             int* __restrict__ order, KfdbHit* __restrict__ hits, int* __restrict__ slist, int* __restrict__ head);
__global__ void k_kfdb_score(const unsigned* __restrict__ ids, const double* __restrict__ vals, const long long* __restrict__ rstart,
                             const int* __restrict__ rn, KfdbQuerySet qs, const int* __restrict__ order, const int* __restrict__ slist,
                             const int* __restrict__ head, KfdbHit* __restrict__ hits, int R, int scoring);

__global__ void k_input_remap(const uint8_t* __restrict__ src, int sw, int sh, int sstride, size_t simg, int C, const float* __restrict__ mapx,
                              const float* __restrict__ mapy, int out_w, int out_h, uint8_t* __restrict__ dst, int dst_pitch, size_t dst_stride);
__global__ void k_input_resize(const uint8_t* __restrict__ src, int sw, int sh, int sstride, size_t simg, int C, const ResizeTap* __restrict__ xt,
                               const ResizeTap* __restrict__ yt, int out_w, int out_h, uint8_t* __restrict__ dst, int dst_pitch, size_t dst_stride);
__global__ void k_input_gray(const uint8_t* __restrict__ src, int sstride, size_t simg, int C, int ridx, int ry, int gy, int by, int shift, int w, int h,
                             uint8_t* __restrict__ dst, int dst_pitch, size_t dst_stride);

}
```

Baseline: 115,600.

## Store right-image aux in row-bucket order and batch patch loads in orient_brief

k_layout now writes each keypoint's bucket position (row_pos) instead of a row_items indirection list. orient_brief writes the aux record directly at that bucket-sorted position and packs the final index into aux.w, so stereo matching reads right keypoints contiguously without the kpsR/bucket_items indirection. The orient kernel also preloads level info per lane, groups four patch loads before computing moments, double-buffers the BRIEF window loads, and requests eight waves per EU. This adds register pressure, and it assumes the final index fits within the bits above kAuxIndexShift.

Measured after the change: 117,500, median of 6. 1.02x the previous value.

```diff
diff --git a/orb_slam3_detailed_comments_amd/csrc/k_describe.hip b/orb_slam3_detailed_comments_amd/csrc/k_describe.hip
--- a/orb_slam3_detailed_comments_amd/csrc/k_describe.hip
+++ b/orb_slam3_detailed_comments_amd/csrc/k_describe.hip
@@ -46,7 +46,7 @@
                                                 const uint32_t* __restrict__ lvl_keys, int kp_total_cap,
                                                 const int* __restrict__ lvl_count, int lap0, int lap1,
                                                 int* __restrict__ final_idx, int* __restrict__ n_out, int* __restrict__ mono_out,
-                                                int nb, int* __restrict__ row_start, int* __restrict__ row_items) {
+                                                int nb, int* __restrict__ row_start, int* __restrict__ row_pos) {
     ORBX_DYN_SMEM(smem);
     __shared__ unsigned long long s_scan[20];
     __shared__ int s_cnt[kMaxLevels], s_off[kMaxLevels + 1];
@@ -117,14 +117,14 @@
     if (kp_total_cap <= 256 * kLayoutPer) {
 #pragma unroll
         for (int k = 0; k < kLayoutPer; k++)
-            if (valid[k]) row_items[(size_t)b * kp_total_cap + atomicAdd(&cursor[bucket_of(key[k], lvl[k])], 1)] = fin[k];
+            if (valid[k]) row_pos[(size_t)b * kp_total_cap + tid * kLayoutPer + k] = atomicAdd(&cursor[bucket_of(key[k], lvl[k])], 1);
         return;
     }
     int l = 0;
     for (int s = tid; s < kp_total_cap; s += 256) {
         while (l + 1 < nlevels && s_off[l + 1] <= s) l++;
         if (s - s_off[l] < s_cnt[l])
-            row_items[(size_t)b * kp_total_cap + atomicAdd(&cursor[bucket_of(lvl_keys[(size_t)b * kp_total_cap + s], l)], 1)] = final_idx[(size_t)b * kp_total_cap + s];
+            row_pos[(size_t)b * kp_total_cap + s] = atomicAdd(&cursor[bucket_of(lvl_keys[(size_t)b * kp_total_cap + s], l)], 1);
     }
 }
 
@@ -132,11 +132,17 @@
 constexpr int kWinR = 18, kWinRows = 2 * kWinR + 1, kWinDw = 10, kWinTrips = (kWinRows * kWinDw + 63) / 64;
 static_assert(kKpPerWave == kKpPerWaveDecl, "orbx_kernels.h out of date");
 constexpr int kKpPerWaveSmall = kKpPerWaveSmallDecl;
+constexpr int kPatchGroup = 4;
+#ifdef ORBX_EMU
+#define ORBX_EIGHT_WAVES
+#else
+#define ORBX_EIGHT_WAVES __attribute__((amdgpu_waves_per_eu(8, 8)))
+#endif
 template <int KPW>
 __device__ __forceinline__ void orient_brief_impl(const LevelInfo* __restrict__ lv, int nlevels,
                                                       const uint8_t* __restrict__ pyr, const uint8_t* __restrict__ blur, size_t pyr_stride,
                                                       const uint32_t* __restrict__ lvl_keys, int kp_total_cap,
-                                                      const int* __restrict__ lvl_count, const int* __restrict__ final_idx,
+                                                      const int* __restrict__ lvl_count, const int* __restrict__ final_idx, const int* __restrict__ row_pos,
                                                       UmaxTab umax, KeyPointRec* __restrict__ out_kps,
                                                       unsigned long long* __restrict__ out_desc, int4* __restrict__ out_aux, int B, int groups_per_image) {
     __shared__ __attribute__((aligned(16))) uint8_t s_win[4][kWinRows * kWinDw * 4];
@@ -147,86 +153,134 @@
     const int slot0 = (gx * 4 + (int)(threadIdx.x >> 6)) * KPW;
     if (slot0 >= kp_total_cap) return;
     const int myslot = slot0 + (lane < KPW ? lane : 0);
-    int my_valid = 0, my_level = 0, my_pitch = 0, my_fi = 0;
-    uint32_t my_key = 0;
-    int my_off = 0;
-    if (myslot < kp_total_cap) {
-        for (int l = 1; l < nlevels; l++) if (myslot >= lv[l].kp_off) my_level = l;
-        const int i = myslot - lv[my_level].kp_off;
-        my_valid = i < lvl_count[(size_t)b * nlevels + my_level];
-        if (!my_valid && lane < KPW) {
-            const int zrow = final_idx[(size_t)b * kp_total_cap + myslot];
-            unsigned long long* z = out_desc + ((size_t)b * kp_total_cap + zrow) * 4;
-            z[0] = 0ull; z[1] = 0ull; z[2] = 0ull; z[3] = 0ull;
-        }
-        if (my_valid) {
-            my_key = lvl_keys[(size_t)b * kp_total_cap + myslot];
-            my_pitch = lv[my_level].pitch;
-            my_off = (int)lv[my_level].off + (key_y(my_key) + kBorder) * my_pitch + (key_x(my_key) + kBorder);
-            my_fi = final_idx[(size_t)b * kp_total_cap + myslot];
-        }
-    }
+    const int in_cap = myslot < kp_total_cap;
+    const int ll = lane < nlevels ? lane : nlevels - 1;
+    const int lv_kpoff = lv[ll].kp_off, lv_pitch = lv[ll].pitch, lv_off = lv[ll].off, lv_patch = lv[ll].patch;
+    const float lv_scale = lv[ll].scale;
+    const int lv_cnt = lvl_count[(size_t)b * nlevels + ll];
+    const size_t sl = (size_t)b * kp_total_cap + (in_cap ? myslot : slot0);
+    const uint32_t ld_key = lvl_keys[sl];
+    const int my_fi = final_idx[sl], my_pos = row_pos[sl];
+    const int r8 = lane >> 3, cg = lane & 7;
+    int um[4];
+#pragma unroll
+    for (int trip = 0; trip < 4; trip++) {
+        const int v = -kHalfPatch + 8 * trip + r8;
+        const int av = v < 0 ? -v : v;
+        um[trip] = umax.u[av <= kHalfPatch ? av : 0];
+    }
+    uint32_t pat[4];
+#pragma unroll
+    for (int r = 0; r < 4; r++) pat[r] = load_u32_any((const uint8_t*)&BRIEF_PATTERN[4 * (64 * r + lane)]);
+    int my_level = 0;
+    for (int l = 1; l < nlevels; l++) my_level += ORBX_READLANE(lv_kpoff, l) <= myslot;
+    const int my_pitch = __shfl(lv_pitch, my_level), my_patch = __shfl(lv_patch, my_level);
+    const float my_scale = __shfl(lv_scale, my_level);
+    const int my_kpoff = __shfl(lv_kpoff, my_level), my_cnt = __shfl(lv_cnt, my_level);
+    const int my_valid = in_cap && myslot - my_kpoff < my_cnt;
+    if (!my_valid && in_cap && lane < KPW) {
+        unsigned long long* z = out_desc + ((size_t)b * kp_total_cap + my_fi) * 4;
+        z[0] = 0ull; z[1] = 0ull; z[2] = 0ull; z[3] = 0ull;
+    }
+    const uint32_t my_key = my_valid ? ld_key : 0u;
+    const int my_off = __shfl(lv_off, my_level) + (key_y(my_key) + kBorder) * my_pitch + (key_x(my_key) + kBorder);
     const unsigned long long vmask = __ballot(my_valid && lane < KPW);
     if (vmask == 0ull) return;
     const BufRsrc raw0 = buf_make(pyr + (size_t)b * pyr_stride);
     const BufRsrc blur0 = buf_make(blur + (size_t)b * pyr_stride);
-    const int r8 = lane >> 3, cg = lane & 7;
-    uint32_t wu4[4], wv4[4], on4[4];
+    uint32_t wu4[4], on4[4];
 #pragma unroll
     for (int trip = 0; trip < 4; trip++) {
         const int v = -kHalfPatch + 8 * trip + r8;
         const int av = v < 0 ? -v : v;
-        uint32_t pu = 0, pv = 0, po = 0;
+        uint32_t pu = 0, po = 0;
 #pragma unroll
         for (int j = 0; j < 4; j++) {
             const int u = -kHalfPatch + 4 * cg + j;
             const int au = u < 0 ? -u : u;
-            const bool on = av <= kHalfPatch && au <= kHalfPatch && au <= umax.u[av <= kHalfPatch ? av : 0];
-            if (on) { pu |= (uint32_t)(u + 16) << (8 * j); pv |= (uint32_t)(v + 16) << (8 * j); po |= 1u << (8 * j); }
-        }
-        wu4[trip] = pu; wv4[trip] = pv; on4[trip] = po;
-    }
-    int my_m10 = 0, my_m01 = 0;
-    for (int k = 0; k < KPW; k++) {
-        if (!((vmask >> k) & 1ull)) continue;
+            const bool on = av <= kHalfPatch && au <= kHalfPatch && au <= um[trip];
+            if (on) { pu |= (uint32_t)(u + 16) << (8 * j); po |= 1u << (8 * j); }
+        }
+        wu4[trip] = pu; on4[trip] = po;
+    }
+    auto patch_load = [&](int k, uint32_t (&I4)[4]) {
         const int pitch = ORBX_READLANE(my_pitch, k);
         const uint32_t so = (uint32_t)(ORBX_READLANE(my_off, k) - kHalfPatch * pitch - kHalfPatch);
-        uint32_t I4[4];
+        const uint32_t vo = (uint32_t)(__mul24(r8, pitch) + 4 * cg);
 #pragma unroll
         for (int trip = 0; trip < 4; trip++)
-            I4[trip] = buf_load_u32(raw0, (uint32_t)(__mul24(8 * trip + r8, pitch) + 4 * cg), so);
-        uint32_t du = 0, dv = 0, ds = 0;
-#pragma unroll
-        for (int trip = 0; trip < 4; trip++) { du = dot4_u8(I4[trip], wu4[trip], du); dv = dot4_u8(I4[trip], wv4[trip], dv); ds = dot4_u8(I4[trip], on4[trip], ds); }
-        int m10 = (int)du - 16 * (int)ds, m01 = (int)dv - 16 * (int)ds;
+            I4[trip] = buf_load_u32(raw0, vo, so + (uint32_t)(8 * trip * pitch));
+    };
+    int my_m10 = 0, my_m01 = 0;
+    auto patch_moments = [&](int k, const uint32_t (&I4)[4]) {
+        uint32_t du = 0;
+        int ds = 0, m01 = 0;
+#pragma unroll
+        for (int trip = 0; trip < 4; trip++) {
+            const int s = (int)dot4_u8(I4[trip], on4[trip], 0u);
+            du = dot4_u8(I4[trip], wu4[trip], du); ds += s; m01 += mul24(-kHalfPatch + 8 * trip + r8, s);
+        }
+        int m10 = (int)du - 16 * ds;
         m10 = wave_sum(m10); m01 = wave_sum(m01);
         if (lane == k) { my_m10 = m10; my_m01 = m01; }
-    }
-    float my_angle, my_a, my_b;
-    steer_from_moments((float)my_m01, (float)my_m10, &my_angle, &my_a, &my_b);
-    float px0[4], py0[4], px1[4], py1[4];
-#pragma unroll
-    for (int r = 0; r < 4; r++) {
-        const signed char* p = &BRIEF_PATTERN[4 * (64 * r + lane)];
-        px0[r] = (float)p[0]; py0[r] = (float)p[1]; px1[r] = (float)p[2]; py1[r] = (float)p[3];
+    };
+    const int kfirst = __ffsll(vmask) - 1;
+    {
+        constexpr int G = KPW < kPatchGroup ? KPW : kPatchGroup;
+        unsigned long long rem = vmask;
+        while (rem) {
+            int ks[G];
+            uint32_t I4[G][4];
+#pragma unroll
+            for (int g = 0; g < G; g++) {
+                if (g == 0 || rem) { ks[g] = __ffsll(rem) - 1; rem &= rem - 1ull; }
+                else ks[g] = ks[g - 1];
+                patch_load(ks[g], I4[g]);
+            }
+#pragma unroll
+            for (int g = 0; g < G; g++) patch_moments(ks[g], I4[g]);
+        }
     }
     uint8_t* win = s_win[threadIdx.x >> 6];
-    for (int k = 0; k < KPW; k++) {
-        if (!((vmask >> k) & 1ull)) continue;
+    auto win_load = [&](int k, uint32_t (&wv)[kWinTrips]) {
         const int pitch = ORBX_READLANE(my_pitch, k);
         const uint32_t so = (uint32_t)(ORBX_READLANE(my_off, k) - kWinR * pitch - kWinR);
-        const float a = __int_as_float(ORBX_READLANE(__float_as_int(my_a), k)), bb = __int_as_float(ORBX_READLANE(__float_as_int(my_b), k));
-        const int fi = ORBX_READLANE(my_fi, k);
-        uint32_t wv[kWinTrips];
 #pragma unroll
         for (int t = 0; t < kWinTrips; t++) {
             const int i = lane + 64 * t;
             if (i < kWinRows * kWinDw) wv[t] = buf_load_u32(blur0, (uint32_t)(__mul24(i / kWinDw, pitch) + 4 * (i % kWinDw)), so);
         }
+    };
+    auto win_store = [&](const uint32_t (&wv)[kWinTrips]) {
         ORBX_WAVE_SYNC();
 #pragma unroll
         for (int t = 0; t < kWinTrips; t++) { const int i = lane + 64 * t; if (i < kWinRows * kWinDw) ((uint32_t*)win)[i] = wv[t]; }
         ORBX_WAVE_SYNC();
+    };
+    uint32_t wfirst[kWinTrips];
+    win_load(kfirst, wfirst);
+    float my_angle, my_a, my_b;
+    steer_from_moments((float)my_m01, (float)my_m10, &my_angle, &my_a, &my_b);
+    if (lane < KPW && my_valid) {
+        KeyPointRec k;
+        float xf = (float)(key_x(my_key) + kBorder), yf = (float)(key_y(my_key) + kBorder);
+        if (my_level != 0) { xf = __fmul_rn(xf, my_scale); yf = __fmul_rn(yf, my_scale); }
+        k.x = xf; k.y = yf; k.size = (float)my_patch; k.angle = my_angle; k.response = (float)key_s(my_key);
+        k.octave = my_level; k.class_id = -1;
+        out_kps[(size_t)b * kp_total_cap + my_fi] = k;
+        const float r = __fmul_rn(2.0f, my_scale);
+        int4 aux; aux.x = (int)floorf(__fsub_rn(yf, r)); aux.y = (int)ceilf(__fadd_rn(yf, r)); aux.z = __float_as_int(xf); aux.w = my_level | (my_fi << kAuxIndexShift);
+        out_aux[(size_t)b * kp_total_cap + my_pos] = aux;
+    }
+    float px0[4], py0[4], px1[4], py1[4];
+#pragma unroll
+    for (int r = 0; r < 4; r++) {
+        px0[r] = (float)(signed char)(pat[r] & 0xFFu); py0[r] = (float)(signed char)((pat[r] >> 8) & 0xFFu);
+        px1[r] = (float)(signed char)((pat[r] >> 16) & 0xFFu); py1[r] = (float)(signed char)(pat[r] >> 24);
+    }
+    auto brief = [&](int k) {
+        const float a = __int_as_float(ORBX_READLANE(__float_as_int(my_a), k)), bb = __int_as_float(ORBX_READLANE(__float_as_int(my_b), k));
+        const int fi = ORBX_READLANE(my_fi, k);
         constexpr float kRoundMagic = 12582912.0f;
         constexpr uint32_t kRoundFold = 0x400000u * (4u * kWinDw) + 0x4B400000u - (uint32_t)(kWinR * 4 * kWinDw + kWinR);
         int t0v[4], t1v[4];
@@ -246,36 +300,39 @@
             if (lane == r) mine = w;
         }
         if (lane < 4) out_desc[((size_t)b * kp_total_cap + fi) * 4 + lane] = mine;
-    }
-    if (lane < KPW && my_valid) {
-        const LevelInfo L = lv[my_level];
-        KeyPointRec k;
-        float xf = (float)(key_x(my_key) + kBorder), yf = (float)(key_y(my_key) + kBorder);
-        if (my_level != 0) { xf = __fmul_rn(xf, L.scale); yf = __fmul_rn(yf, L.scale); }
-        k.x = xf; k.y = yf; k.size = (float)L.patch; k.angle = my_angle; k.response = (float)key_s(my_key);
-        k.octave = my_level; k.class_id = -1;
-        out_kps[(size_t)b * kp_total_cap + my_fi] = k;
-        const float r = __fmul_rn(2.0f, L.scale);
-        int4 aux; aux.x = (int)floorf(__fsub_rn(yf, r)); aux.y = (int)ceilf(__fadd_rn(yf, r)); aux.z = __float_as_int(xf); aux.w = my_level;
-        out_aux[(size_t)b * kp_total_cap + my_fi] = aux;
-    }
-}
-
-__global__ void __launch_bounds__(256) k_orient_brief(const LevelInfo* __restrict__ lv, int nlevels,
+    };
+    win_store(wfirst);
+    {
+        unsigned long long rem = vmask & (vmask - 1ull);
+        int k = kfirst;
+        while (rem) {
+            const int kn = __ffsll(rem) - 1;
+            rem &= rem - 1ull;
+            uint32_t wn[kWinTrips];
+            win_load(kn, wn);
+            brief(k);
+            win_store(wn);
+            k = kn;
+        }
+        brief(k);
+    }
+}
+
+__global__ void __launch_bounds__(256) ORBX_EIGHT_WAVES k_orient_brief(const LevelInfo* __restrict__ lv, int nlevels,
                                                       const uint8_t* __restrict__ pyr, const uint8_t* __restrict__ blur, size_t pyr_stride,
                                                       const uint32_t* __restrict__ lvl_keys, int kp_total_cap,
-                                                      const int* __restrict__ lvl_count, const int* __restrict__ final_idx,
+                                                      const int* __restrict__ lvl_count, const int* __restrict__ final_idx, const int* __restrict__ row_pos,
                                                       UmaxTab umax, KeyPointRec* __restrict__ out_kps,
                                                       unsigned long long* __restrict__ out_desc, int4* __restrict__ out_aux, int B, int groups_per_image) {
-    orient_brief_impl<kKpPerWave>(lv, nlevels, pyr, blur, pyr_stride, lvl_keys, kp_total_cap, lvl_count, final_idx, umax, out_kps, out_desc, out_aux, B, groups_per_image);
-}
-__global__ void __launch_bounds__(256) k_orient_brief_small(const LevelInfo* __restrict__ lv, int nlevels,
+    orient_brief_impl<kKpPerWave>(lv, nlevels, pyr, blur, pyr_stride, lvl_keys, kp_total_cap, lvl_count, final_idx, row_pos, umax, out_kps, out_desc, out_aux, B, groups_per_image);
+}
+__global__ void __launch_bounds__(256) ORBX_EIGHT_WAVES k_orient_brief_small(const LevelInfo* __restrict__ lv, int nlevels,
                                                       const uint8_t* __restrict__ pyr, const uint8_t* __restrict__ blur, size_t pyr_stride,
                                                       const uint32_t* __restrict__ lvl_keys, int kp_total_cap,
-                                                      const int* __restrict__ lvl_count, const int* __restrict__ final_idx,
+                                                      const int* __restrict__ lvl_count, const int* __restrict__ final_idx, const int* __restrict__ row_pos,
                                                       UmaxTab umax, KeyPointRec* __restrict__ out_kps,
                                                       unsigned long long* __restrict__ out_desc, int4* __restrict__ out_aux, int B, int groups_per_image) {
-    orient_brief_impl<kKpPerWaveSmall>(lv, nlevels, pyr, blur, pyr_stride, lvl_keys, kp_total_cap, lvl_count, final_idx, umax, out_kps, out_desc, out_aux, B, groups_per_image);
+    orient_brief_impl<kKpPerWaveSmall>(lv, nlevels, pyr, blur, pyr_stride, lvl_keys, kp_total_cap, lvl_count, final_idx, row_pos, umax, out_kps, out_desc, out_aux, B, groups_per_image);
 }
 
 __global__ void __launch_bounds__(256) k_undistort(const KeyPointRec* __restrict__ kps, const int* __restrict__ n_per_frame, int cap, UndistortParams U,
diff --git a/orb_slam3_detailed_comments_amd/csrc/k_match.hip b/orb_slam3_detailed_comments_amd/csrc/k_match.hip
--- a/orb_slam3_detailed_comments_amd/csrc/k_match.hip
+++ b/orb_slam3_detailed_comments_amd/csrc/k_match.hip
@@ -20,9 +20,9 @@
 
 __global__ void __launch_bounds__(256) k_stereo_match(const LevelInfo* __restrict__ lv,
                                                       const KeyPointRec* __restrict__ kpsL, const unsigned long long* __restrict__ descL, const int* __restrict__ nL,
-                                                      const KeyPointRec* __restrict__ kpsR, const unsigned long long* __restrict__ descR,
+                                                      const unsigned long long* __restrict__ descR,
                                                       const int4* __restrict__ auxR, const int* __restrict__ nR,
-                                                      const int* __restrict__ bucket_start, const int* __restrict__ bucket_items, int nb, int lookback,
+                                                      const int* __restrict__ bucket_start, int nb, int lookback,
                                                       int cap, const uint8_t* __restrict__ pyrL, const uint8_t* __restrict__ pyrR, size_t pyr_stride,
                                                       StereoParams P, float* __restrict__ uRight, float* __restrict__ depth, int* __restrict__ sad) {
     const int b = (int)blockIdx.y, lane = lane_id();
@@ -31,83 +31,93 @@
     const size_t o = (size_t)b * cap + iL;
     if (iL >= nL[b]) { if (lane == 0) { uRight[o] = -1.0f; depth[o] = -1.0f; sad[o] = -1; } return; }
     const KeyPointRec kL = kpsL[o];
-    const int levelL = kL.octave;
+    const int levelL = ORBX_UNIFORM(kL.octave);
     const float uL = kL.x, vL = kL.y;
     const float maxD = __fdiv_rn(P.mbf, P.mb);
     const float minU = __fsub_rn(uL, maxD), maxU = uL;
     float out_u = -1.0f, out_d = -1.0f; int out_sad = -1;
     const int rowL = __float2int_rz(vL);
     const int nr = nR[b];
+    const LevelInfo& Lv = lv[levelL];
+    const float sf = Lv.inv_scale, Lscale = Lv.scale;
+    const int Lw = Lv.w, Lhh = Lv.h, Lpitch = Lv.pitch, Loff = Lv.off;
     unsigned best = (unsigned)P.th_high << 16;
+    int best_x = 0;
     if (!(maxU < 0)) {
         const unsigned long long* dl = descL + 4 * o;
         const unsigned long long d0 = dl[0], d1 = dl[1], d2 = dl[2], d3 = dl[3];
         const int4* ar = auxR + (size_t)b * cap;
         const int* bs = bucket_start + (size_t)b * (nb + 1);
-        const int* items = bucket_items + (size_t)b * cap;
         const int jbeg = bs[imin(imax(rowL - lookback, 0) >> kStereoRowShift, nb - 1)], jend = bs[imin(imax(rowL, 0) >> kStereoRowShift, nb - 1) + 1];
-        auto visit = [&](int iR, const int4& a) {
-            if (rowL < a.x || rowL > a.y) return;
-            if (a.w < levelL - 1 || a.w > levelL + 1) return;
+        auto gate = [&](const int4& a) {
+            const int oct = a.w & ((1 << kAuxIndexShift) - 1);
             const float xr = __int_as_float(a.z);
-            if (xr >= minU && xr <= maxU) {
-                const unsigned long long* dr = descR + 4 * ((size_t)b * cap + iR);
-                const int dist = __popcll(d0 ^ dr[0]) + __popcll(d1 ^ dr[1]) + __popcll(d2 ^ dr[2]) + __popcll(d3 ^ dr[3]);
-                const unsigned cand = ((unsigned)dist << 16) | (unsigned)iR;
-                if ((P.debug_flags & 2) ? dist < (int)(best >> 16) : cand < best) best = cand;
-            }
+            return rowL >= a.x && rowL <= a.y && oct >= levelL - 1 && oct <= levelL + 1 && xr >= minU && xr <= maxU;
+        };
+        auto take = [&](const int4& a, const unsigned long long* dr) {
+            const int dist = __popcll(d0 ^ dr[0]) + __popcll(d1 ^ dr[1]) + __popcll(d2 ^ dr[2]) + __popcll(d3 ^ dr[3]);
+            const unsigned cand = ((unsigned)dist << 16) | (unsigned)(a.w >> kAuxIndexShift);
+            if ((P.debug_flags & 2) ? dist < (int)(best >> 16) : cand < best) { best = cand; best_x = a.z; }
         };
         if (P.debug_flags & 4) {
-            for (int j = jend - 1; j >= jbeg; j--) { const int iR = items[j]; visit(iR, ar[iR]); }
+            for (int j = jend - 1; j >= jbeg; j--) {
+                const int4 a = ar[j];
+                if (gate(a)) take(a, descR + 4 * ((size_t)b * cap + (a.w >> kAuxIndexShift)));
+            }
         } else
         for (int base = jbeg; base < jend; base += 128) {
-            int4 a[2]; int idx[2];
+            int4 a[2];
 #pragma unroll
             for (int u = 0; u < 2; u++) {
-                int j = base + 64 * u + lane;
+                const int j = base + 64 * u + lane;
                 const bool in = j < jend;
-                if (P.debug_flags & 1) j = jend - 1 - (j - jbeg);
-                idx[u] = in ? items[j] : -1;
-            }
+                int jj = in ? j : jend - 1;
+                if (P.debug_flags & 1) jj = jend - 1 - (jj - jbeg);
+                a[u] = ar[jj];
+                if (!in) { a[u].x = 1; a[u].y = 0; }
+            }
+            bool pass[2];
+            unsigned long long r[2][4];
 #pragma unroll
             for (int u = 0; u < 2; u++) {
-                if (idx[u] >= 0) a[u] = ar[idx[u]]; else { a[u].x = 1; a[u].y = 0; a[u].z = 0; a[u].w = 0; }
-            }
-#pragma unroll
-            for (int u = 0; u < 2; u++) visit(idx[u], a[u]);
-        }
-    }
+                pass[u] = gate(a[u]);
+                const unsigned long long* dr = pass[u] ? descR + 4 * ((size_t)b * cap + (a[u].w >> kAuxIndexShift)) : dl;
+#pragma unroll
+                for (int w = 0; w < 4; w++) r[u][w] = dr[w];
+            }
+#pragma unroll
+            for (int u = 0; u < 2; u++) if (pass[u]) take(a[u], r[u]);
+        }
+    }
+    const unsigned mine = best;
     best = wave_min_u32(best);
     const int bestDist = (int)(best >> 16);
     if (bestDist < P.th_orb && nr > 0) {
-        const int bestIdxR = (int)(best & 0xFFFFu);
-        const float uR0 = kpsR[(size_t)b * cap + bestIdxR].x;
-        const LevelInfo Lv = lv[levelL];
-        const float sf = Lv.inv_scale;
+        const float uR0 = __int_as_float(ORBX_READLANE(best_x, __ffsll(__ballot(mine == best)) - 1));
         const float scaleduL = roundf(__fmul_rn(kL.x, sf)), scaledvL = roundf(__fmul_rn(kL.y, sf));
         const float scaleduR0 = roundf(__fmul_rn(uR0, sf));
         const int w = 5, Lh = 5;
         const float iniu = scaleduR0 + (float)(Lh - w), endu = scaleduR0 + (float)(Lh + w + 1);
         const int cu = (int)scaleduL, cv = (int)scaledvL, cr = (int)scaleduR0;
-        const bool inb = cv - w >= 0 && cv + w < Lv.h && cu - w >= 0 && cu + w < Lv.w && cr - Lh - w >= 0 && cr + Lh + w < Lv.w;
-        if (!(iniu < 0 || endu >= (float)Lv.w) && inb) {
-            const uint8_t* IL = pyrL + (size_t)b * pyr_stride + Lv.off;
-            const uint8_t* IR = pyrR + (size_t)b * pyr_stride + Lv.off;
-            const int g = lane >> 4, k = lane & 15;
+        const bool inb = cv - w >= 0 && cv + w < Lhh && cu - w >= 0 && cu + w < Lw && cr - Lh - w >= 0 && cr + Lh + w < Lw;
+        if (!(iniu < 0 || endu >= (float)Lw) && inb) {
+            const uint8_t* IL = pyrL + (size_t)b * pyr_stride + Loff;
+            const uint8_t* IR = pyrR + (size_t)b * pyr_stride + Loff;
+            const int g = lane >> 4, k = lane & 15, kk = imin(k, 10);
+            uint32_t l0[3], l1[3], l2[3], r0[3], r1[3], r2[3];
+#pragma unroll
+            for (int t = 0; t < 3; t++) {
+                const int rofs = __mul24(cv - w + imin(g + 4 * t, 10), Lpitch);
+                const uint8_t* lp = IL + (uint32_t)(rofs + (cu - w));
+                const uint8_t* rp = IR + (uint32_t)(rofs + (cr - w - Lh + kk));
+                l0[t] = load_u32_any(lp); l1[t] = load_u32_any(lp + 4); l2[t] = load_u32_any(lp + 7);
+                r0[t] = load_u32_any(rp); r1[t] = load_u32_any(rp + 4); r2[t] = load_u32_any(rp + 7);
+            }
             uint32_t acc = 0;
-            if (k < 11) {
-#pragma unroll
-                for (int t = 0; t < 3; t++) {
-                    const int row = g + 4 * t;
-                    if (row < 11) {
-                        const int rofs = __mul24(cv - w + row, Lv.pitch);
-                        const uint8_t* lp = IL + (uint32_t)(rofs + (cu - w));
-                        const uint8_t* rp = IR + (uint32_t)(rofs + (cr - w - Lh + k));
-                        const uint32_t l0 = load_u32_any(lp), l1 = load_u32_any(lp + 4), l2 = load_u32_any(lp + 7) & 0xFFFFFF00u;
-                        const uint32_t r0 = load_u32_any(rp), r1 = load_u32_any(rp + 4), r2 = load_u32_any(rp + 7) & 0xFFFFFF00u;
-                        acc = sad4_u8(l0, r0, sad4_u8(l1, r1, sad4_u8(l2, r2, acc)));
-                    }
-                }
+#pragma unroll
+            for (int t = 0; t < 3; t++) {
+                const uint32_t s = sad4_u8(l0[t], r0[t], sad4_u8(l1[t], r1[t], sad4_u8(l2[t] & 0xFFFFFF00u, r2[t] & 0xFFFFFF00u, 0u)));
+                if (g + 4 * t < 11 && k < 11) acc += s;
             }
             acc += __shfl_xor(acc, 16);
             acc += __shfl_xor(acc, 32);
@@ -118,7 +128,7 @@
                 const float deltaR = __fdiv_rn(__fsub_rn(dist1, dist3),
                                                __fmul_rn(2.0f, __fsub_rn(__fadd_rn(dist1, dist3), __fmul_rn(2.0f, dist2))));
                 if (!(deltaR < -1 || deltaR > 1)) {
-                    float bestuR = __fmul_rn(Lv.scale, __fadd_rn(__fadd_rn(scaleduR0, (float)bestinc), deltaR));
+                    float bestuR = __fmul_rn(Lscale, __fadd_rn(__fadd_rn(scaleduR0, (float)bestinc), deltaR));
                     float disparity = __fsub_rn(uL, bestuR);
                     if (disparity >= 0 && disparity < maxD) {
                         if (disparity <= 0) { disparity = 0.01f; bestuR = (float)((double)uL - 0.01); }
diff --git a/orb_slam3_detailed_comments_amd/csrc/orbx_api.cpp b/orb_slam3_detailed_comments_amd/csrc/orbx_api.cpp
--- a/orb_slam3_detailed_comments_amd/csrc/orbx_api.cpp
+++ b/orb_slam3_detailed_comments_amd/csrc/orbx_api.cpp
@@ -325,7 +325,7 @@
         h->d_status.p = h->d_nm.p ? h->d_nm.p + 2 * b : nullptr; h->d_status.n = h->d_nm.p ? 4 : 0;
         e |= h->d_kps.ensure(b * cap); e |= h->d_desc.ensure(b * cap * 4); e |= h->d_aux.ensure(b * cap * 4);
         e |= h->d_uRight.ensure(b * cap); e |= h->d_depth.ensure(b * cap); e |= h->d_sad.ensure(b * cap); e |= h->d_nmatch.ensure(b);
-        e |= h->d_rowstart.ensure(b * (size_t)((h->H >> kStereoRowShift) + 3)); e |= h->d_rowitems.ensure(b * cap);
+        e |= h->d_rowstart.ensure(b * (size_t)((h->H >> kStereoRowShift) + 3)); e |= h->d_rowpos.ensure(b * cap);
         e |= h->d_knn.ensure(4 * b * cap); e |= h->d_ratio.ensure(b * cap);
         e |= h->h_nm.ensure(3 * b + 4); e |= h->h_cnt.ensure(2 * b + 4); e |= h->d_qtprof.ensure(32);
         if (e) return fail(ORBX_E_DEVICE, "device allocation failed (batch %d of %dx%d)", B, W, H);
@@ -478,7 +478,7 @@
     {
         dim3 grid(B, 1, 1);
         ORBX_LAUNCH(k_layout, grid, blk1, 2 * (size_t)(nb_rows + 1) * sizeof(int), h->s0, (const LevelInfo*)h->d_lv.p, nl, (const uint32_t*)h->d_lvl_keys.p, h->kp_total_cap,
-                    (const int*)h->d_lvl_count.p, lap0, lap1, h->d_final_idx.p, h->d_nm.p, h->d_nm.p + h->maxB, nb_rows, h->d_rowstart.p, h->d_rowitems.p);
+                    (const int*)h->d_lvl_count.p, lap0, lap1, h->d_final_idx.p, h->d_nm.p, h->d_nm.p + h->maxB, nb_rows, h->d_rowstart.p, h->d_rowpos.p);
     }
     stage_end(h, ST_LAYOUT, h->s0);
     if (!one_launch) rt::stream_wait_event(h->s0, h->ev_join);
@@ -490,10 +490,10 @@
         dim3 grid(gpi * 8 * ((B + 7) / 8), 1, 1);
         if (small) ORBX_LAUNCH(k_orient_brief_small, grid, blk1, 0, h->s0, (const LevelInfo*)h->d_lv.p, nl, (const uint8_t*)h->d_pyr.p, (const uint8_t*)h->d_blur.p,
                     h->pyr_stride, (const uint32_t*)h->d_lvl_keys.p, h->kp_total_cap, (const int*)h->d_lvl_count.p, (const int*)h->d_final_idx.p,
-                    h->umax, h->d_kps.p, h->d_desc.p, (int4*)h->d_aux.p, B, gpi);
+                    (const int*)h->d_rowpos.p, h->umax, h->d_kps.p, h->d_desc.p, (int4*)h->d_aux.p, B, gpi);
         else ORBX_LAUNCH(k_orient_brief, grid, blk1, 0, h->s0, (const LevelInfo*)h->d_lv.p, nl, (const uint8_t*)h->d_pyr.p, (const uint8_t*)h->d_blur.p,
                     h->pyr_stride, (const uint32_t*)h->d_lvl_keys.p, h->kp_total_cap, (const int*)h->d_lvl_count.p, (const int*)h->d_final_idx.p,
-                    h->umax, h->d_kps.p, h->d_desc.p, (int4*)h->d_aux.p, B, gpi);
+                    (const int*)h->d_rowpos.p, h->umax, h->d_kps.p, h->d_desc.p, (int4*)h->d_aux.p, B, gpi);
     }
     if (h->undist.active) {
         dim3 grid((h->kp_total_cap + 255) / 256, B, 1);
@@ -562,7 +562,7 @@
     for (auto& x : h->d_si) x.release();
     h->d_kps_un.release();
     h->d_lp.release(); h->d_depth_in.release(); h->h_lp_in.release(); h->h_lp_out.release();
-    h->d_aux.release(); h->d_qtprof.release(); h->d_qtpool.release(); h->d_rowstart.release(); h->d_rowitems.release();
+    h->d_aux.release(); h->d_qtprof.release(); h->d_qtpool.release(); h->d_rowstart.release(); h->d_rowpos.release();
     h->d_mapx.release(); h->d_mapy.release(); h->d_in_xt.release(); h->d_in_yt.release(); h->d_frame.release();
     h->d_exp.release(); for (auto& x : h->h_exp) x.release();
     delete h;
@@ -1111,9 +1111,9 @@
     const int lookback = (int)std::ceil(4.0f * R->scale[R->nlevels - 1]) + 2;
     ORBX_LAUNCH(k_stereo_match, grid, blk, 0, L->s0, (const LevelInfo*)L->d_lv.p,
                 (const KeyPointRec*)(L->d_kps.p + (size_t)lf * cap), (const unsigned long long*)(L->d_desc.p + (size_t)lf * cap * 4), (const int*)(L->d_nm.p + lf),
-                (const KeyPointRec*)(R->d_kps.p + (size_t)rf * cap), (const unsigned long long*)(R->d_desc.p + (size_t)rf * cap * 4),
+                (const unsigned long long*)(R->d_desc.p + (size_t)rf * cap * 4),
                 (const int4*)(R->d_aux.p + (size_t)rf * cap * 4), (const int*)(R->d_nm.p + rf),
-                (const int*)(R->d_rowstart.p + (size_t)rf * (nb + 1)), (const int*)(R->d_rowitems.p + (size_t)rf * cap), nb, lookback, cap, (const uint8_t*)(L->d_pyr.p + (size_t)lf * L->pyr_stride), (const uint8_t*)(R->d_pyr.p + (size_t)rf * R->pyr_stride), L->pyr_stride,
+                (const int*)(R->d_rowstart.p + (size_t)rf * (nb + 1)), nb, lookback, cap, (const uint8_t*)(L->d_pyr.p + (size_t)lf * L->pyr_stride), (const uint8_t*)(R->d_pyr.p + (size_t)rf * R->pyr_stride), L->pyr_stride,
                 P, L->d_uRight.p, L->d_depth.p, L->d_sad.p);
     dim3 grid2(B, 1, 1);
     ORBX_LAUNCH(k_stereo_median, grid2, blk, 0, L->s0, (const int*)(L->d_nm.p + lf), cap, L->d_uRight.p, L->d_depth.p,
diff --git a/orb_slam3_detailed_comments_amd/csrc/orbx_internal.h b/orb_slam3_detailed_comments_amd/csrc/orbx_internal.h
--- a/orb_slam3_detailed_comments_amd/csrc/orbx_internal.h
+++ b/orb_slam3_detailed_comments_amd/csrc/orbx_internal.h
@@ -123,7 +123,7 @@
     const void* g_images = nullptr; const void* g_pyr = nullptr;
     bool in_active = false; int in_channels = 1, in_rgb = 1, in_gray_variant = 0, in_geometry = 0, in_out_w = 0, in_out_h = 0, in_tap_w = 0, in_tap_h = 0;
     orbx::DevBuf<float> d_mapx, d_mapy; orbx::DevBuf<orbx::ResizeTap> d_in_xt, d_in_yt; orbx::DevBuf<uint8_t> d_frame;
-    orbx::DevBuf<int> d_rowstart, d_rowitems;
+    orbx::DevBuf<int> d_rowstart, d_rowpos;
     orbx::DevBuf<uint8_t> d_lp, d_depth_in; orbx::HostBuf<uint8_t> h_lp_in, h_lp_out;
     size_t lp_pool = 0; bool lp_pending = false;
     orbx::PendingBatch batch;
diff --git a/orb_slam3_detailed_comments_amd/csrc/orbx_kernels.h b/orb_slam3_detailed_comments_amd/csrc/orbx_kernels.h
--- a/orb_slam3_detailed_comments_amd/csrc/orbx_kernels.h
+++ b/orb_slam3_detailed_comments_amd/csrc/orbx_kernels.h
@@ -77,23 +77,24 @@
 __global__ void k_layout(const LevelInfo* __restrict__ lv, int nlevels, const uint32_t* __restrict__ lvl_keys,
                          int kp_total_cap, const int* __restrict__ lvl_count, int lap0, int lap1,
                          int* __restrict__ final_idx, int* __restrict__ n_out, int* __restrict__ mono_out,
-                         int nb, int* __restrict__ row_start, int* __restrict__ row_items);
+                         int nb, int* __restrict__ row_start, int* __restrict__ row_pos);
 #ifndef ORBX_STEREO_ROW_SHIFT
 #define ORBX_STEREO_ROW_SHIFT 3
 #endif
 constexpr int kStereoRowShift = ORBX_STEREO_ROW_SHIFT;
+constexpr int kAuxIndexShift = 8;
 constexpr int kKpPerWaveDecl = 8;
 constexpr int kKpPerWaveSmallDecl = 2;
 __global__ void k_orient_brief(const LevelInfo* __restrict__ lv, int nlevels, const uint8_t* __restrict__ pyr,
                                const uint8_t* __restrict__ blur, size_t pyr_stride,
                                const uint32_t* __restrict__ lvl_keys, int kp_total_cap,
-                               const int* __restrict__ lvl_count, const int* __restrict__ final_idx, UmaxTab umax,
+                               const int* __restrict__ lvl_count, const int* __restrict__ final_idx, const int* __restrict__ row_pos, UmaxTab umax,
                                KeyPointRec* __restrict__ out_kps, unsigned long long* __restrict__ out_desc, int4* __restrict__ out_aux,
                                int B, int groups_per_image);
 __global__ void k_orient_brief_small(const LevelInfo* __restrict__ lv, int nlevels, const uint8_t* __restrict__ pyr,
                                const uint8_t* __restrict__ blur, size_t pyr_stride,
                                const uint32_t* __restrict__ lvl_keys, int kp_total_cap,
-                               const int* __restrict__ lvl_count, const int* __restrict__ final_idx, UmaxTab umax,
+                               const int* __restrict__ lvl_count, const int* __restrict__ final_idx, const int* __restrict__ row_pos, UmaxTab umax,
                                KeyPointRec* __restrict__ out_kps, unsigned long long* __restrict__ out_desc, int4* __restrict__ out_aux,
                                int B, int groups_per_image);
 __global__ void k_undistort(const KeyPointRec* __restrict__ kps, const int* __restrict__ n_per_frame, int cap, UndistortParams U, KeyPointRec* __restrict__ kps_un);
@@ -101,9 +102,9 @@
                                  const unsigned long long* __restrict__ Bm, int nb, int* __restrict__ out);
 __global__ void k_stereo_match(const LevelInfo* __restrict__ lv, const KeyPointRec* __restrict__ kpsL,
                                const unsigned long long* __restrict__ descL, const int* __restrict__ nL,
-                               const KeyPointRec* __restrict__ kpsR, const unsigned long long* __restrict__ descR,
+                               const unsigned long long* __restrict__ descR,
                                const int4* __restrict__ auxR, const int* __restrict__ nR, const int* __restrict__ bucket_start,
-                               const int* __restrict__ bucket_items, int nb, int lookback, int cap, const uint8_t* __restrict__ pyrL,
+                               int nb, int lookback, int cap, const uint8_t* __restrict__ pyrL,
                                const uint8_t* __restrict__ pyrR, size_t pyr_stride, StereoParams P,
                                float* __restrict__ uRight, float* __restrict__ depth, int* __restrict__ sad);
 __global__ void k_stereo_median(const int* __restrict__ nL, int cap, float* __restrict__ uRight,
```
